# nubot-nudt/LCR-Net

Measured on AMD Instinct MI355X. Metric: scans/s (120k-pt KITTI-shape scan -> 256-D descriptor), higher is better.
Workload: dtype f32 (K-deep GEMMs, K >= 288 and N >= 64: fp32 operands as bf16 x 3 split, 6 of 9 products on the bf16 matrix cores, fp32 accumulate — error vs fp64 <= the fp32-MFMA kernel's; every other GEMM, KPConv and attention: fp32 MFMA); 1 GPU; configs[1]: batch of 8 synthetic 64-beam scans (~120k pts, 0.3 m voxel -> ~16k pts), voxelise + 3 subsamples + 10 radius searches + KPConv encoder + NetVLAD, seeded random weights; distinct_input_batches=4, streams=pre-processing stream (own host thread, 2 batches ahead) + 2 encoder stream(s), parallelism=scan-parallel x1, all-gather of descriptors

## Files before the change

include/lcr_hip.h:

```cpp
#ifndef LCR_HIP_H
#define LCR_HIP_H
#include <stddef.h>
#include <stdint.h>
#ifdef __cplusplus
extern "C" {
#endif

#define LCR_OK 0
#define LCR_EARG (-1)
#define LCR_ESPACE (-2)
#define LCR_EHIP (-3)

#define LCR_STATUS_KEY_OVERFLOW 1u
#define LCR_STATUS_LEN_MISMATCH 2u
#define LCR_GN_REPLICAS 8

const char* lcr_last_error(void);
void lcr_ktimer_enable(int on);
void lcr_ktimer_sample(int every);
void lcr_ktimer_kinds(unsigned mask);
int lcr_ktimer_read(int kind, int max_records, double* seconds, int64_t* meta);
int lcr_ktimer_read2(int kind, int max_records, double* seconds, double* seconds_kernel, int64_t* meta);
int lcr_stream_spin(int microseconds, void* stream);
int lcr_version(void);

int lcr_grid_subsample_ws_bytes(int64_t n_cap, int B, size_t* bytes);
int lcr_grid_subsample(const float* xyz, const int64_t* len, int B, int64_t n_cap, float voxel,
                       float* out_xyz, int64_t* out_len, uint32_t* status,
                       void* ws, size_t ws_bytes, void* stream);
int lcr_grid_subsample_ex(const float* xyz, const int64_t* len, int B, int64_t n_cap, float voxel, int key_bits_hint,
                          float* out_xyz, int64_t* out_len, uint32_t* status,
                          void* ws, size_t ws_bytes, void* stream);
int lcr_grid_subsample_rows(const float* xyz, int row_floats, const int64_t* len, int B, int64_t n_cap, float voxel, int key_bits_hint,
                            float* out_xyz, int64_t* out_len, uint32_t* status,
                            void* ws, size_t ws_bytes, void* stream);
int lcr_hashmap_order_host(const uint64_t* keys_host, int64_t n, int64_t* order_host);
int lcr_hashmap_bucket_host(const uint64_t* codes_host, int64_t n, int phase, int64_t* out_host);

int lcr_voxel_down_sample_ws_bytes(int64_t n_cap, int B, size_t* bytes);
int lcr_voxel_down_sample(const float* rows, int row_floats, int out_cols, const int64_t* len, int B, int64_t n_cap, double voxel,
                          int key_bits_hint, float* out_f32, double* out_f64, int64_t* out_len, uint32_t* status,
                          void* ws, size_t ws_bytes, void* stream);

int lcr_support_grid_ws_bytes(int64_t ns_cap, int B, size_t* bytes);
int lcr_support_grid_build(const float* s, const int64_t* slen, int B, int64_t ns_cap, float radius,
                           uint32_t* status, void* grid_ws, size_t grid_ws_bytes, void* stream);
int lcr_radius_query(const float* q, const int64_t* qlen, int B, int64_t nq_cap,
                     const void* grid_ws, int64_t ns_cap , float radius, int limit,
                     int64_t* out_idx64, int32_t* out_idx32, int32_t* out_cnt, void* stream);
int lcr_radius_query_ordered(const float* q, const int64_t* qlen, int B, int64_t nq_cap,
                             const void* grid_ws, int64_t ns_cap, float radius, int limit,
                             int64_t* out_idx64, int32_t* out_idx32, int32_t* out_cnt, const int32_t* q_order, void* stream);
typedef struct LcrRadiusQuery {
    const float*   q;
    const int64_t* qlen;
    int64_t        nq_cap;
    const void*    grid_ws;
    int64_t        ns_cap;
    float          radius;
    int            limit;
    int32_t*       out_idx32;
    const int32_t* q_order;
} LcrRadiusQuery;
#define LCR_RADIUS_QUERY_MULTI_MAX 12
int lcr_radius_query_multi(const LcrRadiusQuery* list, int n, int B, void* stream);
int lcr_support_grid_build_ex(const float* s, const int64_t* slen, int B, int64_t ns_cap, float radius,
                              uint32_t* status, void* grid_ws, size_t grid_ws_bytes, int32_t* order, void* stream);
int lcr_support_grid_order(const void* grid_ws, int64_t ns_cap, int B, int32_t* order, void* stream);
int lcr_radius_search_ws_bytes(int64_t nq_cap, int64_t ns_cap, int B, size_t* bytes);
int lcr_radius_search(const float* q, const float* s, const int64_t* qlen, const int64_t* slen, int B,
                      int64_t nq_cap, int64_t ns_cap, float radius, int limit,
                      int64_t* out_idx64, int32_t* out_idx32, int32_t* out_cnt, uint32_t* status,
                      void* ws, size_t ws_bytes, void* stream);

#define LCR_MAX_STAGES 8
typedef struct LcrPrecomputeLayout {
  int     num_stages, B, upsampling;
  int64_t n_raw;
  int     limits[LCR_MAX_STAGES];
  int64_t cap[LCR_MAX_STAGES];
  size_t  off_points[LCR_MAX_STAGES];
  size_t  off_lengths[LCR_MAX_STAGES];
  size_t  off_order[LCR_MAX_STAGES];
  size_t  off_neighbors[LCR_MAX_STAGES];
  size_t  off_subsampling[LCR_MAX_STAGES];
  size_t  off_upsampling[LCR_MAX_STAGES];
  size_t  out_bytes, ws_bytes;
} LcrPrecomputeLayout;
int lcr_precompute_layout(int64_t n0, int B, int num_stages, const int* limits, int upsampling, int64_t n_raw,
                          LcrPrecomputeLayout* layout);
int lcr_precompute_batch(const float* points0, const int64_t* lengths0, const LcrPrecomputeLayout* layout, float voxel_size,
                         float radius, float raw_voxel, int key_bits_hint, void* out, size_t out_bytes, void* ws, size_t ws_bytes,
                         int64_t* lengths_host, uint32_t* status_host, void* stream);
int lcr_precompute_batch_rows(const float* points0, int raw_row_floats, const int64_t* lengths0, const LcrPrecomputeLayout* layout,
                              float voxel_size, float radius, float raw_voxel, int key_bits_hint, void* out, size_t out_bytes, void* ws,
                              size_t ws_bytes, int64_t* lengths_host, uint32_t* status_host, void* stream);
int lcr_precompute_ws_bytes_ex(const LcrPrecomputeLayout* layout, int raw_method, size_t* bytes);
int lcr_precompute_batch_rows_ex(const float* points0, int raw_row_floats, const int64_t* lengths0, const LcrPrecomputeLayout* layout,
                                 float voxel_size, float radius, double raw_voxel, int raw_method, int key_bits_hint, void* out,
                                 size_t out_bytes, void* ws, size_t ws_bytes, int64_t* lengths_host, uint32_t* status_host, void* stream);

int lcr_gemm_f32(const float* A, const float* B, float* C, int64_t M, int N, int K, int transA, int transB,
                 const float* bias, const float* rowdiv, const int64_t* seg_len, int S, int groups, double* stats,
                 void* stream);
int lcr_split_bf16x3(const float* w, int64_t n, uint16_t* planes, void* stream);
int lcr_split_bf16x3_tiles(const float* w, int N, int K, uint16_t* tiles, void* stream);
int lcr_gemm_f32_bsplit(const float* A, const uint16_t* Bs_tiles, float* C, int64_t M, int N, int K, const float* bias, const float* rowdiv,
                        const int64_t* seg_len, int S, int groups, double* stats, void* stream);
int lcr_gemm_f32_masked(const float* A, const float* B, float* C, int64_t M, int N, int K, const float* bias, const float* rowdiv,
                        const int64_t* seg_len, int S, int groups, double* stats, const uint16_t* row_mask, int block_k, void* stream);
int lcr_gemm_f32_bsplit_masked(const float* A, const uint16_t* Bs_tiles, float* C, int64_t M, int N, int K, const float* bias,
                               const float* rowdiv, const int64_t* seg_len, int S, int groups, double* stats, const uint16_t* row_mask,
                               int block_k, void* stream);
int lcr_kpconv_mask_ok(int64_t M, int N, int K, int split);
int lcr_gemm_f32_anorm(const float* A, const float* B, float* C, int64_t M, int N, int K, const float* bias,
                       const double* a_stats, const float* a_gamma, const float* a_beta, int a_groups, float a_eps,
                       float a_slope, const int64_t* seg_len, int S, int groups, double* stats, void* stream);
int lcr_gemm_f32_batched_ta(const float* A, const float* B, float* C, int64_t M, int N, int count, const int* k_host,
                            const int64_t* a_off_host, const int64_t* b_off_host, const int64_t* c_off_host, void* stream);
int lcr_kpconv_aggregate(const float* s_feats, const uint8_t* s_pos, const float* q_pts, const float* s_pts,
                         const void* idx, int idx_is_64, int64_t M, int64_t Ns, int H, int C,
                         const float* kernel_points_host, float sigma, float* A, float* nn,
                         const int32_t* order , void* stream);
#define LCR_KP_VALID_FIRST 1
int lcr_kpconv_aggregate_ex(const float* s_feats, const uint8_t* s_pos, const float* q_pts, const float* s_pts,
                            const void* idx, int idx_is_64, int64_t M, int64_t Ns, int H, int C,
                            const float* kernel_points_host, float sigma, float* A, float* nn,
                            const int32_t* order, int flags, void* stream);
int lcr_kpconv_aggregate_mask(const float* s_feats, const uint8_t* s_pos, const float* q_pts, const float* s_pts,
                              const void* idx, int idx_is_64, int64_t M, int64_t Ns, int H, int C,
                              const float* kernel_points_host, float sigma, float* A, float* nn, uint16_t* mask,
                              const int32_t* order, int flags, void* stream);
int lcr_kpconv_fused(const float* s_feats, const uint8_t* s_pos, const float* q_pts, const float* s_pts, const void* idx,
                     int idx_is_64, int64_t M, int64_t Ns, int H, int C, const float* kernel_points_host, float sigma,
                     const float* W, const float* bias, float* out, const int64_t* seg_len, int S, int groups, double* stats,
                     const int32_t* order, void* stream);
int lcr_kpconv_cin1(const float* s_feats, const float* q_pts, const float* s_pts, const void* idx, int idx_is_64,
                    int64_t M, int64_t Ns, int H, const float* kernel_points_host, float sigma, const float* W,
                    const float* bias, int Cout, float* out, const int32_t* order, void* stream);
int lcr_maxpool(const float* x, const void* idx, int idx_is_64, int64_t M, int64_t Ns, int H, int C, float* out,
                const int32_t* order, void* stream);
int lcr_row_positive(const float* x, int64_t N, int C, uint8_t* pos, void* stream);
int lcr_groupnorm_stats(const float* x, int64_t N, int C, int groups, const int64_t* seg_len, int S, double* stats, void* stream);
int lcr_groupnorm_apply(const float* x, const double* stats, const float* gamma, const float* beta, const float* res,
                        const double* res_stats, const float* res_gamma, const float* res_beta, float* y, int64_t N, int C,
                        int groups, const int64_t* seg_len, int S, float eps, float slope, int act, uint8_t* pos, void* stream);

#define LCR_ENC_BLOCKS 10
typedef struct LcrUnaryW {
  const float *w, *b;
  const float *gn_w, *gn_b;
  const uint16_t* w_split;
} LcrUnaryW;
typedef struct LcrBlockW {
  int   cin, cout, strided;
  float sigma;
  const float* kernel_points_host;
  const float *kp_w, *kp_b;
  const float* kp_wt;
  const uint16_t* kp_wt_split;
  const float *normconv_w, *normconv_b;
  LcrUnaryW unary1, unary2, shortcut;
} LcrBlockW;
typedef struct LcrEncoderW {
  int   groups, c1_cout;
  float c1_sigma;
  const float* c1_kernel_points_host;
  const float *c1_w, *c1_b;
  const float *c1_gn_w, *c1_gn_b;
  LcrBlockW blocks[LCR_ENC_BLOCKS];
} LcrEncoderW;
int lcr_encoder_ws_bytes(const LcrEncoderW* W, const int64_t* n_host, int S, size_t* bytes);
int lcr_encoder_forward(const LcrEncoderW* W, const float* feats0, const float* const* points, const int32_t* const* neighbors,
                        const int32_t* const* subsampling, const int32_t* const* order, const int64_t* const* seg_len, int S,
                        const int64_t* n_host, const int64_t* seg_min_rows_host, const int* limits, float* const* out_feats, void* ws,
                        size_t ws_bytes, void* stream);
#define LCR_ENC_LISTS_VALID_FIRST 1u
int lcr_encoder_forward_ex(const LcrEncoderW* W, const float* feats0, const float* const* points, const int32_t* const* neighbors,
                           const int32_t* const* subsampling, const int32_t* const* order, const int64_t* const* seg_len, int S,
                           const int64_t* n_host, const int64_t* seg_min_rows_host, const int* limits, float* const* out_feats,
                           unsigned flags, void* ws, size_t ws_bytes, void* stream);

typedef struct LcrNetvladWeights {
  const float* cluster_weights;
  const float* cluster_weights2;
  const float* hidden1_weights;
  const float *bn1_w, *bn1_b, *bn1_mean, *bn1_var;
  const float *bn2_w, *bn2_b, *bn2_mean, *bn2_var;
  const float* gating_weights;
  const float *gbn_w, *gbn_b, *gbn_mean, *gbn_var;
} LcrNetvladWeights;
int lcr_netvlad_ws_bytes(int64_t n_rows, int S, size_t* bytes);
int lcr_netvlad_forward(const float* feats , const int64_t* seg_len_host, int S,
                        const LcrNetvladWeights* weights_host, float* out , void* ws, size_t ws_bytes, void* stream);

int lcr_rotary_embed(float* x, const float* theta, int64_t N, int heads, void* stream);
int lcr_attention_f32(const float* q, const float* k, const float* v, int64_t Nq, int64_t Nk, int heads, int head_dim,
                      float* out, void* stream);
int lcr_attention_seg_f32(const float* q, const float* k, const float* v, const int64_t* q_len_host, const int64_t* k_len_host, int P,
                          int heads, int head_dim, float* out, void* stream);
int lcr_attention_topk_f32(const float* q, const float* k, const float* v, const int64_t* q_len_host, const int64_t* k_len_host,
                           const int* kk_host, int P, int heads, int head_dim, float* out, void* stream);
int lcr_add_layernorm(const float* a, const float* b, const float* gamma, const float* beta, int64_t N, int D, float eps,
                      float* y, void* stream);
int lcr_relu_inplace(float* x, int64_t n, void* stream);

#define LCR_ROFORMER_MAX_BLOCKS 16
typedef struct LcrLinearW {
  const float *w, *b;
} LcrLinearW;
typedef struct LcrRoformerLayerW {
  LcrLinearW   q, k, v, lin;
  const float *ln1_w, *ln1_b;
  float        ln1_eps;
  LcrLinearW   expand, squeeze;
  const float *ln2_w, *ln2_b;
  float        ln2_eps;
} LcrRoformerLayerW;
typedef struct LcrRoformerW {
  int        d_in, d_model, d_out, heads, num_blocks;
  int        block_is_self[LCR_ROFORMER_MAX_BLOCKS];
  LcrLinearW emb1, emb2, in_proj, out_proj;
  LcrRoformerLayerW layers[LCR_ROFORMER_MAX_BLOCKS];
} LcrRoformerW;
int lcr_roformer_ws_bytes(const LcrRoformerW* W, int64_t n_rows, size_t* bytes);
int lcr_roformer_forward(const LcrRoformerW* W, const float* points, const float* feats, const int64_t* lens0_host, const int64_t* lens1_host,
                         int P, float* out, float* theta_out, void* ws, size_t ws_bytes, void* stream);

int lcr_retrieval_ws_bytes(int64_t Q, int64_t C, size_t* bytes);
int lcr_retrieval_topk(const float* queries , int64_t Q, int64_t q0, const float* database , int64_t C,
                       int D, int k, int exclude, int32_t* out_idx , float* out_d2 ,
                       void* ws, size_t ws_bytes, void* stream);

int lcr_gemm_f32_strided_batched(const float* A, const float* B, float* C, int64_t M, int N, int K, int transA, int transB,
                                 int64_t strideA, int64_t strideB, int64_t strideC, int count, void* stream);

int lcr_vote_shift(const float* xyz, const float* offsets, int64_t N, float max_range, float* out, void* stream);
int lcr_greedy_nms_ws_bytes(int64_t n_total, size_t* bytes);
int lcr_greedy_nms(const float* pts, const int64_t* len, int B, int64_t n_total, float radius, uint8_t* keep,
                   int64_t* out_len, void* ws, void* stream);
int lcr_neighbor_mean(const float* pts, const void* idx, int idx_is_64, int64_t M, int H, int64_t pad, float* out, void* stream);
int lcr_point_to_node_ws_bytes(int64_t N, int M, size_t* bytes);
int lcr_point_to_node_partition(const float* points, int64_t N, const float* nodes, int M, int K, int32_t* p2n, int64_t* knn,
                                uint8_t* knn_mask, uint8_t* node_mask, uint32_t* status, void* ws, size_t ws_bytes, void* stream);

int lcr_point_to_node_partition_stack(const float* points, const int64_t* point_off, const float* nodes, const int64_t* node_off, int C, int K,
                                      int32_t* p2n_out, int64_t* knn, uint8_t* knn_mask, uint8_t* node_mask, uint32_t* status, void* ws,
                                      size_t ws_bytes, void* stream);
int lcr_build_padded_scores(const float* raw, const uint8_t* row_mask, const uint8_t* col_mask, int64_t B, int M, int N,
                            float scale, const float* alpha, float inf_val, float* S, void* stream);
int lcr_log_sinkhorn(float* S, const uint8_t* row_mask, const uint8_t* col_mask, int64_t B, int M, int N, int iters,
                     float inf_val, float* uv_ws, void* stream);
int lcr_log_sinkhorn_ws_floats(int64_t B, int M, int N, size_t* floats);
int lcr_log_sinkhorn_form(int64_t B, int M, int N, int* form);
int lcr_log_sinkhorn_ex(float* S, const uint8_t* row_mask, const uint8_t* col_mask, int64_t B, int M, int N, int iters,
                        float inf_val, float* uv_ws, size_t uv_floats, void* stream);
int lcr_top1_matching_ws_bytes(int64_t B, int M, int N, size_t* bytes);
int lcr_top1_matching(const float* logS, int64_t B, int M, int N, const uint8_t* row_mask, const uint8_t* col_mask,
                      int64_t* total, int32_t* out_bij, float* out_score, void* ws, size_t ws_bytes, void* stream);
int lcr_top1_matching_ex(const float* logS, int64_t B, int M, int N, const uint8_t* row_mask, const uint8_t* col_mask, int mutual,
                         int64_t* total, int32_t* out_bij, float* out_score, void* ws, size_t ws_bytes, void* stream);
int lcr_patch_scores(const float* feats_a, int64_t Na, const float* feats_b, int64_t Nb, int C, const int64_t* idx_a, const int64_t* idx_b,
                     const uint8_t* mask_a, const uint8_t* mask_b, int64_t P, int K, float scale, const float* alpha, float inf_val, float* S,
                     void* stream);
int lcr_topk_matching_ws_bytes(int64_t B, int M, int N, size_t* bytes);
int lcr_topk_matching(const float* logS, int64_t B, int M, int N, const uint8_t* row_mask, const uint8_t* col_mask, int K, int mutual,
                      int64_t* total, int32_t* out_bij, float* out_score, void* ws, size_t ws_bytes, void* stream);
int lcr_topk_matching_ex(const float* logS, int64_t B, int M, int N, const uint8_t* row_mask, const uint8_t* col_mask, int K, int mutual,
                         int use_dustbin, float confidence_threshold, const float* global_scores, int64_t* total, int32_t* out_bij,
                         float* out_score, void* ws, size_t ws_bytes, void* stream);
int lcr_upsample_concat(const float* x, int64_t Nx, int C1, const void* idx, int idx_is_64, int H, const float* skip, int C2,
                        int64_t N, float* out, void* stream);
int lcr_gather_rows(const float* src, int64_t pad, int C, const int64_t* idx, int64_t R, float* out, void* stream);
int lcr_procrustes_batched(const float* src, const float* ref, const float* w, const int32_t* start, int P, float eps, float* T, void* stream);
int lcr_inlier_count(const float* T, int P, const float* src, const float* ref, int n, float radius, const int32_t* start,
                     int min_count, int32_t* counts, int32_t* best, void* stream);
int lcr_lgr_ws_bytes(int64_t n, int H, int S, size_t* bytes);
int lcr_local_global_registration(const float* src, const float* ref, const float* score, int64_t n, const int32_t* hyp_start, int H,
                                  const int32_t* seg_hyp_start, int S, float radius, int min_count, int steps, float* T_out,
                                  float* hyp_out, int32_t* counts_out, int32_t* best_out, void* ws, size_t ws_bytes, void* stream);
int lcr_local_global_registration_ex(const float* src, const float* ref, const float* score, int64_t n, const int32_t* hyp_start, int H,
                                     const int32_t* seg_hyp_start, int S, float radius, int min_count, int steps, int correspondence_limit,
                                     float* T_out, float* hyp_out, int32_t* counts_out, int32_t* best_out, void* ws, size_t ws_bytes,
                                     void* stream);
int lcr_inlier_weights(const float* T_all, const int32_t* sel, const float* src, const float* ref, const float* score, int n,
                       float radius, float* w_out, void* stream);

int lcr_ransac_ws_bytes(int S, int iterations, size_t* bytes);
int lcr_ransac_correspondences(const float* src, const float* ref, const int32_t* start, int S, float thr, int ransac_n, int iterations,
                               uint64_t seed, float* T, int32_t* inliers, float* rmse, int32_t* best_h, float* T_all, int32_t* counts_all,
                               float* sse_all, void* ws, size_t ws_bytes, void* stream);
int lcr_ransac_sample_host(uint64_t seed, int64_t h0, int64_t count, int ransac_n, int64_t n, int32_t* idx_host);
int lcr_ransac_ex_ws_bytes(int S, int iterations, int64_t n_corr, size_t* bytes);
int lcr_ransac_correspondences_ex(const float* src, const float* ref, const int32_t* start, int S, const int32_t* corr, const int32_t* src_start,
                                  const int32_t* ref_start, int64_t n_corr, float thr, int ransac_n, int iterations, uint64_t seed,
                                  float edge_similarity, float checker_distance, float* T, int32_t* inliers, float* rmse, int32_t* best_h,
                                  float* T_all, int32_t* counts_all, float* sse_all, uint8_t* reject_all, void* ws, size_t ws_bytes, void* stream);

int lcr_feature_nn_ws_bytes(int S, int64_t nq, int64_t nd, size_t* bytes);
int lcr_feature_nn(const float* qf, const float* df, const int32_t* q_start, const int32_t* d_start, int S, int C, int64_t nq, int64_t nd,
                   int32_t* nn, float* d2, void* ws, size_t ws_bytes, void* stream);
int lcr_feature_correspondences_ws_bytes(int S, size_t* bytes);
int lcr_feature_correspondences(const int32_t* nn_sr, const int32_t* src_start, const int32_t* nn_rs, const int32_t* ref_start, int S, int min_rows,
                                int32_t* corr, int32_t* start, int32_t* mutual_used, void* ws, size_t ws_bytes, void* stream);

int lcr_icp_ws_bytes(int S, int64_t ns, int64_t nt, size_t* bytes);
int lcr_icp_point_to_point(const float* src, const int64_t* src_len, const float* tgt, const int64_t* tgt_len, int S, const double* init,
                           float max_correspondence_distance, int max_iteration, double relative_fitness, double relative_rmse, double* T,
                           double* fitness, double* inlier_rmse, int32_t* iterations, int32_t* corr, double* T_hist, double* fitness_hist,
                           double* rmse_hist, int check_every, void* ws, size_t ws_bytes, void* stream);

int lcr_icp_plane_ws_bytes(int S, int64_t ns, int64_t nt, size_t* bytes);
int lcr_icp_point_to_plane(const float* src, const int64_t* src_len, const float* tgt, const int64_t* tgt_len, const float* tgt_normals, int S,
                           const double* init, float max_correspondence_distance, int max_iteration, double relative_fitness,
                           double relative_rmse, double* T, double* fitness, double* inlier_rmse, int32_t* iterations, int32_t* corr,
                           double* T_hist, double* fitness_hist, double* rmse_hist, int check_every, void* ws, size_t ws_bytes, void* stream);

int lcr_normals_ws_bytes(int B, int64_t n, size_t* bytes);
int lcr_estimate_normals(const float* points, const int64_t* lengths, int B, float radius, int max_nn, const float* viewpoint, float* normals,
                         float* curvature, int32_t* count, void* ws, size_t ws_bytes, void* stream);

#ifdef __cplusplus
}
#endif
#endif
```

include/lcr_hip_debug.h:

```cpp
#ifndef LCR_HIP_DEBUG_H
#define LCR_HIP_DEBUG_H

#ifdef __cplusplus
extern "C" {
#endif

void lcr_gemm_debug_force_tile(int tile);
void lcr_gemm_debug_deep(int mode);
void lcr_gemm_debug_streamk(int mode);
void lcr_groupnorm_debug_general(int on);
void lcr_kpconv_debug_off64(int on);

#ifdef __cplusplus
}
#endif
#endif
```

lcr-net_amd/_lib.py:

```python
import ctypes
import os

import torch

_PKG = os.path.dirname(os.path.abspath(__file__))
LIB_PATH = os.path.join(_PKG, "liblcr_hip.so")

_lib = None

c_f32p = ctypes.c_void_p
c_vp = ctypes.c_void_p
c_i64 = ctypes.c_int64
c_int = ctypes.c_int
c_float = ctypes.c_float
c_size_p = ctypes.POINTER(ctypes.c_size_t)
c_size_t = ctypes.c_size_t

_SIGS = {
    "lcr_last_error": (ctypes.c_char_p, []),
    "lcr_version": (c_int, []),
    "lcr_support_grid_ws_bytes": (c_int, [c_i64, c_int, c_size_p]),
    "lcr_support_grid_build": (c_int, [c_vp, c_vp, c_int, c_i64, c_float, c_vp, c_vp, ctypes.c_size_t, c_vp]),
    "lcr_precompute_layout": (c_int, [c_i64, c_int, c_int, c_vp, c_int, c_i64, c_vp]),
    "lcr_precompute_batch": (c_int, [c_vp, c_vp, c_vp, c_float, c_float, c_float, c_int, c_vp, c_size_t, c_vp, c_size_t, c_vp, c_vp, c_vp]),
    "lcr_precompute_batch_rows": (c_int, [c_vp, c_int, c_vp, c_vp, c_float, c_float, c_float, c_int, c_vp, c_size_t, c_vp, c_size_t, c_vp, c_vp, c_vp]),
    "lcr_precompute_ws_bytes_ex": (c_int, [c_vp, c_int, c_size_p]),
    "lcr_precompute_batch_rows_ex": (c_int, [c_vp, c_int, c_vp, c_vp, c_float, c_float, ctypes.c_double, c_int, c_int, c_vp, c_size_t, c_vp, c_size_t,
                                             c_vp, c_vp, c_vp]),
    "lcr_radius_query_multi": (c_int, [c_vp, c_int, c_int, c_vp]),
    "lcr_radius_query": (c_int, [c_vp, c_vp, c_int, c_i64, c_vp, c_i64, c_float, c_int, c_vp, c_vp, c_vp, c_vp]),
    "lcr_stream_spin": (c_int, [c_int, c_vp]),
    "lcr_radius_query_ordered": (c_int, [c_vp, c_vp, c_int, c_i64, c_vp, c_i64, c_float, c_int, c_vp, c_vp, c_vp, c_vp, c_vp]),
    "lcr_radius_search_ws_bytes": (c_int, [c_i64, c_i64, c_int, c_size_p]),
    "lcr_radius_search": (c_int, [c_vp, c_vp, c_vp, c_vp, c_int, c_i64, c_i64, c_float, c_int, c_vp, c_vp, c_vp, c_vp,
                                  c_vp, ctypes.c_size_t, c_vp]),
    "lcr_grid_subsample_ws_bytes": (c_int, [c_i64, c_int, c_size_p]),
    "lcr_grid_subsample": (c_int, [c_vp, c_vp, c_int, c_i64, c_float, c_vp, c_vp, c_vp, c_vp, ctypes.c_size_t, c_vp]),
    "lcr_grid_subsample_ex": (c_int, [c_vp, c_vp, c_int, c_i64, c_float, c_int, c_vp, c_vp, c_vp, c_vp, ctypes.c_size_t, c_vp]),
    "lcr_grid_subsample_rows": (c_int, [c_vp, c_int, c_vp, c_int, c_i64, c_float, c_int, c_vp, c_vp, c_vp, c_vp, ctypes.c_size_t, c_vp]),
    "lcr_hashmap_order_host": (c_int, [c_vp, c_i64, c_vp]),
    "lcr_hashmap_bucket_host": (c_int, [c_vp, c_i64, c_int, c_vp]),
    "lcr_voxel_down_sample_ws_bytes": (c_int, [c_i64, c_int, c_size_p]),
    "lcr_voxel_down_sample": (c_int, [c_vp, c_int, c_int, c_vp, c_int, c_i64, ctypes.c_double, c_int, c_vp, c_vp, c_vp, c_vp, c_vp, ctypes.c_size_t,
                                      c_vp]),
    "lcr_gemm_f32": (c_int, [c_vp, c_vp, c_vp, c_i64, c_int, c_int, c_int, c_int, c_vp, c_vp, c_vp, c_int, c_int, c_vp, c_vp]),
    "lcr_gemm_f32_anorm": (c_int, [c_vp, c_vp, c_vp, c_i64, c_int, c_int, c_vp, c_vp, c_vp, c_vp, c_int, c_float, c_float, c_vp, c_int,
                                   c_int, c_vp, c_vp]),
    "lcr_ktimer_enable": (None, [c_int]),
    "lcr_ktimer_sample": (None, [c_int]),
    "lcr_ktimer_kinds": (None, [ctypes.c_uint]),
    "lcr_ktimer_read": (c_int, [c_int, c_int, c_vp, c_vp]),
    "lcr_ktimer_read2": (c_int, [c_int, c_int, c_vp, c_vp, c_vp]),
    "lcr_encoder_ws_bytes": (c_int, [c_vp, c_vp, c_int, c_size_p]),
    "lcr_encoder_forward": (c_int, [c_vp, c_vp, c_vp, c_vp, c_vp, c_vp, c_vp, c_int, c_vp, c_vp, c_vp, c_vp, c_vp, c_size_t, c_vp]),
    "lcr_roformer_ws_bytes": (c_int, [c_vp, c_i64, c_size_p]),
    "lcr_roformer_forward": (c_int, [c_vp, c_vp, c_vp, c_vp, c_vp, c_int, c_vp, c_vp, c_vp, c_size_t, c_vp]),
    "lcr_encoder_forward_ex": (c_int, [c_vp, c_vp, c_vp, c_vp, c_vp, c_vp, c_vp, c_int, c_vp, c_vp, c_vp, c_vp, ctypes.c_uint, c_vp, c_size_t, c_vp]),
    "lcr_kpconv_aggregate": (c_int, [c_vp, c_vp, c_vp, c_vp, c_vp, c_int, c_i64, c_i64, c_int, c_int, c_vp, c_float, c_vp, c_vp, c_vp, c_vp]),
    "lcr_kpconv_aggregate_mask": (c_int, [c_vp, c_vp, c_vp, c_vp, c_vp, c_int, c_i64, c_i64, c_int, c_int, c_vp, c_float, c_vp, c_vp, c_vp, c_vp,
                                          c_int, c_vp]),
    "lcr_kpconv_fused": (c_int, [c_vp, c_vp, c_vp, c_vp, c_vp, c_int, c_i64, c_i64, c_int, c_int, c_vp, c_float, c_vp, c_vp, c_vp, c_vp, c_int,
                                 c_int, c_vp, c_vp, c_vp]),
    "lcr_kpconv_cin1": (c_int, [c_vp, c_vp, c_vp, c_vp, c_int, c_i64, c_i64, c_int, c_vp, c_float, c_vp, c_vp, c_int, c_vp, c_vp, c_vp]),
    "lcr_maxpool": (c_int, [c_vp, c_vp, c_int, c_i64, c_i64, c_int, c_int, c_vp, c_vp, c_vp]),
    "lcr_support_grid_order": (c_int, [c_vp, c_i64, c_int, c_vp, c_vp]),
    "lcr_row_positive": (c_int, [c_vp, c_i64, c_int, c_vp, c_vp]),
    "lcr_groupnorm_stats": (c_int, [c_vp, c_i64, c_int, c_int, c_vp, c_int, c_vp, c_vp]),
    "lcr_groupnorm_apply": (c_int, [c_vp, c_vp, c_vp, c_vp, c_vp, c_vp, c_vp, c_vp, c_vp, c_i64, c_int, c_int, c_vp, c_int,
                                    c_float, c_float, c_int, c_vp, c_vp]),
    "lcr_rotary_embed": (c_int, [c_vp, c_vp, c_i64, c_int, c_vp]),
    "lcr_attention_f32": (c_int, [c_vp, c_vp, c_vp, c_i64, c_i64, c_int, c_int, c_vp, c_vp]),
    "lcr_attention_seg_f32": (c_int, [c_vp, c_vp, c_vp, c_vp, c_vp, c_int, c_int, c_int, c_vp, c_vp]),
    "lcr_attention_topk_f32": (c_int, [c_vp, c_vp, c_vp, c_vp, c_vp, c_vp, c_int, c_int, c_int, c_vp, c_vp]),
    "lcr_add_layernorm": (c_int, [c_vp, c_vp, c_vp, c_vp, c_i64, c_int, c_float, c_vp, c_vp]),
    "lcr_relu_inplace": (c_int, [c_vp, c_i64, c_vp]),
    "lcr_retrieval_ws_bytes": (c_int, [c_i64, c_i64, c_size_p]),
    "lcr_retrieval_topk": (c_int, [c_vp, c_i64, c_i64, c_vp, c_i64, c_int, c_int, c_int, c_vp, c_vp, c_vp, ctypes.c_size_t, c_vp]),
    "lcr_gemm_f32_strided_batched": (c_int, [c_vp, c_vp, c_vp, c_i64, c_int, c_int, c_int, c_int, c_i64, c_i64, c_i64, c_int, c_vp]),
    "lcr_gemm_f32_batched_ta": (c_int, [c_vp, c_vp, c_vp, c_i64, c_int, c_int, c_vp, c_vp, c_vp, c_vp, c_vp]),
    "lcr_vote_shift": (c_int, [c_vp, c_vp, c_i64, c_float, c_vp, c_vp]),
    "lcr_greedy_nms_ws_bytes": (c_int, [c_i64, c_size_p]),
    "lcr_greedy_nms": (c_int, [c_vp, c_vp, c_int, c_i64, c_float, c_vp, c_vp, c_vp, c_vp]),
    "lcr_neighbor_mean": (c_int, [c_vp, c_vp, c_int, c_i64, c_int, c_i64, c_vp, c_vp]),
    "lcr_point_to_node_ws_bytes": (c_int, [c_i64, c_int, c_size_p]),
    "lcr_point_to_node_partition": (c_int, [c_vp, c_i64, c_vp, c_int, c_int, c_vp, c_vp, c_vp, c_vp, c_vp, c_vp, ctypes.c_size_t, c_vp]),
    "lcr_point_to_node_partition_stack": (c_int, [c_vp, c_vp, c_vp, c_vp, c_int, c_int, c_vp, c_vp, c_vp, c_vp, c_vp, c_vp, ctypes.c_size_t, c_vp]),
    "lcr_build_padded_scores": (c_int, [c_vp, c_vp, c_vp, c_i64, c_int, c_int, c_float, c_vp, c_float, c_vp, c_vp]),
    "lcr_log_sinkhorn": (c_int, [c_vp, c_vp, c_vp, c_i64, c_int, c_int, c_int, c_float, c_vp, c_vp]),
    "lcr_log_sinkhorn_ws_floats": (c_int, [c_i64, c_int, c_int, c_size_p]),
    "lcr_log_sinkhorn_form": (c_int, [c_i64, c_int, c_int, ctypes.POINTER(c_int)]),
    "lcr_split_bf16x3": (c_int, [c_vp, c_i64, c_vp, c_vp]),
    "lcr_split_bf16x3_tiles": (c_int, [c_vp, c_int, c_int, c_vp, c_vp]),
    "lcr_gemm_f32_bsplit": (c_int, [c_vp, c_vp, c_vp, c_i64, c_int, c_int, c_vp, c_vp, c_vp, c_int, c_int, c_vp, c_vp]),
    "lcr_gemm_f32_bsplit_masked": (c_int, [c_vp, c_vp, c_vp, c_i64, c_int, c_int, c_vp, c_vp, c_vp, c_int, c_int, c_vp, c_vp, c_int, c_vp]),
    "lcr_gemm_f32_masked": (c_int, [c_vp, c_vp, c_vp, c_i64, c_int, c_int, c_vp, c_vp, c_vp, c_int, c_int, c_vp, c_vp, c_int, c_vp]),
    "lcr_kpconv_mask_ok": (c_int, [c_i64, c_int, c_int, c_int]),
    "lcr_log_sinkhorn_ex": (c_int, [c_vp, c_vp, c_vp, c_i64, c_int, c_int, c_int, c_float, c_vp, ctypes.c_size_t, c_vp]),
    "lcr_top1_matching_ws_bytes": (c_int, [c_i64, c_int, c_int, c_size_p]),
    "lcr_top1_matching": (c_int, [c_vp, c_i64, c_int, c_int, c_vp, c_vp, c_vp, c_vp, c_vp, c_vp, ctypes.c_size_t, c_vp]),
    "lcr_top1_matching_ex": (c_int, [c_vp, c_i64, c_int, c_int, c_vp, c_vp, c_int, c_vp, c_vp, c_vp, c_vp, ctypes.c_size_t, c_vp]),
    "lcr_topk_matching_ws_bytes": (c_int, [c_i64, c_int, c_int, c_size_p]),
    "lcr_topk_matching": (c_int, [c_vp, c_i64, c_int, c_int, c_vp, c_vp, c_int, c_int, c_vp, c_vp, c_vp, c_vp, ctypes.c_size_t, c_vp]),
    "lcr_patch_scores": (c_int, [c_vp, c_i64, c_vp, c_i64, c_int, c_vp, c_vp, c_vp, c_vp, c_i64, c_int, c_float, c_vp, c_float, c_vp, c_vp]),
    "lcr_topk_matching_ex": (c_int, [c_vp, c_i64, c_int, c_int, c_vp, c_vp, c_int, c_int, c_int, c_float, c_vp, c_vp, c_vp, c_vp, c_vp, ctypes.c_size_t,
                                     c_vp]),
    "lcr_local_global_registration_ex": (c_int, [c_vp, c_vp, c_vp, c_i64, c_vp, c_int, c_vp, c_int, c_float, c_int, c_int, c_int, c_vp, c_vp, c_vp, c_vp,
                                                 c_vp, ctypes.c_size_t, c_vp]),
    "lcr_upsample_concat": (c_int, [c_vp, c_i64, c_int, c_vp, c_int, c_int, c_vp, c_int, c_i64, c_vp, c_vp]),
    "lcr_gather_rows": (c_int, [c_vp, c_i64, c_int, c_vp, c_i64, c_vp, c_vp]),
    "lcr_procrustes_batched": (c_int, [c_vp, c_vp, c_vp, c_vp, c_int, c_float, c_vp, c_vp]),
    "lcr_inlier_count": (c_int, [c_vp, c_int, c_vp, c_vp, c_int, c_float, c_vp, c_int, c_vp, c_vp, c_vp]),
    "lcr_inlier_weights": (c_int, [c_vp, c_vp, c_vp, c_vp, c_vp, c_int, c_float, c_vp, c_vp]),
    "lcr_lgr_ws_bytes": (c_int, [c_i64, c_int, c_int, c_size_p]),
    "lcr_local_global_registration": (c_int, [c_vp, c_vp, c_vp, c_i64, c_vp, c_int, c_vp, c_int, c_float, c_int, c_int, c_vp, c_vp, c_vp, c_vp, c_vp,
                                              ctypes.c_size_t, c_vp]),
    "lcr_netvlad_ws_bytes": (c_int, [c_i64, c_int, c_size_p]),
    "lcr_netvlad_forward": (c_int, [c_vp, c_vp, c_int, c_vp, c_vp, c_vp, ctypes.c_size_t, c_vp]),
    "lcr_ransac_ws_bytes": (c_int, [c_int, c_int, c_size_p]),
    "lcr_ransac_correspondences": (c_int, [c_vp, c_vp, c_vp, c_int, c_float, c_int, c_int, ctypes.c_uint64, c_vp, c_vp, c_vp, c_vp, c_vp, c_vp, c_vp,
                                           c_vp, ctypes.c_size_t, c_vp]),
    "lcr_ransac_sample_host": (c_int, [ctypes.c_uint64, c_i64, c_i64, c_int, c_i64, c_vp]),
    "lcr_ransac_ex_ws_bytes": (c_int, [c_int, c_int, c_i64, c_size_p]),
    "lcr_ransac_correspondences_ex": (c_int, [c_vp, c_vp, c_vp, c_int, c_vp, c_vp, c_vp, c_i64, c_float, c_int, c_int, ctypes.c_uint64, c_float,
                                              c_float, c_vp, c_vp, c_vp, c_vp, c_vp, c_vp, c_vp, c_vp, c_vp, ctypes.c_size_t, c_vp]),
    "lcr_feature_nn_ws_bytes": (c_int, [c_int, c_i64, c_i64, c_size_p]),
    "lcr_feature_nn": (c_int, [c_vp, c_vp, c_vp, c_vp, c_int, c_int, c_i64, c_i64, c_vp, c_vp, c_vp, ctypes.c_size_t, c_vp]),
    "lcr_feature_correspondences_ws_bytes": (c_int, [c_int, c_size_p]),
    "lcr_feature_correspondences": (c_int, [c_vp, c_vp, c_vp, c_vp, c_int, c_int, c_vp, c_vp, c_vp, c_vp, ctypes.c_size_t, c_vp]),
    "lcr_icp_ws_bytes": (c_int, [c_int, c_i64, c_i64, c_size_p]),
    "lcr_icp_point_to_point": (c_int, [c_vp, c_vp, c_vp, c_vp, c_int, c_vp, c_float, c_int, ctypes.c_double, ctypes.c_double, c_vp, c_vp, c_vp, c_vp,
                                       c_vp, c_vp, c_vp, c_vp, c_int, c_vp, ctypes.c_size_t, c_vp]),
    "lcr_icp_plane_ws_bytes": (c_int, [c_int, c_i64, c_i64, c_size_p]),
    "lcr_icp_point_to_plane": (c_int, [c_vp, c_vp, c_vp, c_vp, c_vp, c_int, c_vp, c_float, c_int, ctypes.c_double, ctypes.c_double, c_vp, c_vp,
                                       c_vp, c_vp, c_vp, c_vp, c_vp, c_vp, c_int, c_vp, ctypes.c_size_t, c_vp]),
    "lcr_normals_ws_bytes": (c_int, [c_int, c_i64, c_size_p]),
    "lcr_estimate_normals": (c_int, [c_vp, c_vp, c_int, c_float, c_int, c_vp, c_vp, c_vp, c_vp, c_vp, ctypes.c_size_t, c_vp]),
}


_RELEASES_GIL = {"lcr_roformer_forward", "lcr_precompute_batch", "lcr_precompute_batch_rows", "lcr_precompute_batch_rows_ex", "lcr_hashmap_bucket_host", "lcr_encoder_forward", "lcr_encoder_forward_ex", "lcr_ktimer_read",
                 "lcr_ktimer_read2", "lcr_hashmap_order_host", "lcr_ransac_sample_host", "lcr_icp_point_to_point", "lcr_icp_point_to_plane", "lcr_netvlad_forward", "lcr_log_sinkhorn", "lcr_log_sinkhorn_ex",
                 "lcr_local_global_registration", "lcr_local_global_registration_ex", "lcr_retrieval_topk", "lcr_stream_spin"}


def build():
    import importlib.util
    spec = importlib.util.spec_from_file_location("_lcr_build", os.path.join(_PKG, "csrc", "build.py"))
    mod = importlib.util.module_from_spec(spec)
    spec.loader.exec_module(mod)
    return mod.build()


def lib():
    global _lib
    if _lib is None:
        if not os.path.exists(LIB_PATH):
            raise RuntimeError(
                "liblcr_hip.so not found at %s — build it with `python lcr-net_amd/csrc/build.py` "
                "(there is no CPU fallback for the lcr-net_amd hot path)" % LIB_PATH)
        L = ctypes.CDLL(LIB_PATH)
        for name, (res, args) in _SIGS.items():
            if not hasattr(L, name):
                continue
            fn = getattr(L, name)
            fn.restype = res
            fn.argtypes = args
        if os.environ.get("LCR_CTYPES_KEEP_GIL", "1") != "0":
            K = ctypes.PyDLL(LIB_PATH)
            for name, (res, args) in _SIGS.items():
                if name in _RELEASES_GIL or not hasattr(K, name):
                    continue
                fn = getattr(K, name)
                fn.restype = res
                fn.argtypes = args
                setattr(L, name, fn)
        _lib = L
    return _lib


def check(rc, what):
    if rc != 0:
        msg = lib().lcr_last_error()
        raise RuntimeError("%s failed (rc=%d): %s" % (what, rc, msg.decode() if msg else ""))


def ptr(t):
    return ctypes.c_void_p(t.data_ptr()) if t is not None else ctypes.c_void_p(0)


def stream_ptr(device=None):
    idx = device.index if isinstance(device, torch.device) else None
    if idx is None:
        idx = torch.cuda.current_device() if not isinstance(device, int) else device
    return ctypes.c_void_p(torch._C._cuda_getCurrentRawStream(idx))


def require_cuda(*tensors):
    for t in tensors:
        if t is not None and not t.is_cuda:
            raise RuntimeError("lcr-net_amd ops run on the GPU only: got a %s tensor (no CPU fallback)" % t.device)


def workspace(nbytes, device):
    return torch.empty(max(int(nbytes), 256), dtype=torch.uint8, device=device)
```

lcr-net_amd/csrc/encoder.hip:

```cpp
#include <algorithm>
#include <cstdlib>
#include <cstring>

#include "common.h"

#define TURN(call) ([&]() { LaunchTurn turn_; return (call); }())

namespace lcr {

constexpr float ENC_GN_EPS = 1e-5f;
constexpr float ENC_SLOPE = 0.1f;

struct Arena {
  char*  base;
  size_t off, cap;
  template <typename T>
  T* take(size_t n) {
    const size_t o = off;
    off = align_up(off + n * sizeof(T));
    return (base && off <= cap) ? reinterpret_cast<T*>(base + o) : nullptr;
  }
};

struct StageIO {
  const float*   pts;
  const int64_t* seg;
  const int32_t* order;
  int64_t        n;
  int64_t        min_rows;
};

struct StatsPool {
  double* base;
  size_t  off, cap;
  int     S, groups;
  double* take() {
    const size_t n = static_cast<size_t>(GN_REPLICAS) * S * groups * 2;
    if (off + n > cap) return nullptr;
    double* p = base + off;
    off += n;
    return p;
  }
};

static size_t stats_doubles(int S, int groups) { return static_cast<size_t>(GN_REPLICAS) * S * groups * 2 * 44; }

static int unary_raw(const LcrUnaryW& u, const float* x, int64_t n, int cin, int cout, const StageIO& st, StatsPool& sp, Arena& ws,
                     float** y_out, double** stats_out, hipStream_t s) {
  float* y = ws.take<float>(static_cast<size_t>(n) * cout);
  double* stats = sp.take();
  if (!y || !stats) return LCR_ESPACE;
  const bool split = u.w_split && cin >= 288 && cin % 32 == 0 && cout >= 64;
  int rc = split ? TURN(lcr_gemm_f32_bsplit(x, u.w_split, y, n, cout, cin, u.b, nullptr, st.seg, sp.S, sp.groups, stats, s))
                 : TURN(lcr_gemm_f32(x, u.w, y, n, cout, cin, 0, 1, u.b, nullptr, st.seg, sp.S, sp.groups, stats, s));
  *y_out = y;
  *stats_out = stats;
  return rc;
}

static int residual_block(const LcrBlockW& b, const float* s_feats, const StageIO& q, const StageIO& sup, const void* idx, int H,
                          StatsPool& sp, Arena& ws, float* out, unsigned enc_flags, hipStream_t s) {
  const int mid = b.cout / 4, g = sp.groups;
  const int64_t M = q.n, Ns = sup.n;
  int rc;
  const float* x = s_feats;
  uint8_t* pos = ws.take<uint8_t>(static_cast<size_t>(Ns));
  if (!pos) return LCR_ESPACE;
  if (b.unary1.w) {
    float* y1;
    double* st1;
    if ((rc = unary_raw(b.unary1, s_feats, Ns, b.cin, mid, sup, sp, ws, &y1, &st1, s))) return rc;
    float* x1 = ws.take<float>(static_cast<size_t>(Ns) * mid);
    if (!x1) return LCR_ESPACE;
    if ((rc = TURN(lcr_groupnorm_apply(y1, st1, b.unary1.gn_w, b.unary1.gn_b, nullptr, nullptr, nullptr, nullptr, x1, Ns, mid, g, sup.seg, sp.S,
                                  ENC_GN_EPS, ENC_SLOPE, 1, pos, s))))
      return rc;
    x = x1;
  } else if ((rc = TURN(lcr_row_positive(s_feats, Ns, b.cin, pos, s)))) {
    return rc;
  }
  float* A = ws.take<float>(static_cast<size_t>(M) * 15 * mid);
  float* nn = ws.take<float>(static_cast<size_t>(M));
  float* kpo = ws.take<float>(static_cast<size_t>(M) * mid);
  uint16_t* kmask = ws.take<uint16_t>(static_cast<size_t>(M));
  double* stc = sp.take();
  if (!A || !nn || !kpo || !kmask || !stc) return LCR_ESPACE;
  static const bool vf_env_off = getenv("LCR_KP_VALID_FIRST") && atoi(getenv("LCR_KP_VALID_FIRST")) == 0;
  const int vf_flag = ((enc_flags & LCR_ENC_LISTS_VALID_FIRST) && !vf_env_off) ? LCR_KP_VALID_FIRST : 0;
  static const bool fused32 = getenv("LCR_KPCONV_FUSED") != nullptr;
  if (fused32 && mid == 32 && sp.S <= 64) {
    if ((rc = TURN(lcr_kpconv_fused(x, pos, q.pts, sup.pts, idx, 0, M, Ns, H, mid, b.kernel_points_host, b.sigma, b.kp_w, b.kp_b, kpo, q.seg, sp.S, g,
                                    stc, q.order, s))))
      return rc;
  } else {
    const bool split = b.kp_wt_split && mid >= 64;
    if (!((split || b.kp_wt) && lcr_kpconv_mask_ok(M, mid, 15 * mid, split))) kmask = nullptr;
    if ((rc = TURN(lcr_kpconv_aggregate_mask(x, pos, q.pts, sup.pts, idx, 0, M, Ns, H, mid, b.kernel_points_host, b.sigma, A, nn, kmask, q.order, vf_flag,
                                             s))))
      return rc;
    if (split) {
      if ((rc = TURN(kmask ? lcr_gemm_f32_bsplit_masked(A, b.kp_wt_split, kpo, M, mid, 15 * mid, b.kp_b, nn, q.seg, sp.S, g, stc, kmask, mid, s)
                           : lcr_gemm_f32_bsplit(A, b.kp_wt_split, kpo, M, mid, 15 * mid, b.kp_b, nn, q.seg, sp.S, g, stc, s))))
        return rc;
    } else if (kmask) {
      if ((rc = TURN(lcr_gemm_f32_masked(A, b.kp_wt, kpo, M, mid, 15 * mid, b.kp_b, nn, q.seg, sp.S, g, stc, kmask, mid, s)))) return rc;
    } else if ((rc = TURN(b.kp_wt ? lcr_gemm_f32(A, b.kp_wt, kpo, M, mid, 15 * mid, 0, 1, b.kp_b, nn, q.seg, sp.S, g, stc, s)
                                  : lcr_gemm_f32(A, b.kp_w, kpo, M, mid, 15 * mid, 0, 0, b.kp_b, nn, q.seg, sp.S, g, stc, s)))) return rc;
  }
  float* y;
  double* sty;
  static const bool no_anorm = getenv("LCR_NO_NORM_ON_LOAD") != nullptr;
  if (!no_anorm && mid <= 256 && mid % 4 == 0 && b.cout > 32 && q.min_rows >= 64) {
    y = ws.take<float>(static_cast<size_t>(M) * b.cout);
    sty = sp.take();
    if (!y || !sty) return LCR_ESPACE;
    if ((rc = TURN(lcr_gemm_f32_anorm(kpo, b.unary2.w, y, M, b.cout, mid, b.unary2.b, stc, b.normconv_w, b.normconv_b, g, ENC_GN_EPS, ENC_SLOPE,
                                      q.seg, sp.S, g, sty, s))))
      return rc;
  } else {
    float* x2 = ws.take<float>(static_cast<size_t>(M) * mid);
    if (!x2) return LCR_ESPACE;
    if ((rc = TURN(lcr_groupnorm_apply(kpo, stc, b.normconv_w, b.normconv_b, nullptr, nullptr, nullptr, nullptr, x2, M, mid, g, q.seg, sp.S, ENC_GN_EPS,
                                  ENC_SLOPE, 1, nullptr, s))))
      return rc;
    if ((rc = unary_raw(b.unary2, x2, M, mid, b.cout, q, sp, ws, &y, &sty, s))) return rc;
  }
  const float* res = s_feats;
  if (b.strided) {
    float* pooled = ws.take<float>(static_cast<size_t>(M) * b.cin);
    if (!pooled) return LCR_ESPACE;
    if ((rc = TURN(lcr_maxpool(s_feats, idx, 0, M, Ns, H, b.cin, pooled, q.order, s)))) return rc;
    res = pooled;
  }
  const double* str = nullptr;
  if (b.shortcut.w) {
    float* r;
    double* st;
    if ((rc = unary_raw(b.shortcut, res, M, b.cin, b.cout, q, sp, ws, &r, &st, s))) return rc;
    res = r;
    str = st;
  }
  return TURN(lcr_groupnorm_apply(y, sty, b.unary2.gn_w, b.unary2.gn_b, res, str, str ? b.shortcut.gn_w : nullptr, str ? b.shortcut.gn_b : nullptr, out,
                             M, b.cout, g, q.seg, sp.S, ENC_GN_EPS, ENC_SLOPE, 1, nullptr, s));
}

static size_t block_ws_bytes(const LcrBlockW& b, int64_t M, int64_t Ns) {
  Arena a{nullptr, 0, ~size_t(0)};
  const int mid = b.cout / 4;
  a.take<uint8_t>(Ns);
  a.take<float>(static_cast<size_t>(Ns) * mid);
  a.take<float>(static_cast<size_t>(Ns) * mid);
  a.take<float>(static_cast<size_t>(M) * 15 * mid);
  a.take<float>(M);
  a.take<float>(static_cast<size_t>(M) * mid);
  a.take<uint16_t>(static_cast<size_t>(M));
  a.take<float>(static_cast<size_t>(M) * mid);
  a.take<float>(static_cast<size_t>(M) * b.cout);
  a.take<float>(static_cast<size_t>(M) * b.cin);
  a.take<float>(static_cast<size_t>(M) * b.cout);
  return a.off;
}

static const int BLOCK_Q[LCR_ENC_BLOCKS] = {0, 1, 1, 1, 2, 2, 2, 3, 3, 3};
static const int BLOCK_S[LCR_ENC_BLOCKS] = {0, 0, 1, 1, 1, 2, 2, 2, 3, 3};

}

using namespace lcr;

extern "C" int lcr_encoder_ws_bytes(const LcrEncoderW* W, const int64_t* n_host, int S, size_t* bytes) {
  if (!W || !n_host || !bytes || S < 1) return LCR_EARG;
  size_t blk = 0, pp = 0;
  for (int i = 0; i < LCR_ENC_BLOCKS; ++i) {
    blk = std::max(blk, block_ws_bytes(W->blocks[i], n_host[BLOCK_Q[i]], n_host[BLOCK_S[i]]));
    pp = std::max(pp, align_up(sizeof(float) * static_cast<size_t>(n_host[BLOCK_Q[i]]) * W->blocks[i].cout));
  }
  pp = std::max(pp, align_up(sizeof(float) * static_cast<size_t>(n_host[0]) * W->c1_cout * 2));
  *bytes = blk + 2 * pp + align_up(sizeof(double) * stats_doubles(S, W->groups)) + 4096;
  return LCR_OK;
}

extern "C" int lcr_encoder_forward(const LcrEncoderW* W, const float* feats0, const float* const* points, const int32_t* const* neighbors,
                                   const int32_t* const* subsampling, const int32_t* const* order, const int64_t* const* seg_len, int S,
                                   const int64_t* n_host, const int64_t* seg_min_rows_host, const int* limits, float* const* out_feats,
                                   void* ws, size_t ws_bytes, void* stream) {
  return lcr_encoder_forward_ex(W, feats0, points, neighbors, subsampling, order, seg_len, S, n_host, seg_min_rows_host, limits, out_feats, 0u, ws,
                                ws_bytes, stream);
}

extern "C" int lcr_encoder_forward_ex(const LcrEncoderW* W, const float* feats0, const float* const* points, const int32_t* const* neighbors,
                                      const int32_t* const* subsampling, const int32_t* const* order, const int64_t* const* seg_len, int S,
                                      const int64_t* n_host, const int64_t* seg_min_rows_host, const int* limits, float* const* out_feats,
                                      unsigned flags, void* ws, size_t ws_bytes, void* stream) {
  if (!W || !feats0 || !points || !neighbors || !subsampling || !seg_len || !n_host || !limits || !out_feats || !ws || S < 1) {
    set_error("lcr_encoder_forward: bad argument");
    return LCR_EARG;
  }
  size_t need = 0;
  lcr_encoder_ws_bytes(W, n_host, S, &need);
  if (ws_bytes < need) {
    set_error("lcr_encoder_forward: workspace too small (%zu < %zu)", ws_bytes, need);
    return LCR_ESPACE;
  }
  hipStream_t s = static_cast<hipStream_t>(stream);
  StageIO st[4];
  for (int i = 0; i < 4; ++i) st[i] = StageIO{points[i], seg_len[i], order ? order[i] : nullptr, n_host[i], seg_min_rows_host ? seg_min_rows_host[i] : 0};
  Arena top{static_cast<char*>(ws), 0, ws_bytes};
  StatsPool sp{top.take<double>(stats_doubles(S, W->groups)), 0, stats_doubles(S, W->groups), S, W->groups};
  size_t pp = 0;
  for (int i = 0; i < LCR_ENC_BLOCKS; ++i) pp = std::max(pp, sizeof(float) * static_cast<size_t>(n_host[BLOCK_Q[i]]) * W->blocks[i].cout);
  pp = std::max(pp, sizeof(float) * static_cast<size_t>(n_host[0]) * W->c1_cout * 2);
  float* ping = reinterpret_cast<float*>(top.take<char>(pp));
  float* pong = reinterpret_cast<float*>(top.take<char>(pp));
  const size_t scratch0 = top.off;
  if (!sp.base || !ping || !pong) return LCR_ESPACE;
  hipMemsetAsync(sp.base, 0, sizeof(double) * sp.cap, s);

  int rc;
  float* cur;
  {
    const int64_t n0 = n_host[0];
    float* raw = ping;
    float* f = ping + static_cast<size_t>(n0) * W->c1_cout;
    double* stt = sp.take();
    if ((rc = TURN(lcr_kpconv_cin1(feats0, st[0].pts, st[0].pts, neighbors[0], 0, n0, n0, limits[0], W->c1_kernel_points_host, W->c1_sigma, W->c1_w,
                              W->c1_b, W->c1_cout, raw, st[0].order, s))))
      return rc;
    if ((rc = TURN(lcr_groupnorm_stats(raw, n0, W->c1_cout, W->groups, st[0].seg, S, stt, s)))) return rc;
    if ((rc = TURN(lcr_groupnorm_apply(raw, stt, W->c1_gn_w, W->c1_gn_b, nullptr, nullptr, nullptr, nullptr, f, n0, W->c1_cout, W->groups, st[0].seg, S,
                                  ENC_GN_EPS, ENC_SLOPE, 1, nullptr, s))))
      return rc;
    cur = f;
  }
  static const int STAGE_LAST[4] = {0, 3, 6, 9};
  for (int i = 0; i < LCR_ENC_BLOCKS; ++i) {
    const int qs = BLOCK_Q[i], ss = BLOCK_S[i];
    const bool strided = qs != ss;
    const void* idx = strided ? static_cast<const void*>(subsampling[ss]) : static_cast<const void*>(neighbors[qs]);
    const int H = limits[ss];
    float* out = nullptr;
    for (int k = 0; k < 4; ++k)
      if (STAGE_LAST[k] == i) out = out_feats[k];
    if (!out) out = (cur >= ping && cur < ping + pp / sizeof(float)) ? pong : ping;
    Arena scratch{static_cast<char*>(ws), scratch0, ws_bytes};
    if ((rc = residual_block(W->blocks[i], cur, st[qs], st[ss], idx, H, sp, scratch, out, flags, s))) {
      if (rc == LCR_ESPACE) set_error("lcr_encoder_forward: block %d ran out of workspace", i);
      return rc;
    }
    cur = out;
  }
  return check_launch("lcr_encoder_forward");
}
```

lcr-net_amd/csrc/gemm_f32.hip:

```cpp
#include <cstdio>
#include <cstdlib>
#include <map>
#include <mutex>
#include <type_traits>

#include "common.h"

namespace lcr {

typedef float floatx16 __attribute__((ext_vector_type(16)));

constexpr int GM_BK = 32;
constexpr int GM_T = 256;

constexpr int GM_MAX_BATCH = 64;
struct GemmBatch {
  int     count;
  int     strided;
  int     k[GM_MAX_BATCH];
  int64_t a_off[GM_MAX_BATCH], b_off[GM_MAX_BATCH], c_off[GM_MAX_BATCH];
};

struct GemmEpilogue {
  const float*   bias;
  const float*   rowdiv;
  const int64_t* seg_len;
  int            S;
  int            groups;
  double*        stats;
};

struct ANorm {
  const double* stats;
  const float*  gamma;
  const float*  beta;
  int           groups;
  float         eps, slope;
};
constexpr int AN_KMAX = 256;

__device__ __forceinline__ float4 ld4(const float* p) { return *reinterpret_cast<const float4*>(p); }

template <int R, int LD, bool VEC, bool RM = false>
struct LoaderT {
  static constexpr int PIECES = R * 8 / GM_T;
  float4 reg[PIECES];
  unsigned okmask;
  int kb;
  __device__ __forceinline__ void load(const float* __restrict__ src, int64_t rows_total, int K, int64_t r0, int k0) {
    kb = k0;
#pragma unroll
    for (int j = 0; j < PIECES; ++j) {
      const int f = threadIdx.x + GM_T * j;
      const int row = f >> 3, c4 = f & 7;
      int64_t gr = r0 + row;
      gr = gr < rows_total ? gr : rows_total - 1;
      const int gk = k0 + c4 * 4;
      if (VEC) {
        const bool ok = gk < K;
        reg[j] = ld4(src + gr * K + (ok ? gk : 0));
        okmask = j == 0 ? (ok ? 1u : 0u) : (okmask | (ok ? (1u << j) : 0u));
      } else {
        const float* p = src + gr * K;
        float4 v;
        v.x = gk + 0 < K ? p[gk + 0] : 0.f;
        v.y = gk + 1 < K ? p[gk + 1] : 0.f;
        v.z = gk + 2 < K ? p[gk + 2] : 0.f;
        v.w = gk + 3 < K ? p[gk + 3] : 0.f;
        reg[j] = v;
        okmask = ~0u;
      }
    }
  }
  __device__ __forceinline__ void store_piece(float* __restrict__ S, int j) const {
    const int f = threadIdx.x + GM_T * j;
    const int row = f >> 3, c4 = f & 7;
    const bool ok = (okmask >> j) & 1u;
    if (RM) {
      *reinterpret_cast<float4*>(&S[row * LD + c4 * 4]) = ok ? reg[j] : make_float4(0.f, 0.f, 0.f, 0.f);
      return;
    }
    S[(c4 * 4 + 0) * LD + row] = ok ? reg[j].x : 0.f;
    S[(c4 * 4 + 1) * LD + row] = ok ? reg[j].y : 0.f;
    S[(c4 * 4 + 2) * LD + row] = ok ? reg[j].z : 0.f;
    S[(c4 * 4 + 3) * LD + row] = ok ? reg[j].w : 0.f;
  }
  __device__ __forceinline__ void store(float* __restrict__ S) const {
#pragma unroll
    for (int j = 0; j < PIECES; ++j) store_piece(S, j);
  }
  __device__ __forceinline__ void store_norm(float* __restrict__ S, const float* __restrict__ tab, int split, float slope) const {
    static_assert(RM, "normalise-on-load is built for the row-major A tile");
#pragma unroll
    for (int j = 0; j < PIECES; ++j) {
      const int f = threadIdx.x + GM_T * j;
      const int row = f >> 3, c4 = f & 7;
      const bool ok = (okmask >> j) & 1u;
      const float* t = tab + (row >= split ? 2 * AN_KMAX : 0) + (ok ? kb + c4 * 4 : 0);
      const float4 sc = *reinterpret_cast<const float4*>(t), sh = *reinterpret_cast<const float4*>(t + AN_KMAX);
      float4 v;
      v.x = fmaf(reg[j].x, sc.x, sh.x), v.y = fmaf(reg[j].y, sc.y, sh.y), v.z = fmaf(reg[j].z, sc.z, sh.z), v.w = fmaf(reg[j].w, sc.w, sh.w);
      v.x = v.x > 0.f ? v.x : v.x * slope, v.y = v.y > 0.f ? v.y : v.y * slope;
      v.z = v.z > 0.f ? v.z : v.z * slope, v.w = v.w > 0.f ? v.w : v.w * slope;
      *reinterpret_cast<float4*>(&S[row * LD + c4 * 4]) = ok ? v : make_float4(0.f, 0.f, 0.f, 0.f);
    }
  }
};

template <int W, int LD, bool VEC>
struct LoaderN {
  static constexpr int PIECES = 8 * W / GM_T;
  float4 reg[PIECES];
  unsigned okmask;
  __device__ __forceinline__ void load(const float* __restrict__ src, int64_t cols_total, int K, int64_t c0, int k0) {
#pragma unroll
    for (int j = 0; j < PIECES; ++j) {
      const int f = threadIdx.x + GM_T * j;
      const int kr = f / (W / 4), c4 = f % (W / 4);
      const int gk = k0 + kr;
      const int64_t gc = c0 + c4 * 4;
      const bool kok = gk < K;
      const float* p = src + static_cast<int64_t>(kok ? gk : 0) * cols_total;
      if (VEC) {
        const bool ok = kok && gc < cols_total;
        reg[j] = ld4(p + (gc < cols_total ? gc : 0));
        okmask = j == 0 ? (ok ? 1u : 0u) : (okmask | (ok ? (1u << j) : 0u));
      } else {
        float4 v;
        v.x = (kok && gc + 0 < cols_total) ? p[gc + 0] : 0.f;
        v.y = (kok && gc + 1 < cols_total) ? p[gc + 1] : 0.f;
        v.z = (kok && gc + 2 < cols_total) ? p[gc + 2] : 0.f;
        v.w = (kok && gc + 3 < cols_total) ? p[gc + 3] : 0.f;
        reg[j] = v;
        okmask = ~0u;
      }
    }
  }
  __device__ __forceinline__ void store_piece(float* __restrict__ S, int j) const {
    const int f = threadIdx.x + GM_T * j;
    const int kr = f / (W / 4), c4 = f % (W / 4);
    const bool ok = (okmask >> j) & 1u;
    *reinterpret_cast<float4*>(&S[kr * LD + c4 * 4]) = ok ? reg[j] : make_float4(0.f, 0.f, 0.f, 0.f);
  }
  __device__ __forceinline__ void store(float* __restrict__ S) const {
#pragma unroll
    for (int j = 0; j < PIECES; ++j) store_piece(S, j);
  }
};

__device__ __forceinline__ int seg_of_row(const int64_t* __restrict__ seg_len, int S, int64_t row) {
  int s = 0;
  int64_t end = seg_len[0];
  while (s + 1 < S && row >= end) {
    ++s;
    end += seg_len[s];
  }
  return s;
}

template <int BM, int BN, int WM, int WN, int NT>
__device__ __forceinline__ void gemm_epilogue(floatx16 (&acc)[NT], float* __restrict__ C, int64_t M, int N, int64_t m0, int n0, int64_t m_tile,
                                              const GemmEpilogue& ep, const float (&bias_v)[NT], int blk_first, int64_t blk_seg_start,
                                              int64_t blk_seg_end, int wm, int wn, int lane) {
  const bool want_stats = ep.stats != nullptr;
  const int gs = want_stats ? N / ep.groups : 1;
  const int64_t wrow0 = m0 + wm * 32;

  const bool interior = m0 + BM <= M && n0 + BN <= N && M * static_cast<int64_t>(N) < (int64_t(1) << 30);
  if (interior) {
    const unsigned row_l = static_cast<unsigned>(wrow0) + 4u * static_cast<unsigned>(lane >> 5);
#pragma unroll
    for (int j = 0; j < NT; ++j) {
      const unsigned col = static_cast<unsigned>(n0 + wn * (32 * NT) + j * 32 + (lane & 31));
      const float bv = bias_v[j];
      const unsigned off0 = row_l * static_cast<unsigned>(N) + col;
      if (ep.rowdiv) {
#pragma unroll
        for (int r = 0; r < 16; ++r) {
          const unsigned dr = static_cast<unsigned>((r & 3) + 8 * (r >> 2));
          const float v = acc[j][r] / ep.rowdiv[row_l + dr] + bv;
          C[off0 + dr * static_cast<unsigned>(N)] = v;
          acc[j][r] = v;
        }
      } else {
#pragma unroll
        for (int r = 0; r < 16; ++r) {
          const unsigned dr = static_cast<unsigned>((r & 3) + 8 * (r >> 2));
          const float v = acc[j][r] + bv;
          C[off0 + dr * static_cast<unsigned>(N)] = v;
          acc[j][r] = v;
        }
      }
    }
  } else
#pragma unroll
  for (int j = 0; j < NT; ++j) {
    const int col = n0 + wn * (32 * NT) + j * 32 + (lane & 31);
    const float bv = bias_v[j];
#pragma unroll
    for (int r = 0; r < 16; ++r) {
      const int64_t row = wrow0 + (r & 3) + 8 * (r >> 2) + 4 * (lane >> 5);
      float v = acc[j][r];
      if (row < M) {
        if (ep.rowdiv) v = v / ep.rowdiv[row];
        v += bv;
        if (col < N) C[row * N + col] = v;
      } else {
        v = 0.f;
      }
      acc[j][r] = v;
    }
  }

  if (want_stats) {
    __shared__ float s_part[2][2 * WM][BN];
    double* rep = ep.stats + static_cast<int64_t>(m_tile % GN_REPLICAS) * ep.S * ep.groups * 2;
    int64_t seg_start = blk_seg_start, seg_end = blk_seg_end;
    const int64_t blk_last_row = min(m0 + BM - 1, M - 1);
    const bool uniform = blk_last_row < seg_end;
    if (uniform) {
#pragma unroll
      for (int j = 0; j < NT; ++j) {
        float s = 0.f, ss = 0.f;
#pragma unroll
        for (int r = 0; r < 16; ++r) {
          s += acc[j][r];
          ss = fmaf(acc[j][r], acc[j][r], ss);
        }
        const int cl = wn * (32 * NT) + j * 32 + (lane & 31);
        s_part[0][2 * wm + (lane >> 5)][cl] = s;
        s_part[1][2 * wm + (lane >> 5)][cl] = ss;
      }
      __syncthreads();
      if (threadIdx.x < BN) {
        const int cl = threadIdx.x;
        double ds = 0.0, dss = 0.0;
#pragma unroll
        for (int r = 0; r < 2 * WM; ++r) {
          ds += static_cast<double>(s_part[0][r][cl]);
          dss += static_cast<double>(s_part[1][r][cl]);
        }
        const int span = gs < 64 ? gs : 64;
        for (int d = 1; d < span; d <<= 1) {
          ds += __shfl_xor(ds, d);
          dss += __shfl_xor(dss, d);
        }
        const int col = n0 + cl;
        if ((cl & (span - 1)) == 0 && col < N) {
          double* d = rep + (static_cast<int64_t>(blk_first) * ep.groups + col / gs) * 2;
          atomicAdd(d, ds);
          atomicAdd(d + 1, dss);
        }
      }
    } else if (wrow0 < M) {
      const int64_t wlast = min(wrow0 + 31, M - 1);
      int sg = blk_first;
      while (sg + 1 < ep.S && wrow0 >= seg_end) {
        ++sg;
        seg_start = seg_end;
        seg_end += ep.seg_len[sg];
      }
      while (true) {
        const bool whole = seg_start <= wrow0 && wlast < seg_end;
#pragma unroll
        for (int j = 0; j < NT; ++j) {
          const int col = n0 + wn * (32 * NT) + j * 32 + (lane & 31);
          float s = 0.f, ss = 0.f;
#pragma unroll
          for (int r = 0; r < 16; ++r) {
            const int64_t row = wrow0 + (r & 3) + 8 * (r >> 2) + 4 * (lane >> 5);
            const float v = (whole || (row >= seg_start && row < seg_end)) ? acc[j][r] : 0.f;
            s += v;
            ss = fmaf(v, v, ss);
          }
          double ds = s, dss = ss;
          ds += __shfl_xor(ds, 32);
          dss += __shfl_xor(dss, 32);
          const int span = gs < 32 ? gs : 32;
          for (int d = 1; d < span; d <<= 1) {
            ds += __shfl_xor(ds, d);
            dss += __shfl_xor(dss, d);
          }
          if (lane < 32 && (lane & (span - 1)) == 0 && col < N) {
            double* d = rep + (static_cast<int64_t>(sg) * ep.groups + col / gs) * 2;
            atomicAdd(d, ds);
            atomicAdd(d + 1, dss);
          }
        }
        if (wlast < seg_end || sg + 1 >= ep.S) break;
        ++sg;
        seg_start = seg_end;
        seg_end += ep.seg_len[sg];
      }
    }
  }
}

template <int BM, int BN, int WM, int WN, bool TA, bool TB, bool VEC, bool SHORT = false, bool ANORM = false>
__global__ __launch_bounds__(GM_T, SHORT ? 6 : 2) void k_gemm_f32(const float* __restrict__ A, const float* __restrict__ B, float* __restrict__ C,
                                                       int64_t M, int N, int K, GemmEpilogue ep, GemmBatch batch, ANorm an) {
  static_assert(!ANORM || (SHORT && !TA && VEC && BN / (32 * WN) == 1), "normalise-on-load: light form, row-major A");
  static_assert(WM * WN == 4 && BM == 32 * WM, "one 32-row MFMA tile per wavefront along M");
  constexpr int k_begin = 0;
  if (batch.count) {
    const int z = blockIdx.z;
    if (batch.strided) {
      A += static_cast<int64_t>(z) * batch.a_off[0];
      B += static_cast<int64_t>(z) * batch.b_off[0];
      C += static_cast<int64_t>(z) * batch.c_off[0];
      K = batch.k[0];
    } else {
      A += batch.a_off[z];
      B += batch.b_off[z];
      C += batch.c_off[z];
      K = batch.k[z];
    }
  }
  constexpr int NT = BN / (32 * WN);
  constexpr int NBUF = SHORT ? 1 : 2;
  constexpr bool NEWP = NT == 1;
  constexpr bool ARM = NEWP && !TA, BRM = NEWP && TB;
  constexpr int LDR = GM_BK + 4;
  constexpr int LDA = ARM ? LDR : (TA ? BM + 4 : BM + 1);
  constexpr int LDB = BRM ? LDR : (TB ? BN + 1 : BN + 4);
  __shared__ __attribute__((aligned(16))) float As[NBUF][ARM ? BM * LDR : GM_BK * LDA];
  __shared__ __attribute__((aligned(16))) float Bs[NBUF][BRM ? BN * LDR : GM_BK * LDB];

  const int lane = threadIdx.x & 63, w = __builtin_amdgcn_readfirstlane(threadIdx.x >> 6);
  const int wm = w / WN, wn = w % WN;
  const int ntn = (N + BN - 1) / BN;
  const int xcd = blockIdx.x & 7, slot = blockIdx.x >> 3;
  const int64_t m_tile = static_cast<int64_t>(slot / ntn) * 8 + xcd;
  const int64_t m0 = m_tile * BM;
  const int n0 = (slot % ntn) * BN;
  if (m0 >= M) return;

  LoaderT<BM, LDA, VEC, ARM> la_t[NBUF];
  LoaderN<BM, LDA, VEC> la_n[NBUF];
  LoaderT<BN, LDB, VEC, BRM> lb_t[NBUF];
  LoaderN<BN, LDB, VEC> lb_n[NBUF];

  auto gload = [&](int k0, int r) {
    if (TA) la_n[r].load(A, M, K, m0, k0);
    else la_t[r].load(A, M, K, m0, k0);
    if (TB) lb_t[r].load(B, N, K, n0, k0);
    else lb_n[r].load(B, N, K, n0, k0);
  };
  auto sstore = [&](int buf, int r) {
    if (TA) la_n[r].store(As[buf]);
    else la_t[r].store(As[buf]);
    if (TB) lb_t[r].store(Bs[buf]);
    else lb_n[r].store(Bs[buf]);
  };

  constexpr int NACC = (NT == 1 && BM == 128) ? 2 : 1;
  floatx16 acc[NT], acc2[NT];
#pragma unroll
  for (int j = 0; j < NT; ++j)
#pragma unroll
    for (int r = 0; r < 16; ++r) {
      acc[j][r] = 0.f;
      acc2[j][r] = 0.f;
    }

  const int nk = (K + GM_BK - 1) / GM_BK;
  gload(k_begin, 0);
  if (!SHORT) gload(k_begin + GM_BK, NBUF - 1);
  const bool want_stats = ep.stats != nullptr;
  float bias_v[NT];
#pragma unroll
  for (int j = 0; j < NT; ++j) {
    const int col = n0 + (w % WN) * (32 * NT) + j * 32 + (lane & 31);
    bias_v[j] = (ep.bias && col < N) ? ep.bias[col] : 0.f;
  }
  float an_g[2] = {0.f, 0.f}, an_b[2] = {0.f, 0.f};
  if constexpr (ANORM) {
#pragma unroll
    for (int u = 0; u < 2; ++u) {
      const int e = threadIdx.x + u * GM_T;
      if (e < 2 * K) {
        const int k = e >= K ? e - K : e;
        an_g[u] = an.gamma[k];
        an_b[u] = an.beta[k];
      }
    }
  }
  int blk_first = 0;
  int64_t blk_seg_start = 0, blk_seg_end = 0;
  if (want_stats || ANORM) {
    blk_seg_end = ep.seg_len[0];
    while (blk_first + 1 < ep.S && m0 >= blk_seg_end) {
      ++blk_first;
      blk_seg_start = blk_seg_end;
      blk_seg_end += ep.seg_len[blk_first];
    }
  }
  __shared__ __attribute__((aligned(16))) float s_an[ANORM ? 4 * AN_KMAX : 4];
  int an_split = BM;
  if constexpr (ANORM) {
    an_split = static_cast<int>(min(static_cast<int64_t>(BM), blk_seg_end - m0));
    const int gs = K / an.groups;
    __shared__ float2 s_mr[2 * 64];
    for (int e = threadIdx.x; e < 2 * an.groups; e += GM_T) {
      const int slot = e >= an.groups ? 1 : 0, g = e - slot * an.groups;
      const int sg = min(blk_first + slot, ep.S - 1);
      const double cnt = static_cast<double>(ep.seg_len[sg]) * gs;
      double sx = 0.0, sxx = 0.0;
      for (int rep = 0; rep < GN_REPLICAS; ++rep) {
        const int64_t o = ((static_cast<int64_t>(rep) * ep.S + sg) * an.groups + g) * 2;
        sx += an.stats[o];
        sxx += an.stats[o + 1];
      }
      const double mean = sx / cnt;
      const double var = fmax(sxx / cnt - mean * mean, 0.0);
      s_mr[e] = make_float2(static_cast<float>(mean), static_cast<float>(1.0 / sqrt(var + static_cast<double>(an.eps))));
    }
    __syncthreads();
#pragma unroll
    for (int u = 0; u < 2; ++u) {
      const int e = threadIdx.x + u * GM_T;
      if (e < 2 * K) {
        const int slot = e >= K ? 1 : 0, k = e - slot * K;
        const float2 mr = s_mr[slot * an.groups + k / gs];
        const float sc = mr.y * an_g[u];
        s_an[slot * 2 * AN_KMAX + k] = sc;
        s_an[slot * 2 * AN_KMAX + AN_KMAX + k] = fmaf(-mr.x, sc, an_b[u]);
      }
    }
    __syncthreads();
  }
  auto sstore_a0 = [&]() {
    if constexpr (ANORM) la_t[0].store_norm(As[0], s_an, an_split, an.slope);
  };
  if constexpr (ANORM) {
    sstore_a0();
    lb_t[0].store(Bs[0]);
  } else {
    sstore(0, 0);
  }
  __syncthreads();
  const int half = lane >> 5;
  const int a_off = ARM ? (wm * 32 + (lane & 31)) * LDR + half * 16 : half * (NEWP ? 16 : 1) * LDA + wm * 32 + (lane & 31);
  const int b_off = BRM ? (wn * (32 * NT) + (lane & 31)) * LDR + half * 16 : half * (NEWP ? 16 : 1) * LDB + wn * (32 * NT) + (lane & 31);
  auto fetch4_a = [&](const float* as, int q, float (&o)[4]) {
    if (ARM) {
      const float4 v = *reinterpret_cast<const float4*>(as + 4 * q);
      o[0] = v.x, o[1] = v.y, o[2] = v.z, o[3] = v.w;
    } else {
#pragma unroll
      for (int i = 0; i < 4; ++i) o[i] = as[(4 * q + i) * LDA];
    }
  };
  auto fetch4_b = [&](const float* bs, int q, float (&o)[4]) {
    if (BRM) {
      const float4 v = *reinterpret_cast<const float4*>(bs + 4 * q);
      o[0] = v.x, o[1] = v.y, o[2] = v.z, o[3] = v.w;
    } else {
#pragma unroll
      for (int i = 0; i < 4; ++i) o[i] = bs[(4 * q + i) * LDB];
    }
  };
  if constexpr (SHORT) {
    constexpr int KKS = GM_BK / 2, PFS = 4;
    for (int t = 0; t < nk; ++t) {
      if (t > 0) {
        gload(k_begin + t * GM_BK, 0);
        __syncthreads();
        if constexpr (ANORM) {
          sstore_a0();
          lb_t[0].store(Bs[0]);
        } else {
          sstore(0, 0);
        }
        __syncthreads();
      }
      const float* as = As[0] + a_off;
      const float* bs = Bs[0] + b_off;
      static_assert(NEWP, "the light form is only instantiated for single-accumulator tiles");
      float af[2][4], bf[2][4];
      fetch4_a(as, 0, af[0]);
      fetch4_b(bs, 0, bf[0]);
      fetch4_a(as, 1, af[1]);
      fetch4_b(bs, 1, bf[1]);
#pragma unroll
      for (int q = 0; q < KKS / 4; ++q) {
#pragma unroll
        for (int i = 0; i < 4; ++i) acc[0] = __builtin_amdgcn_mfma_f32_32x32x2f32(af[q & 1][i], bf[q & 1][i], acc[0], 0, 0, 0);
        if (q + 2 < KKS / 4) {
          fetch4_a(as, q + 2, af[q & 1]);
          fetch4_b(bs, q + 2, bf[q & 1]);
        }
      }
    }
  } else {
  constexpr int KK = GM_BK / 2;
  constexpr int PF = NT == 1 ? KK : (NT == 2 ? 8 : 4);
  constexpr int PA = BM * 8 / GM_T, PB = BN * 8 / GM_T;
  constexpr int ST0 = KK - (PA + PB) - 1 > 2 ? (KK - (PA + PB)) / 2 : 1;
  auto step = [&](auto buf_c, auto full_c, int t) {
    constexpr int BUF = decltype(buf_c)::value;
    constexpr bool FULL = decltype(full_c)::value;
    if (FULL || t + 2 < nk) gload(k_begin + (t + 2) * GM_BK, BUF);
    const bool do_store = FULL || t + 1 < nk;
    const float* as = As[BUF] + a_off;
    const float* bs = Bs[BUF] + b_off;
    float af[PF], bf[PF][NT];
    if constexpr (NEWP) {
#pragma unroll
      for (int q = 0; q < KK / 4; ++q) {
        float a4[4], b4[4];
        fetch4_a(as, q, a4);
        fetch4_b(bs, q, b4);
#pragma unroll
        for (int i = 0; i < 4; ++i) {
          af[4 * q + i] = a4[i];
          bf[4 * q + i][0] = b4[i];
        }
      }
    } else {
#pragma unroll
      for (int d = 0; d < PF; ++d) {
        af[d] = as[d * 2 * LDA];
#pragma unroll
        for (int j = 0; j < NT; ++j) bf[d][j] = bs[d * 2 * LDB + j * 32];
      }
    }
    __builtin_amdgcn_sched_barrier(0);
#pragma unroll
    for (int kk = 0; kk < KK; ++kk) {
      const int sl = kk % PF;
#pragma unroll
      for (int j = 0; j < NT; ++j) {
        if (NACC == 2 && (kk & 1)) acc2[j] = __builtin_amdgcn_mfma_f32_32x32x2f32(af[sl], bf[sl][j], acc2[j], 0, 0, 0);
        else acc[j] = __builtin_amdgcn_mfma_f32_32x32x2f32(af[sl], bf[sl][j], acc[j], 0, 0, 0);
      }
      if (kk + PF < KK) {
        af[sl] = as[(kk + PF) * 2 * LDA];
#pragma unroll
        for (int j = 0; j < NT; ++j) bf[sl][j] = bs[(kk + PF) * 2 * LDB + j * 32];
      }
      const int piece = kk - ST0;
      if (do_store && piece >= 0 && piece < PA + PB) {
        if (piece < PA) {
          if (TA) la_n[1 - BUF].store_piece(As[1 - BUF], piece);
          else la_t[1 - BUF].store_piece(As[1 - BUF], piece);
        } else {
          if (TB) lb_t[1 - BUF].store_piece(Bs[1 - BUF], piece - PA);
          else lb_n[1 - BUF].store_piece(Bs[1 - BUF], piece - PA);
        }
      }
    }
    __syncthreads();
  };
  int t = 0;
  for (; t + 3 < nk; t += 2) {
    step(std::integral_constant<int, 0>{}, std::true_type{}, t);
    step(std::integral_constant<int, 1>{}, std::true_type{}, t + 1);
  }
  for (; t < nk; t += 2) {
    step(std::integral_constant<int, 0>{}, std::false_type{}, t);
    if (t + 1 >= nk) break;
    step(std::integral_constant<int, 1>{}, std::false_type{}, t + 1);
  }

  }

  if (NACC == 2) {
#pragma unroll
    for (int j = 0; j < NT; ++j)
#pragma unroll
      for (int r = 0; r < 16; ++r) acc[j][r] += acc2[j][r];
  }

  gemm_epilogue<BM, BN, WM, WN, NT>(acc, C, M, N, m0, n0, m_tile, ep, bias_v, blk_first, blk_seg_start, blk_seg_end, wm, wn, lane);
}

template <int N_OUTSTANDING>
__device__ __forceinline__ void wait_vmcnt() {
  asm volatile("s_waitcnt vmcnt(%0)" ::"n"(N_OUTSTANDING) : "memory");
}
__device__ __forceinline__ void glds16(const float* base, unsigned off, unsigned lds_dst) {
  unsigned keep;
  asm volatile("s_mov_b32 %0, m0\n\ts_mov_b32 m0, %3\n\ts_nop 0\n\tglobal_load_lds_dwordx4 %1, %2\n\ts_mov_b32 m0, %0"
               : "=&s"(keep)
               : "v"(off), "s"(base), "s"(lds_dst)
               : "memory");
}

__device__ __forceinline__ void glds16_v(const float* addr, unsigned lds_dst) {
  unsigned keep;
  asm volatile("s_mov_b32 %0, m0\n\ts_mov_b32 m0, %2\n\ts_nop 0\n\tglobal_load_lds_dwordx4 %1, off\n\ts_mov_b32 m0, %0"
               : "=&s"(keep)
               : "v"(addr), "s"(lds_dst)
               : "memory");
}
__device__ __attribute__((aligned(16))) float g_zero16[4];

template <int BM, int BN, int WM, int WN, bool MASK = false>
__global__ __launch_bounds__(GM_T, (BM == 64 ? 3 : 2)) void k_gemm_f32_deep(const float* __restrict__ A, const float* __restrict__ B, float* __restrict__ C,
                                                            int64_t M, int N, int K, GemmEpilogue ep, const uint16_t* __restrict__ amask,
                                                            int kshift) {
  static_assert(WM * WN == 4 && BM == 32 * WM && BN == 32 * WN, "one 32x32 accumulator per wavefront");
  constexpr int LA = BM / 32, LB = BN / 32, LPW = LA + LB;
  constexpr int STAGE_A = BM * 128, STAGE = (BM + BN) * 128;
  constexpr int NS = 3;
  __shared__ __attribute__((aligned(1024))) char lds[NS * STAGE];
  const int lane = threadIdx.x & 63, w = __builtin_amdgcn_readfirstlane(threadIdx.x >> 6);
  const int wm = w / WN, wn = w % WN;
  const int ntn = (N + BN - 1) / BN;
  const int xcd = blockIdx.x & 7, slot = blockIdx.x >> 3;
  const int64_t m_tile = static_cast<int64_t>(slot / ntn) * 8 + xcd;
  const int64_t m0 = m_tile * BM;
  const int n0 = (slot % ntn) * BN;
  if (m0 >= M) return;
  const unsigned lds_base = static_cast<unsigned>(reinterpret_cast<uintptr_t>(lds));

  unsigned oa[LA], ob[LB];
  uint32_t rmask[MASK ? LA : 1];
#pragma unroll
  for (int j = 0; j < LA; ++j) {
    const int row = (w * LA + j) * 8 + (lane >> 3);
    const int c = (lane & 7) ^ ((row >> 1) & 7);
    int64_t gr = m0 + row;
    gr = gr < M ? gr : M - 1;
    oa[j] = static_cast<unsigned>((gr * K + c * 4) * 4);
    if constexpr (MASK) rmask[j] = amask[gr];
  }
#pragma unroll
  for (int j = 0; j < LB; ++j) {
    const int row = (w * LB + j) * 8 + (lane >> 3);
    const int c = (lane & 7) ^ ((row >> 1) & 7);
    int gr = n0 + row;
    gr = gr < N ? gr : N - 1;
    ob[j] = static_cast<unsigned>((static_cast<int64_t>(gr) * K + c * 4) * 4);
  }
  const unsigned dst_a = lds_base + w * LA * 1024, dst_b = lds_base + STAGE_A + w * LB * 1024;
  const float* Ak = A;
  const float* Bk = B;
  int kt = 0;
  auto issue_one = [&](int stage, int j) {
    if (j < LA) {
      if constexpr (MASK) {
        const float* src = ((rmask[j] >> (kt >> kshift)) & 1u)
                               ? reinterpret_cast<const float*>(reinterpret_cast<const char*>(A) + (oa[j] + static_cast<unsigned>(kt * GM_BK * 4)))
                               : g_zero16;
        glds16_v(src, dst_a + stage * STAGE + j * 1024);
      } else {
        glds16(Ak, oa[j], dst_a + stage * STAGE + j * 1024);
      }
    } else {
      glds16(Bk, ob[j - LA], dst_b + stage * STAGE + (j - LA) * 1024);
    }
  };
  auto advance = [&] {
    Ak += GM_BK;
    Bk += GM_BK;
    if constexpr (MASK) ++kt;
  };
  auto issue = [&](int stage) {
#pragma unroll
    for (int j = 0; j < LPW; ++j) issue_one(stage, j);
    advance();
  };

  const int half = lane >> 5;
  const int ra = wm * 32 + (lane & 31), rb = wn * 32 + (lane & 31);
  int offa[4], offb[4];
#pragma unroll
  for (int q = 0; q < 4; ++q) {
    offa[q] = ra * 128 + (((4 * half + q) ^ ((ra >> 1) & 7)) << 4);
    offb[q] = STAGE_A + rb * 128 + (((4 * half + q) ^ ((rb >> 1) & 7)) << 4);
  }
  float4 fa[4], fb[4];
  floatx16 acc;
#pragma unroll
  for (int r = 0; r < 16; ++r) acc[r] = 0.f;
  const int nk = K / GM_BK;

  issue(0);
  if (nk > 1) issue(1);
  if (nk > 2) issue(2);
  float bias_v[1];
  {
    const int col = n0 + wn * 32 + (lane & 31);
    bias_v[0] = (ep.bias && col < N) ? ep.bias[col] : 0.f;
  }
  int blk_first = 0;
  int64_t blk_seg_start = 0, blk_seg_end = 0;
  if (ep.stats != nullptr) {
    blk_seg_end = ep.seg_len[0];
    while (blk_first + 1 < ep.S && m0 >= blk_seg_end) {
      ++blk_first;
      blk_seg_start = blk_seg_end;
      blk_seg_end += ep.seg_len[blk_first];
    }
  }
  if (nk > 2) wait_vmcnt<2 * LPW>();
  else if (nk > 1) wait_vmcnt<LPW>();
  else wait_vmcnt<0>();
  __syncthreads();
#pragma unroll
  for (int q = 0; q < 4; ++q) {
    fa[q] = *reinterpret_cast<const float4*>(lds + offa[q]);
    fb[q] = *reinterpret_cast<const float4*>(lds + offb[q]);
  }

  auto mfma = [&](float a, float b) { acc = __builtin_amdgcn_mfma_f32_32x32x2f32(a, b, acc, 0, 0, 0); };
  auto mfma4 = [&](const float4& a, const float4& b) {
    mfma(a.x, b.x);
    mfma(a.y, b.y);
    mfma(a.z, b.z);
    mfma(a.w, b.w);
  };
  auto pin = [] { __builtin_amdgcn_sched_barrier(0); };
  auto step = [&](auto st_c, auto full_c, int t) {
    constexpr int ST = decltype(st_c)::value;
    constexpr bool FULL = decltype(full_c)::value;
    constexpr int NXT = (ST + 1) % NS;
    float4 na[4], nb[4];
    mfma4(fa[0], fb[0]);
    const bool more = FULL || t + 1 < nk;
    const bool load = FULL || t + 3 < nk;
    pin();
    if (more) {
      if (FULL || t + 2 < nk) wait_vmcnt<LPW>();
      else wait_vmcnt<0>();
      __syncthreads();
    }
    const float a1[4] = {fa[1].x, fa[1].y, fa[1].z, fa[1].w}, b1[4] = {fb[1].x, fb[1].y, fb[1].z, fb[1].w};
    const float a2[4] = {fa[2].x, fa[2].y, fa[2].z, fa[2].w}, b2[4] = {fb[2].x, fb[2].y, fb[2].z, fb[2].w};
#pragma unroll
    for (int q = 0; q < 4; ++q) {
      if (more) {
        na[q] = *reinterpret_cast<const float4*>(lds + NXT * STAGE + offa[q]);
        nb[q] = *reinterpret_cast<const float4*>(lds + NXT * STAGE + offb[q]);
      }
      pin();
      mfma(a1[q], b1[q]);
      pin();
    }
#pragma unroll
    for (int q = 0; q < 4; ++q) {
      if (more && load) {
#pragma unroll
        for (int j = q; j < LPW; j += 4) issue_one(ST, j);
      }
      pin();
      mfma(a2[q], b2[q]);
      pin();
    }
    if (more && load) advance();
    mfma4(fa[3], fb[3]);
    if (more) {
#pragma unroll
      for (int q = 0; q < 4; ++q) fa[q] = na[q], fb[q] = nb[q];
    }
  };
  using I0 = std::integral_constant<int, 0>;
  using I1 = std::integral_constant<int, 1>;
  using I2 = std::integral_constant<int, 2>;
  int t = 0;
  for (; t + 6 <= nk; t += 3) {
    step(I0{}, std::true_type{}, t);
    step(I1{}, std::true_type{}, t + 1);
    step(I2{}, std::true_type{}, t + 2);
  }
  for (; t < nk; t += 3) {
    step(I0{}, std::false_type{}, t);
    if (t + 1 < nk) step(I1{}, std::false_type{}, t + 1);
    if (t + 2 < nk) step(I2{}, std::false_type{}, t + 2);
  }

  floatx16 accs[1] = {acc};
  gemm_epilogue<BM, BN, WM, WN, 1>(accs, C, M, N, m0, n0, m_tile, ep, bias_v, blk_first, blk_seg_start, blk_seg_end, wm, wn, lane);
}

template <int BM, int BN, int WM, int WN>
static int launch_gemm_deep(const float* A, const float* B, float* C, int64_t M, int N, int K, const GemmEpilogue& ep, hipStream_t st,
                            const uint16_t* amask = nullptr, int kshift = 0) {
  const int mt8 = (div_up(M, BM) + 7) / 8 * 8;
  if (amask)
    LCR_LAUNCH_TIMED((k_gemm_f32_deep<BM, BN, WM, WN, true>), dim3(mt8 * div_up(N, BN)), dim3(GM_T), 0, st, A, B, C, M, N, K, ep, amask, kshift);
  else
    LCR_LAUNCH_TIMED((k_gemm_f32_deep<BM, BN, WM, WN>), dim3(mt8 * div_up(N, BN)), dim3(GM_T), 0, st, A, B, C, M, N, K, ep, amask, kshift);
  return check_launch("lcr_gemm_f32");
}

typedef __bf16 bf16x8_t __attribute__((ext_vector_type(8)));
typedef __bf16 bf16x2_t __attribute__((ext_vector_type(2)));
typedef float f32x2_t __attribute__((ext_vector_type(2)));
typedef float f32x4_t __attribute__((ext_vector_type(4)));
typedef uint32_t u32x4_t __attribute__((ext_vector_type(4)));

__device__ __forceinline__ uint32_t pk_bf16(float a, float b) {
  f32x2_t v = {a, b};
  return __builtin_bit_cast(uint32_t, __builtin_convertvector(v, bf16x2_t));
}
__device__ __forceinline__ void split2(float x0, float x1, uint32_t& h1, uint32_t& h2, uint32_t& h3) {
  h1 = pk_bf16(x0, x1);
  const float r0 = fsub(x0, __uint_as_float(h1 << 16)), r1 = fsub(x1, __uint_as_float(h1 & 0xffff0000u));
  h2 = pk_bf16(r0, r1);
  const float s0 = fsub(r0, __uint_as_float(h2 << 16)), s1 = fsub(r1, __uint_as_float(h2 & 0xffff0000u));
  h3 = pk_bf16(s0, s1);
}

__global__ __launch_bounds__(256) void k_split_bf16x3(const float* __restrict__ w, int64_t n, uint16_t* __restrict__ planes) {
  for (int64_t i = (blockIdx.x * static_cast<int64_t>(blockDim.x) + threadIdx.x) * 2; i < n; i += static_cast<int64_t>(gridDim.x) * blockDim.x * 2) {
    const float x0 = w[i], x1 = i + 1 < n ? w[i + 1] : 0.f;
    uint32_t h1, h2, h3;
    split2(x0, x1, h1, h2, h3);
    planes[i] = static_cast<uint16_t>(h1), planes[n + i] = static_cast<uint16_t>(h2), planes[2 * n + i] = static_cast<uint16_t>(h3);
    if (i + 1 < n) planes[i + 1] = static_cast<uint16_t>(h1 >> 16), planes[n + i + 1] = static_cast<uint16_t>(h2 >> 16), planes[2 * n + i + 1] = static_cast<uint16_t>(h3 >> 16);
  }
}

__global__ __launch_bounds__(256) void k_split_bf16x3_tiles(const float* __restrict__ w, int N, int K, uint16_t* __restrict__ tiles) {
  const int KS = K / GM_BK;
  const int64_t blk = blockIdx.x;
  const int ct = static_cast<int>(blk / KS), ks = static_cast<int>(blk % KS);
  const int row = threadIdx.x >> 2, kc = threadIdx.x & 3;
  const int n = ct * 64 + row;
  u32x4_t p1 = {0u, 0u, 0u, 0u}, p2 = p1, p3 = p1;
  if (n < N) {
    const float* src = w + static_cast<int64_t>(n) * K + ks * GM_BK + kc * 8;
    const float4 x0 = ld4(src), x1 = ld4(src + 4);
    uint32_t h1, h2, h3;
    split2(x0.x, x0.y, h1, h2, h3), p1.x = h1, p2.x = h2, p3.x = h3;
    split2(x0.z, x0.w, h1, h2, h3), p1.y = h1, p2.y = h2, p3.y = h3;
    split2(x1.x, x1.y, h1, h2, h3), p1.z = h1, p2.z = h2, p3.z = h3;
    split2(x1.z, x1.w, h1, h2, h3), p1.w = h1, p2.w = h2, p3.w = h3;
  }
  char* dst = reinterpret_cast<char*>(tiles) + blk * 12288 + row * 64 + ((kc ^ ((row >> 2) & 3)) << 4);
  *reinterpret_cast<u32x4_t*>(dst) = p1;
  *reinterpret_cast<u32x4_t*>(dst + 4096) = p2;
  *reinterpret_cast<u32x4_t*>(dst + 8192) = p3;
}

template <int ABL, int NWM, int D = 2, bool MASK = false>
__global__ __launch_bounds__(128 * NWM, 2) void k_gemm_f32_bsplit_p(const float* __restrict__ A, const uint16_t* __restrict__ Bs, float* __restrict__ C,
                                                             int64_t M, int N, int K, GemmEpilogue ep, const uint16_t* __restrict__ amask,
                                                             int kshift) {
  constexpr int BM = 32 * NWM, BN = 64, RS = 64, T = 128 * NWM, PLA = BM * RS, STGA = 3 * PLA, PL = 64 * RS;
  constexpr int NPB = (768 + T - 1) / T;
  constexpr int STG = 3 * PL + (NPB * T - 768) * 16;
  __shared__ __attribute__((aligned(16))) char sA[2 * STGA];
  __shared__ __attribute__((aligned(16))) char sB[2 * STG];
  const int lane = threadIdx.x & 63, w = __builtin_amdgcn_readfirstlane(threadIdx.x >> 6);
  const int wm = w >> 1, wn = w & 1;
  const int ntn = (N + BN - 1) / BN;
  const int xcd = blockIdx.x & 7, slot = blockIdx.x >> 3;
  const int64_t m_tile = static_cast<int64_t>(slot / ntn) * 8 + xcd;
  const int64_t m0 = m_tile * BM;
  const int n0 = (slot % ntn) * BN;
  if (m0 >= M) return;
  const int srow = threadIdx.x >> 3, spc = threadIdx.x & 7;
  const float* ap[2];
  int soff[2];
  uint32_t aoff[2], rmask[2];
#pragma unroll
  for (int j = 0; j < 2; ++j) {
    const int r = srow + j * (T / 8);
    int64_t ga = m0 + r;
    ga = ga < M ? ga : M - 1;
    ap[j] = A + ga * K + spc * 4;
    if constexpr (MASK) {
      aoff[j] = static_cast<uint32_t>((ga * K + spc * 4) * 4);
      rmask[j] = amask[ga];
    } else {
      aoff[j] = rmask[j] = 0;
    }
    soff[j] = r * RS + (((spc >> 1) ^ ((r >> 2) & 3)) << 4) + (spc & 1) * 8;
  }
  const char* bp = reinterpret_cast<const char*>(Bs) + static_cast<int64_t>(n0 / 64) * (K / GM_BK) * 12288;
  int bsrc[NPB], bdst[NPB];
#pragma unroll
  for (int j = 0; j < NPB; ++j) {
    const int q = threadIdx.x + T * j;
// ... 137 lines not shown
      step(I0{}, I0{}, t);
      step(I1{}, I1{}, t + 1);
    }
    if (t < nk) step(I0{}, I0{}, t);
  } else {
    for (; t + 4 <= nk; t += 4) {
      step(I0{}, I0{}, t);
      step(I1{}, I1{}, t + 1);
      step(I0{}, I2{}, t + 2);
      step(I1{}, I3{}, t + 3);
    }
    if (t < nk) step(I0{}, I0{}, t);
    if (t + 1 < nk) step(I1{}, I1{}, t + 1);
    if (t + 2 < nk) step(I0{}, I2{}, t + 2);
  }
#pragma unroll
  for (int r = 0; r < 16; ++r) acc[r] += acc2[r];
  floatx16 accs[1] = {acc};
  gemm_epilogue<BM, BN, NWM, 2, 1>(accs, C, M, N, m0, n0, m_tile, ep, bias_v, blk_first, blk_seg_start, blk_seg_end, wm, wn, lane);
}

struct GemmStreamK {
  float*    partial;
  uint32_t* arrived;
  int       U;
};

template <int BM, int BN, int WM, int WN>
__global__ __launch_bounds__(GM_T, 3) void k_gemm_f32_sk(const float* __restrict__ A, const float* __restrict__ B, float* __restrict__ C,
                                                         int64_t M, int N, int K, GemmEpilogue ep, GemmStreamK sk) {
  static_assert(WM * WN == 4 && BM == 32 * WM, "one 32-row MFMA tile per wavefront along M");
  constexpr int LDA = BM + 1, LDB = BN + 4;
  constexpr int NT = BN / (32 * WN);
  __shared__ __attribute__((aligned(16))) float As[2][GM_BK * LDA];
  __shared__ __attribute__((aligned(16))) float Bs[2][GM_BK * LDB];
  const int lane = threadIdx.x & 63, w = __builtin_amdgcn_readfirstlane(threadIdx.x >> 6);
  const int wm = w / WN, wn = w % WN;
  const int ntn = (N + BN - 1) / BN;
  const int64_t mt = (M + BM - 1) / BM;
  const int xcd = blockIdx.x & 7, u = blockIdx.x >> 3;
  const int64_t mt_x = mt > xcd ? (mt - xcd + 7) / 8 : 0;
  const int nk = (K + GM_BK - 1) / GM_BK;
  const int64_t I = mt_x * ntn * nk;
  auto first_it = [&](int uu) { return static_cast<int64_t>(uu) * I / sk.U; };
  const int64_t it_begin = first_it(u), it_end = first_it(u + 1);
  LoaderT<BM, LDA, true> la[2];
  LoaderN<BN, LDB, true> lb[2];
  const int a_off = (lane >> 5) * LDA + wm * 32 + (lane & 31);
  const int b_off = (lane >> 5) * LDB + wn * (32 * NT) + (lane & 31);
  constexpr int PIECE = NT * 16 * GM_T;
  __shared__ unsigned s_arrived;

  int64_t it = it_begin;
  while (it < it_end) {
    const int64_t lt = it / nk;
    const int ks = static_cast<int>(it - lt * nk);
    const int ns = static_cast<int>(min(static_cast<int64_t>(nk - ks), it_end - it));
    const int64_t m_tile = (lt / ntn) * 8 + xcd;
    const int64_t m0 = m_tile * BM;
    const int n0 = static_cast<int>(lt % ntn) * BN;
    const int k_begin = ks * GM_BK;
    auto gload = [&](int k0, int r) {
      la[r].load(A, M, K, m0, k0);
      lb[r].load(B, N, K, n0, k0);
    };
    floatx16 acc[NT];
#pragma unroll
    for (int j = 0; j < NT; ++j)
#pragma unroll
      for (int r = 0; r < 16; ++r) acc[j][r] = 0.f;
    gload(k_begin, 0);
    gload(k_begin + GM_BK, 1);
    const bool covers_end = ks + ns == nk, covers_start = ks == 0;
    float bias_v[NT];
#pragma unroll
    for (int j = 0; j < NT; ++j) {
      const int col = n0 + wn * (32 * NT) + j * 32 + (lane & 31);
      bias_v[j] = (ep.bias && col < N) ? ep.bias[col] : 0.f;
    }
    int blk_first = 0;
    int64_t blk_seg_start = 0, blk_seg_end = 0;
    la[0].store(As[0]);
    lb[0].store(Bs[0]);
    __syncthreads();

    constexpr int KK = GM_BK / 2;
    constexpr int PF = NT == 1 ? KK : (NT == 2 ? 8 : 4);
    constexpr int PA = BM * 8 / GM_T, PB = BN * 8 / GM_T;
    constexpr int ST0 = KK - (PA + PB) - 1 > 2 ? (KK - (PA + PB)) / 2 : 1;
    auto step = [&](auto buf_c, auto full_c, int t) {
      constexpr int BUF = decltype(buf_c)::value;
      constexpr bool FULL = decltype(full_c)::value;
      if (FULL || t + 2 < ns) gload(k_begin + (t + 2) * GM_BK, BUF);
      const bool do_store = FULL || t + 1 < ns;
      const float* as = As[BUF] + a_off;
      const float* bs = Bs[BUF] + b_off;
      float af[PF], bf[PF][NT];
#pragma unroll
      for (int d = 0; d < PF; ++d) {
        af[d] = as[d * 2 * LDA];
#pragma unroll
        for (int j = 0; j < NT; ++j) bf[d][j] = bs[d * 2 * LDB + j * 32];
      }
      __builtin_amdgcn_sched_barrier(0);
#pragma unroll
      for (int kk = 0; kk < KK; ++kk) {
        const int sl = kk % PF;
#pragma unroll
        for (int j = 0; j < NT; ++j) acc[j] = __builtin_amdgcn_mfma_f32_32x32x2f32(af[sl], bf[sl][j], acc[j], 0, 0, 0);
        if (kk + PF < KK) {
          af[sl] = as[(kk + PF) * 2 * LDA];
#pragma unroll
          for (int j = 0; j < NT; ++j) bf[sl][j] = bs[(kk + PF) * 2 * LDB + j * 32];
        }
        const int piece = kk - ST0;
        if (do_store && piece >= 0 && piece < PA + PB) {
          if (piece < PA) la[1 - BUF].store_piece(As[1 - BUF], piece);
          else lb[1 - BUF].store_piece(Bs[1 - BUF], piece - PA);
        }
      }
      __syncthreads();
    };
    int t = 0;
    for (; t + 3 < ns; t += 2) {
      step(std::integral_constant<int, 0>{}, std::true_type{}, t);
      step(std::integral_constant<int, 1>{}, std::true_type{}, t + 1);
    }
    for (; t < ns; t += 2) {
      step(std::integral_constant<int, 0>{}, std::false_type{}, t);
      if (t + 1 >= ns) break;
      step(std::integral_constant<int, 1>{}, std::false_type{}, t + 1);
    }

    bool finish = true;
    if (!(covers_start && covers_end)) {
      float* mine = sk.partial + (static_cast<int64_t>(blockIdx.x) * 2 + (it == it_begin ? 0 : 1)) * PIECE;
#pragma unroll
      for (int j = 0; j < NT; ++j)
#pragma unroll
        for (int r = 0; r < 16; ++r)
          __hip_atomic_store(&mine[(j * 16 + r) * GM_T + threadIdx.x], acc[j][r], __ATOMIC_RELAXED, __HIP_MEMORY_SCOPE_AGENT);
      const int64_t tile_it0 = lt * nk, tile_it1 = tile_it0 + nk;
      int uf = static_cast<int>(tile_it0 * sk.U / I);
      while (uf > 0 && first_it(uf) > tile_it0) --uf;
      while (first_it(uf + 1) <= tile_it0) ++uf;
      int ul = uf, pieces = 0;
      for (int uu = uf; uu < sk.U && first_it(uu) < tile_it1; ++uu)
        if (first_it(uu + 1) > first_it(uu)) {
          ul = uu;
          ++pieces;
        }
      __builtin_amdgcn_s_waitcnt(0);
      __builtin_amdgcn_fence(__ATOMIC_RELEASE, "workgroup");
      __syncthreads();
      uint32_t* cnt = sk.arrived + (m_tile * ntn + lt % ntn);
      if (threadIdx.x == 0) s_arrived = __hip_atomic_fetch_add(cnt, 1u, __ATOMIC_RELAXED, __HIP_MEMORY_SCOPE_AGENT);
      __syncthreads();
      finish = s_arrived == static_cast<unsigned>(pieces - 1);
      if (finish) {
        __builtin_amdgcn_fence(__ATOMIC_ACQUIRE, "workgroup");
#pragma unroll
        for (int j = 0; j < NT; ++j)
#pragma unroll
          for (int r = 0; r < 16; ++r) acc[j][r] = 0.f;
        for (int uu = uf; uu <= ul; ++uu) {
          if (first_it(uu + 1) <= first_it(uu)) continue;
          const float* pp = sk.partial + (static_cast<int64_t>(uu * 8 + xcd) * 2 + (first_it(uu) >= tile_it0 ? 0 : 1)) * PIECE;
#pragma unroll
          for (int j = 0; j < NT; ++j)
#pragma unroll
            for (int r = 0; r < 16; ++r)
              acc[j][r] += __hip_atomic_load(&pp[(j * 16 + r) * GM_T + threadIdx.x], __ATOMIC_RELAXED, __HIP_MEMORY_SCOPE_AGENT);
        }
        if (threadIdx.x == 0) __hip_atomic_store(cnt, 0u, __ATOMIC_RELAXED, __HIP_MEMORY_SCOPE_AGENT);
      }
    }
    if (finish) {
      if (ep.stats != nullptr) {
        blk_first = 0;
        blk_seg_start = 0;
        blk_seg_end = ep.seg_len[0];
        while (blk_first + 1 < ep.S && m0 >= blk_seg_end) {
          ++blk_first;
          blk_seg_start = blk_seg_end;
          blk_seg_end += ep.seg_len[blk_first];
        }
      }
      gemm_epilogue<BM, BN, WM, WN, NT>(acc, C, M, N, m0, n0, m_tile, ep, bias_v, blk_first, blk_seg_start, blk_seg_end, wm, wn, lane);
    }
    it += ns;
    __syncthreads();
  }
}

template <int BM, int BN, int WM, int WN, bool VEC, bool SHORT = false>
static int launch_gemm(const float* A, const float* B, float* C, int64_t M, int N, int K, int transA, int transB, const GemmEpilogue& ep,
                       hipStream_t st, const GemmBatch* batch = nullptr) {
  static const GemmBatch no_batch = {};
  const GemmBatch& bt = batch ? *batch : no_batch;
  const int mt8 = (div_up(M, BM) + 7) / 8 * 8;
  dim3 grid(mt8 * div_up(N, BN), 1, bt.count ? bt.count : 1);
  dim3 block(GM_T);
  if (!transA && !transB) LCR_LAUNCH_TIMED((k_gemm_f32<BM, BN, WM, WN, false, false, VEC, SHORT>), grid, block, 0, st, A, B, C, M, N, K, ep, bt, ANorm{});
  else if (!transA && transB) LCR_LAUNCH_TIMED((k_gemm_f32<BM, BN, WM, WN, false, true, VEC, SHORT>), grid, block, 0, st, A, B, C, M, N, K, ep, bt, ANorm{});
  else if (transA && !transB) LCR_LAUNCH_TIMED((k_gemm_f32<BM, BN, WM, WN, true, false, VEC, SHORT>), grid, block, 0, st, A, B, C, M, N, K, ep, bt, ANorm{});
  else LCR_LAUNCH_TIMED((k_gemm_f32<BM, BN, WM, WN, true, true, VEC, SHORT>), grid, block, 0, st, A, B, C, M, N, K, ep, bt, ANorm{});
  return check_launch("lcr_gemm_f32");
}

struct SkScratch {
  float*    partial = nullptr;
  uint32_t* arrived = nullptr;
};
static std::mutex g_sk_mu;
static std::map<std::pair<int, hipStream_t>, SkScratch> g_sk_scratch;
constexpr int SK_MAX_GRID = 1024;
constexpr int SK_MAX_TILES = 8192;

static int sk_cu_count() {
  static const int n = [] {
    int dev = 0, cus = 0;
    hipGetDevice(&dev);
    if (hipDeviceGetAttribute(&cus, hipDeviceAttributeMultiprocessorCount, dev) != hipSuccess || cus <= 0) cus = 256;
    return cus;
  }();
  return n;
}

static bool sk_worth(int64_t M, int N, int K) {
  const int cus = sk_cu_count();
  const int64_t tiles = static_cast<int64_t>(div_up(M, 64)) * div_up(N, 64);
  if (K < 480 || tiles < cus / 2 || tiles > 6 * static_cast<int64_t>(cus) || tiles > SK_MAX_TILES) return false;
  const double avg = static_cast<double>(tiles) / cus;
  const double worst = static_cast<double>((tiles + cus - 1) / cus);
  return worst / avg >= 1.10;
}

static int launch_gemm_sk(const float* A, const float* B, float* C, int64_t M, int N, int K, const GemmEpilogue& ep, hipStream_t st) {
  const int cus = sk_cu_count();
  const int64_t iters = static_cast<int64_t>(div_up(M, 64)) * div_up(N, 64) * div_up(K, GM_BK);
  int per_cu = 3;
  while (per_cu > 1 && iters / (static_cast<int64_t>(cus) * per_cu) < 24) --per_cu;
  if (getenv("LCR_SK_PER_CU")) per_cu = atoi(getenv("LCR_SK_PER_CU"));
  int U = cus * per_cu / 8;
  if (U < 1) U = 1;
  if (8 * U > SK_MAX_GRID) U = SK_MAX_GRID / 8;
  int dev = 0;
  hipGetDevice(&dev);
  GemmStreamK sk;
  {
    std::lock_guard<std::mutex> lk(g_sk_mu);
    SkScratch& sc = g_sk_scratch[{dev, st}];
    if (!sc.partial) {
      if (hipMalloc(reinterpret_cast<void**>(&sc.partial), sizeof(float) * 2 * 16 * GM_T * SK_MAX_GRID) != hipSuccess ||
          hipMalloc(reinterpret_cast<void**>(&sc.arrived), sizeof(uint32_t) * SK_MAX_TILES) != hipSuccess) {
        set_error("lcr_gemm_f32: cannot allocate the stream-K scratch");
        return LCR_EHIP;
      }
      hipMemsetAsync(sc.arrived, 0, sizeof(uint32_t) * SK_MAX_TILES, st);
    }
    sk.partial = sc.partial;
    sk.arrived = sc.arrived;
    sk.U = U;
  }
  LCR_LAUNCH_TIMED((k_gemm_f32_sk<64, 64, 2, 2>), dim3(8 * U), dim3(GM_T), 0, st, A, B, C, M, N, K, ep, sk);
  return check_launch("lcr_gemm_f32");
}

}

using namespace lcr;

static int g_force_tile = 0;
extern "C" void lcr_gemm_debug_force_tile(int t) { g_force_tile = t; }
static int g_force_streamk = -1;
static int g_force_deep = -1;
extern "C" void lcr_gemm_debug_deep(int mode) { g_force_deep = mode; }
extern "C" void lcr_gemm_debug_streamk(int mode) { g_force_streamk = mode; }

static int gemm_impl(const float* A, const float* B, float* C, int64_t M, int N, int K, int transA, int transB, const float* bias,
                     const float* rowdiv, const int64_t* seg_len, int S, int groups, double* stats, void* stream);

static int env_int(const char* name, int unset) { return getenv(name) ? atoi(getenv(name)) : unset; }
enum GemmForm { GF_SCALAR, GF_FORCED_TILE, GF_SHORT, GF_DEEP, GF_STREAMK, GF_TILE };
static GemmForm gemm_form(int64_t M, int N, int K, int transA, int transB, bool vec) {
  static const bool no_short = getenv("LCR_GEMM_NO_SHORT") != nullptr;
  static const int short_k = env_int("LCR_GEMM_SHORT_K", 256);
  static const int deep_env = env_int("LCR_GEMM_DEEP", 1);
  static const int sk_env = env_int("LCR_GEMM_STREAMK", 0);
  if (!vec) return GF_SCALAR;
  if (g_force_tile >= 1 && g_force_tile <= 5) return GF_FORCED_TILE;
  const int deep_mode = g_force_deep >= 0 ? g_force_deep : deep_env;
  const bool deep_ok = !transA && transB && K % GM_BK == 0 && !g_force_tile && M * K < (int64_t(1) << 30) && static_cast<int64_t>(N) * K < (int64_t(1) << 30);
  if (deep_mode == 2 && deep_ok) return GF_DEEP;
  if (!no_short && K <= short_k && !transA) return GF_SHORT;
  if (deep_mode && deep_ok) return GF_DEEP;
  if (N <= 32) return GF_TILE;
  const int sk_mode = g_force_streamk >= 0 ? g_force_streamk : sk_env;
  const bool sk_legal = !transA && !transB && K >= 64 && static_cast<int64_t>(div_up(M, 64)) * div_up(N, 64) <= SK_MAX_TILES;
  if (sk_mode && sk_legal && (sk_mode == 2 || sk_worth(M, N, K))) return GF_STREAMK;
  return GF_TILE;
}

extern "C" int lcr_gemm_f32_anorm(const float* A, const float* B, float* C, int64_t M, int N, int K, const float* bias,
                                  const double* a_stats, const float* a_gamma, const float* a_beta, int a_groups, float a_eps,
                                  float a_slope, const int64_t* seg_len, int S, int groups, double* stats, void* stream) {
  if (!A || !B || !C || M < 0 || N <= 32 || K <= 0 || K > AN_KMAX || K % 4 != 0 || !a_stats || !a_gamma || !a_beta || a_groups < 1 ||
      K % a_groups != 0 || a_groups > 64 || !seg_len || S < 1 || reinterpret_cast<uintptr_t>(A) % 16 != 0 || reinterpret_cast<uintptr_t>(B) % 16 != 0) {
    set_error("lcr_gemm_f32_anorm: needs 32 < N, K <= 256, K % 4 == 0, a_groups dividing K, a segment table and 16-byte aligned operands");
    return LCR_EARG;
  }
  if (stats) {
    const int gs = groups >= 1 && N % groups == 0 ? N / groups : 3;
    if ((gs & (gs - 1)) != 0) {
      set_error("lcr_gemm_f32_anorm: statistics need groups dividing N into power-of-two sized groups");
      return LCR_EARG;
    }
  }
  hipStream_t st = static_cast<hipStream_t>(stream);
  KernelTimerScope timed(KT_GEMM, st, M, N, K);
  if (M == 0) return LCR_OK;
  GemmEpilogue ep{bias, nullptr, seg_len, S, groups, stats};
  ANorm an{a_stats, a_gamma, a_beta, a_groups, a_eps, a_slope};
  const int mt8 = (div_up(M, 64) + 7) / 8 * 8;
  LCR_LAUNCH_TIMED((k_gemm_f32<64, 64, 2, 2, false, true, true, true, true>), dim3(mt8 * div_up(N, 64)), dim3(GM_T), 0, st, A, B, C, M,
                     N, K, ep, GemmBatch{}, an);
  return check_launch("lcr_gemm_f32_anorm");
}

extern "C" int lcr_gemm_f32(const float* A, const float* B, float* C, int64_t M, int N, int K, int transA, int transB, const float* bias,
                            const float* rowdiv, const int64_t* seg_len, int S, int groups, double* stats, void* stream) {
  return gemm_impl(A, B, C, M, N, K, transA, transB, bias, rowdiv, seg_len, S, groups, stats, stream);
}

static int gemm_impl(const float* A, const float* B, float* C, int64_t M, int N, int K, int transA, int transB, const float* bias,
                     const float* rowdiv, const int64_t* seg_len, int S, int groups, double* stats, void* stream) {
  if (!A || !B || !C || M < 0 || N <= 0 || K <= 0) {
    set_error("lcr_gemm_f32: bad argument");
    return LCR_EARG;
  }
  if (stats && (!seg_len || S < 1 || groups < 1 || N % groups != 0)) {
    set_error("lcr_gemm_f32: statistics need seg_len, S >= 1 and groups dividing N");
    return LCR_EARG;
  }
  if (stats) {
    const int gs = N / groups;
    if ((gs & (gs - 1)) != 0) {
      set_error("lcr_gemm_f32: channels per group must be a power of two");
      return LCR_EARG;
    }
  }
  hipStream_t st = static_cast<hipStream_t>(stream);
  KernelTimerScope timed(KT_GEMM, st, M, N, K);
  if (M == 0) return LCR_OK;
  GemmEpilogue ep{bias, rowdiv, seg_len, S, groups, stats};
  const int64_t lda = transA ? M : K, ldb = transB ? K : N;
  const bool vec = (lda % 4 == 0) && (ldb % 4 == 0) && (reinterpret_cast<uintptr_t>(A) % 16 == 0) && (reinterpret_cast<uintptr_t>(B) % 16 == 0);
  switch (gemm_form(M, N, K, transA, transB, vec)) {
    case GF_SCALAR: return launch_gemm<128, 64, 4, 1, false>(A, B, C, M, N, K, transA, transB, ep, st);
    case GF_FORCED_TILE:
      switch (g_force_tile) {
        case 1: return launch_gemm<128, 128, 4, 1, true>(A, B, C, M, N, K, transA, transB, ep, st);
        case 2: return launch_gemm<128, 64, 4, 1, true>(A, B, C, M, N, K, transA, transB, ep, st);
        case 3: return launch_gemm<128, 32, 4, 1, true>(A, B, C, M, N, K, transA, transB, ep, st);
        case 4: return launch_gemm<64, 64, 2, 2, true>(A, B, C, M, N, K, transA, transB, ep, st);
        default: return launch_gemm<64, 128, 2, 2, true>(A, B, C, M, N, K, transA, transB, ep, st);
      }
    case GF_SHORT:
      if (N <= 32) return launch_gemm<128, 32, 4, 1, true, true>(A, B, C, M, N, K, transA, transB, ep, st);
      return launch_gemm<64, 64, 2, 2, true, true>(A, B, C, M, N, K, transA, transB, ep, st);
    case GF_DEEP:
      if (N <= 32) return launch_gemm_deep<128, 32, 4, 1>(A, B, C, M, N, K, ep, st);
      return launch_gemm_deep<64, 64, 2, 2>(A, B, C, M, N, K, ep, st);
    case GF_STREAMK: return launch_gemm_sk(A, B, C, M, N, K, ep, st);
    case GF_TILE: break;
  }
  if (N <= 32) return launch_gemm<128, 32, 4, 1, true>(A, B, C, M, N, K, transA, transB, ep, st);
  const int64_t b128 = (M + 127) / 128, nb128 = (N + 127) / 128;
  if (K >= 512 && b128 * nb128 >= 512) return launch_gemm<128, 128, 4, 1, true>(A, B, C, M, N, K, transA, transB, ep, st);
  return launch_gemm<64, 64, 2, 2, true>(A, B, C, M, N, K, transA, transB, ep, st);
}

extern "C" int lcr_split_bf16x3(const float* w, int64_t n, uint16_t* planes, void* stream) {
  if (!w || !planes || n < 0) {
    set_error("lcr_split_bf16x3: bad argument");
    return LCR_EARG;
  }
  if (n == 0) return LCR_OK;
  hipLaunchKernelGGL(k_split_bf16x3, dim3(min(div_up(n, 512), 2048)), dim3(256), 0, static_cast<hipStream_t>(stream), w, n, planes);
  return check_launch("lcr_split_bf16x3");
}

extern "C" int lcr_split_bf16x3_tiles(const float* w, int N, int K, uint16_t* tiles, void* stream) {
  if (!w || !tiles || N < 1 || K < GM_BK || K % GM_BK != 0 || reinterpret_cast<uintptr_t>(w) % 16 != 0 || reinterpret_cast<uintptr_t>(tiles) % 16 != 0) {
    set_error("lcr_split_bf16x3_tiles: needs K %% 32 == 0 and 16-byte aligned buffers");
    return LCR_EARG;
  }
  hipLaunchKernelGGL(k_split_bf16x3_tiles, dim3(div_up(N, 64) * (K / GM_BK)), dim3(256), 0, static_cast<hipStream_t>(stream), w, N, K, tiles);
  return check_launch("lcr_split_bf16x3_tiles");
}

static int bsplit_impl(const float* A, const uint16_t* Bs, float* C, int64_t M, int N, int K, const float* bias, const float* rowdiv,
                       const int64_t* seg_len, int S, int groups, double* stats, const uint16_t* amask, int kshift, void* stream) {
  if (!A || !Bs || !C || M < 0 || N <= 0 || K <= 0 || K % GM_BK != 0 || reinterpret_cast<uintptr_t>(A) % 16 != 0 || reinterpret_cast<uintptr_t>(Bs) % 16 != 0 ||
      K < GM_BK) {
    set_error("lcr_gemm_f32_bsplit: needs K %% 32 == 0 and 16-byte aligned operands");
    return LCR_EARG;
  }
  if (stats && (!seg_len || S < 1 || groups < 1 || N % groups != 0 || ((N / groups) & (N / groups - 1)) != 0)) {
    set_error("lcr_gemm_f32_bsplit: statistics need seg_len, S >= 1 and groups dividing N into power-of-two sized groups");
    return LCR_EARG;
  }
  hipStream_t st = static_cast<hipStream_t>(stream);
  KernelTimerScope timed(KT_GEMM, st, M, N, K);
  if (M == 0) return LCR_OK;
  GemmEpilogue ep{bias, rowdiv, seg_len, S, groups, stats};
  const int mt8 = (div_up(M, 64) + 7) / 8 * 8;
  static const int abl = getenv("LCR_SPLIT_ABL") ? atoi(getenv("LCR_SPLIT_ABL")) : 0;
  const dim3 grid(mt8 * div_up(N, 64)), block(256);
  if (amask) {
    LCR_LAUNCH_TIMED((k_gemm_f32_bsplit_p<0, 2, 2, true>), grid, block, 0, st, A, Bs, C, M, N, K, ep, amask, kshift);
    return check_launch("lcr_gemm_f32_bsplit_masked");
  }
  switch (abl) {
    case 1: LCR_LAUNCH_TIMED((k_gemm_f32_bsplit_p<1, 2>), grid, block, 0, st, A, Bs, C, M, N, K, ep, amask, kshift); break;
    case 2: LCR_LAUNCH_TIMED((k_gemm_f32_bsplit_p<2, 2>), grid, block, 0, st, A, Bs, C, M, N, K, ep, amask, kshift); break;
    case 4: LCR_LAUNCH_TIMED((k_gemm_f32_bsplit_p<4, 2>), grid, block, 0, st, A, Bs, C, M, N, K, ep, amask, kshift); break;
    case 8: LCR_LAUNCH_TIMED((k_gemm_f32_bsplit_p<8, 2>), grid, block, 0, st, A, Bs, C, M, N, K, ep, amask, kshift); break;
    case 16: LCR_LAUNCH_TIMED((k_gemm_f32_bsplit_p<16, 2>), grid, block, 0, st, A, Bs, C, M, N, K, ep, amask, kshift); break;
    case 23: LCR_LAUNCH_TIMED((k_gemm_f32_bsplit_p<23, 2>), grid, block, 0, st, A, Bs, C, M, N, K, ep, amask, kshift); break;
    case 30: LCR_LAUNCH_TIMED((k_gemm_f32_bsplit_p<30, 2>), grid, block, 0, st, A, Bs, C, M, N, K, ep, amask, kshift); break;
    default: LCR_LAUNCH_TIMED((k_gemm_f32_bsplit_p<0, 2>), grid, block, 0, st, A, Bs, C, M, N, K, ep, amask, kshift); break;
  }
  return check_launch("lcr_gemm_f32_bsplit");
}

extern "C" int lcr_gemm_f32_bsplit(const float* A, const uint16_t* Bs, float* C, int64_t M, int N, int K, const float* bias, const float* rowdiv,
                                   const int64_t* seg_len, int S, int groups, double* stats, void* stream) {
  return bsplit_impl(A, Bs, C, M, N, K, bias, rowdiv, seg_len, S, groups, stats, nullptr, 0, stream);
}

static int mask_kshift(int K, int block_k) {
  for (int s = 0; s <= 3; ++s)
    if (block_k == (GM_BK << s)) return K <= 16 * block_k ? s : -1;
  return -1;
}

extern "C" int lcr_gemm_f32_bsplit_masked(const float* A, const uint16_t* Bs, float* C, int64_t M, int N, int K, const float* bias,
                                          const float* rowdiv, const int64_t* seg_len, int S, int groups, double* stats, const uint16_t* row_mask,
                                          int block_k, void* stream) {
  const int ks = mask_kshift(K, block_k);
  if (!row_mask || ks < 0 || M * static_cast<int64_t>(K) >= (int64_t(1) << 29)) {
    set_error("lcr_gemm_f32_bsplit_masked: needs a row mask, block_k = 32 << s (s <= 3) with K <= 16 block_k, and M*K < 2^29");
    return LCR_EARG;
  }
  return bsplit_impl(A, Bs, C, M, N, K, bias, rowdiv, seg_len, S, groups, stats, row_mask, ks, stream);
}

extern "C" int lcr_kpconv_mask_ok(int64_t M, int N, int K, int split) {
  static const bool off = getenv("LCR_KP_MASK") && atoi(getenv("LCR_KP_MASK")) == 0;
  if (off || M <= 0 || N <= 0 || K % 15 != 0 || mask_kshift(K, K / 15) < 0) return 0;
  if (split) return M * static_cast<int64_t>(K) < (int64_t(1) << 29);
  return gemm_form(M, N, K, 0, 1, true) == GF_DEEP;
}

extern "C" int lcr_gemm_f32_masked(const float* A, const float* B, float* C, int64_t M, int N, int K, const float* bias, const float* rowdiv,
                                   const int64_t* seg_len, int S, int groups, double* stats, const uint16_t* row_mask, int block_k, void* stream) {
  const int ks = mask_kshift(K, block_k);
  if (!A || !B || !C || !row_mask || M < 0 || N <= 0 || K <= 0 || K % GM_BK != 0 || ks < 0 || M * static_cast<int64_t>(K) >= (int64_t(1) << 30) ||
      static_cast<int64_t>(N) * K >= (int64_t(1) << 30) || reinterpret_cast<uintptr_t>(A) % 16 != 0 || reinterpret_cast<uintptr_t>(B) % 16 != 0) {
    set_error("lcr_gemm_f32_masked: needs a row mask, block_k = 32 << s (s <= 3) with K <= 16 block_k, K %% 32 == 0, M*K and N*K < 2^30, "
              "16-byte aligned operands");
    return LCR_EARG;
  }
  if (stats && (!seg_len || S < 1 || groups < 1 || N % groups != 0 || ((N / groups) & (N / groups - 1)) != 0)) {
    set_error("lcr_gemm_f32_masked: statistics need seg_len, S >= 1 and groups dividing N into power-of-two sized groups");
    return LCR_EARG;
  }
  hipStream_t st = static_cast<hipStream_t>(stream);
  KernelTimerScope timed(KT_GEMM, st, M, N, K);
  if (M == 0) return LCR_OK;
  GemmEpilogue ep{bias, rowdiv, seg_len, S, groups, stats};
  if (N <= 32) return launch_gemm_deep<128, 32, 4, 1>(A, B, C, M, N, K, ep, st, row_mask, ks);
  return launch_gemm_deep<64, 64, 2, 2>(A, B, C, M, N, K, ep, st, row_mask, ks);
}

extern "C" int lcr_gemm_f32_batched_ta(const float* A, const float* B, float* C, int64_t M, int N, int count, const int* k_host,
                                       const int64_t* a_off_host, const int64_t* b_off_host, const int64_t* c_off_host, void* stream) {
  if (!A || !B || !C || M <= 0 || N <= 0 || count < 1 || count > GM_MAX_BATCH || !k_host || !a_off_host || !b_off_host || !c_off_host) {
    set_error("lcr_gemm_f32_batched_ta: bad argument (count <= %d)", GM_MAX_BATCH);
    return LCR_EARG;
  }
  GemmBatch bt = {};
  bt.count = count;
  for (int i = 0; i < count; ++i) {
    bt.k[i] = k_host[i];
    bt.a_off[i] = a_off_host[i];
    bt.b_off[i] = b_off_host[i];
    bt.c_off[i] = c_off_host[i];
    if (a_off_host[i] % 4 || b_off_host[i] % 4 || k_host[i] < 1) {
      set_error("lcr_gemm_f32_batched_ta: offsets must be multiples of 4 floats and K >= 1");
      return LCR_EARG;
    }
  }
  if ((M % 4) || (N % 4)) {
    set_error("lcr_gemm_f32_batched_ta: M and N must be multiples of 4");
    return LCR_EARG;
  }
  GemmEpilogue ep{nullptr, nullptr, nullptr, 0, 0, nullptr};
  return launch_gemm<64, 64, 2, 2, true>(A, B, C, M, N,  1, 1, 0, ep, static_cast<hipStream_t>(stream), &bt);
}

extern "C" int lcr_gemm_f32_strided_batched(const float* A, const float* B, float* C, int64_t M, int N, int K, int transA, int transB,
                                            int64_t strideA, int64_t strideB, int64_t strideC, int count, void* stream) {
  if (!A || !B || !C || M <= 0 || N <= 0 || K <= 0 || count < 1 || count > 65535 || (strideA % 4) || (strideB % 4)) {
    set_error("lcr_gemm_f32_strided_batched: bad argument");
    return LCR_EARG;
  }
  const int64_t lda = transA ? M : K, ldb = transB ? K : N;
  if ((lda % 4) || (ldb % 4)) {
    set_error("lcr_gemm_f32_strided_batched: leading dimensions must be multiples of 4");
    return LCR_EARG;
  }
  GemmBatch bt = {};
  bt.count = count;
  bt.strided = 1;
  bt.k[0] = K;
  bt.a_off[0] = strideA;
  bt.b_off[0] = strideB;
  bt.c_off[0] = strideC;
  GemmEpilogue ep{nullptr, nullptr, nullptr, 0, 0, nullptr};
  static const int batch_tile = env_int("LCR_GEMM_BATCH_TILE", 64);
  if (batch_tile == 128 && M >= 128 && N >= 128) return launch_gemm<128, 128, 4, 1, true>(A, B, C, M, N, K, transA, transB, ep, static_cast<hipStream_t>(stream), &bt);
  static const bool batch_short = env_int("LCR_GEMM_BATCH_SHORT", 1) != 0;
  if (batch_short && K <= 256 && !transA) return launch_gemm<64, 64, 2, 2, true, true>(A, B, C, M, N, K, transA, transB, ep, static_cast<hipStream_t>(stream), &bt);
  return launch_gemm<64, 64, 2, 2, true>(A, B, C, M, N, K, transA, transB, ep, static_cast<hipStream_t>(stream), &bt);
}
```

lcr-net_amd/functional.py:

```python
import ctypes
import os
import threading

import numpy as np
import torch

from . import _lib

GN_EPS = 1e-5
GN_REPLICAS = 8


class KernelTimer:
    KINDS = {"gemm": 0, "kpconv_aggregate": 1, "radius_query": 2, "attention": 3, "kpconv_fused": 4, "sinkhorn": 5}

    def __init__(self, names):
        self.names = set(names)
        self._cache = None

    def summary(self):
        return {k: [(b, m) for b, _, m in v] for k, v in self.records().items()}

    def records(self):
        if self._cache is None:
            out = {}
            L = _lib.lib()
            for name in self.names:
                kind = self.KINDS[name]
                n = L.lcr_ktimer_read2(kind, 0, None, None, None)
                sec = (ctypes.c_double * max(n, 1))()
                ksec = (ctypes.c_double * max(n, 1))()
                meta = (ctypes.c_int64 * (5 * max(n, 1)))()
                L.lcr_ktimer_read2(kind, n, ctypes.cast(sec, ctypes.c_void_p), ctypes.cast(ksec, ctypes.c_void_p), ctypes.cast(meta, ctypes.c_void_p))
                width = 3 if name == "gemm" else 5
                out[name] = [(sec[i], ksec[i] if ksec[i] >= 0 else None, tuple(int(meta[5 * i + k]) for k in range(width))) for i in range(n)]
            self._cache = out
        return self._cache


def set_timer(timer, sample_every=1):
    _lib.lib().lcr_ktimer_sample(int(sample_every))
    mask = 0
    for name in (timer.names if timer is not None else ()):
        mask |= 1 << KernelTimer.KINDS[name]
    _lib.lib().lcr_ktimer_kinds(mask if timer is not None else 0xffffffff)
    _lib.lib().lcr_ktimer_enable(1 if timer is not None else 0)


def _timed(name, fn, meta=None):
    return fn()


def _seg(seg_len, n, device):
    if seg_len is None:
        return torch.full((1,), int(n), dtype=torch.int64, device=device)
    return seg_len


def host_values(values, dtype, device):
    return torch.tensor(values, dtype=dtype).pin_memory().to(device, non_blocking=True)


def host_tensor(t, device):
    if not torch.is_tensor(t):
        t = torch.from_numpy(t)
    return t.pin_memory().to(device, non_blocking=True)


def _idx_args(idx):
    if idx.dtype == torch.int64:
        return 1
    if idx.dtype == torch.int32:
        return 0
    raise RuntimeError("neighbor indices must be int32 or int64")


class _StatsArena(threading.local):
    buf = None
    off = 0


_ARENA = _StatsArena()


class stats_arena:

    def __init__(self, device, entries=1 << 18):
        self.device, self.entries = device, entries

    def __enter__(self):
        self.prev = (_ARENA.buf, _ARENA.off)
        _ARENA.buf = torch.zeros(self.entries, dtype=torch.float64, device=self.device)
        _ARENA.off = 0
        return self

    def __exit__(self, *exc):
        _ARENA.buf, _ARENA.off = self.prev
        return False


def _zero_stats(S, groups, device):
    n = GN_REPLICAS * S * groups * 2
    buf = _ARENA.buf
    if buf is not None and buf.device == device and _ARENA.off + n <= buf.numel():
        v = buf[_ARENA.off:_ARENA.off + n].view(GN_REPLICAS, S, groups, 2)
        _ARENA.off += n
        return v
    return torch.zeros((GN_REPLICAS, S, groups, 2), dtype=torch.float64, device=device)


def gemm(a, b, trans_b=False, trans_a=False, bias=None, rowdiv=None, seg_len=None, groups=0, row_mask=None):
    if row_mask is not None:
        return _gemm_masked(a, b, trans_b, trans_a, bias, rowdiv, seg_len, groups, row_mask)
    _lib.require_cuda(a, b)
    assert a.dtype == torch.float32 and b.dtype == torch.float32 and a.is_contiguous() and b.is_contiguous()
    M, K = (a.shape[1], a.shape[0]) if trans_a else (a.shape[0], a.shape[1])
    N = b.shape[0] if trans_b else b.shape[1]
    assert (b.shape[1] if trans_b else b.shape[0]) == K, "inner dimensions differ"
    c = torch.empty((M, N), dtype=torch.float32, device=a.device)
    stats = None
    S = 0
    if groups:
        seg_len = _seg(seg_len, M, a.device)
        S = seg_len.numel()
        stats = _zero_stats(S, groups, a.device)
    _timed("gemm", lambda: _lib.check(_lib.lib().lcr_gemm_f32(
        _lib.ptr(a), _lib.ptr(b), _lib.ptr(c), M, N, K, int(trans_a), int(trans_b), _lib.ptr(bias), _lib.ptr(rowdiv),
        _lib.ptr(seg_len) if groups else None, S, int(groups), _lib.ptr(stats), _lib.stream_ptr(a.device)), "lcr_gemm_f32"),
        meta=(M, N, K))
    return c, stats


def kpconv_mask_ok(M, N, K, split):
    return bool(_lib.lib().lcr_kpconv_mask_ok(int(M), int(N), int(K), int(bool(split))))


def _mask_args(a, row_mask):
    M, K = a.shape
    assert row_mask.dtype == torch.int16 and row_mask.is_contiguous() and row_mask.numel() == M and row_mask.device == a.device
    assert K % 15 == 0
    return K // 15


def _gemm_masked(a, b, trans_b, trans_a, bias, rowdiv, seg_len, groups, row_mask):
    _lib.require_cuda(a, b)
    assert trans_b and not trans_a, "the masked form takes A [M,K] and B [N,K]"
    assert a.dtype == torch.float32 and b.dtype == torch.float32 and a.is_contiguous() and b.is_contiguous()
    block_k = _mask_args(a, row_mask)
    M, K = a.shape
    N = b.shape[0]
    assert b.shape[1] == K, "inner dimensions differ"
    c = torch.empty((M, N), dtype=torch.float32, device=a.device)
    stats, S = None, 0
    if groups:
        seg_len = _seg(seg_len, M, a.device)
        S = seg_len.numel()
        stats = _zero_stats(S, groups, a.device)
    _timed("gemm", lambda: _lib.check(_lib.lib().lcr_gemm_f32_masked(
        _lib.ptr(a), _lib.ptr(b), _lib.ptr(c), M, N, K, _lib.ptr(bias), _lib.ptr(rowdiv), _lib.ptr(seg_len) if groups else None, S,
        int(groups), _lib.ptr(stats), _lib.ptr(row_mask), block_k, _lib.stream_ptr(a.device)), "lcr_gemm_f32_masked"), meta=(M, N, K))
    return c, stats


_GEMM_SPLIT = [os.environ.get("LCR_GEMM_SPLIT", "1") not in ("", "0")]


def gemm_split_enabled():
    return _GEMM_SPLIT[0]


def set_gemm_split(on):
    _GEMM_SPLIT[0] = bool(on)


def gemm_split_ok(N, K):
    return K >= 288 and K % 32 == 0 and N >= 64


derived_lock = threading.RLock()


class WeightStamp:
    __slots__ = ("ref", "ptr", "ver", "dev")

    def __init__(self, t):
        import weakref
        self.ref, self.ptr, self.ver, self.dev = weakref.ref(t), t.data_ptr(), t._version, t.device

    def same(self, t):
        return self.ref is not None and self.ref() is t and self.ptr == t.data_ptr() and self.ver == t._version and self.dev == t.device

    def __reduce__(self):
        return (_dead_stamp, ())


def _dead_stamp():
    s = WeightStamp.__new__(WeightStamp)
    s.ref, s.ptr, s.ver, s.dev = None, 0, -1, None
    return s


def drop_derived(module, *names):
    for n in names:
        if n in module.__dict__:
            module.__dict__[n] = None



def publish_derived(t):
    torch.cuda.current_stream(t.device).synchronize()
    return t


def split_bf16x3(w):
    w = w.detach().contiguous()
    N, K = w.shape
    assert K % 32 == 0
    tiles = torch.empty(((N + 63) // 64, K // 32, 3, 64, 32), dtype=torch.int16, device=w.device)
    _lib.check(_lib.lib().lcr_split_bf16x3_tiles(_lib.ptr(w), int(N), int(K), _lib.ptr(tiles), _lib.stream_ptr(w.device)), "lcr_split_bf16x3_tiles")
    tiles.lcr_n = int(N)
    return tiles


def unsplit_bf16x3(tiles):
    CT, KS = tiles.shape[0], tiles.shape[1]
    t = tiles.view(CT, KS, 3, 64, 4, 8)
    row = torch.arange(64, device=tiles.device)
    phys = torch.arange(4, device=tiles.device)[None, :] ^ ((row >> 2) & 3)[:, None]
    t = torch.gather(t, 4, phys.view(1, 1, 1, 64, 4, 1).expand(CT, KS, 3, 64, 4, 8))
    t = t.reshape(CT, KS, 3, 64, 32).permute(2, 0, 3, 1, 4).reshape(3, CT * 64, KS * 32)
    return t[:, :tiles.lcr_n].contiguous().view(torch.bfloat16).float()


def gemm_bsplit(a, planes, bias=None, rowdiv=None, seg_len=None, groups=0, row_mask=None):
    _lib.require_cuda(a, planes)
    assert a.dtype == torch.float32 and a.is_contiguous() and planes.dtype == torch.int16 and planes.is_contiguous() and planes.dim() == 5
    M, K = a.shape
    N = planes.lcr_n
    assert planes.shape[1] * 32 == K and planes.shape[0] == (N + 63) // 64, "inner dimensions differ"
    c = torch.empty((M, N), dtype=torch.float32, device=a.device)
    stats, S = None, 0
    if groups:
        seg_len = _seg(seg_len, M, a.device)
        S = seg_len.numel()
        stats = _zero_stats(S, groups, a.device)
    if row_mask is not None:
        block_k = _mask_args(a, row_mask)
        _lib.check(_lib.lib().lcr_gemm_f32_bsplit_masked(_lib.ptr(a), _lib.ptr(planes), _lib.ptr(c), M, N, K, _lib.ptr(bias), _lib.ptr(rowdiv),
                                                         _lib.ptr(seg_len) if groups else None, S, int(groups), _lib.ptr(stats),
                                                         _lib.ptr(row_mask), block_k, _lib.stream_ptr(a.device)), "lcr_gemm_f32_bsplit_masked")
        return c, stats
    _lib.check(_lib.lib().lcr_gemm_f32_bsplit(_lib.ptr(a), _lib.ptr(planes), _lib.ptr(c), M, N, K, _lib.ptr(bias), _lib.ptr(rowdiv),
                                              _lib.ptr(seg_len) if groups else None, S, int(groups), _lib.ptr(stats), _lib.stream_ptr(a.device)),
               "lcr_gemm_f32_bsplit")
    return c, stats


ANORM_MAX_K, ANORM_MIN_SEG_ROWS = 256, 64


def gemm_anorm_ok(K, N):
    return K <= ANORM_MAX_K and K % 4 == 0 and N > 32


def gemm_anorm(a, a_stats, a_gamma, a_beta, a_groups, weight, bias=None, seg_len=None, groups=0, slope=0.1):
    _lib.require_cuda(a, weight)
    assert a.dtype == torch.float32 and weight.dtype == torch.float32 and a.is_contiguous() and weight.is_contiguous()
    M, K = a.shape
    N = weight.shape[0]
    assert weight.shape[1] == K and gemm_anorm_ok(K, N)
    c = torch.empty((M, N), dtype=torch.float32, device=a.device)
    seg_len = _seg(seg_len, M, a.device)
    S = seg_len.numel()
    stats = _zero_stats(S, groups, a.device) if groups else None
    _timed("gemm", lambda: _lib.check(_lib.lib().lcr_gemm_f32_anorm(
        _lib.ptr(a), _lib.ptr(weight), _lib.ptr(c), M, N, K, _lib.ptr(bias), _lib.ptr(a_stats), _lib.ptr(a_gamma), _lib.ptr(a_beta),
        int(a_groups), GN_EPS, float(slope), _lib.ptr(seg_len), S, int(groups), _lib.ptr(stats), _lib.stream_ptr(a.device)),
        "lcr_gemm_f32_anorm"), meta=(M, N, K))
    return c, stats


def groupnorm_stats(x, groups, seg_len=None):
    seg_len = _seg(seg_len, x.shape[0], x.device)
    stats = _zero_stats(seg_len.numel(), groups, x.device)
    _lib.check(_lib.lib().lcr_groupnorm_stats(_lib.ptr(x), x.shape[0], x.shape[1], groups, _lib.ptr(seg_len), seg_len.numel(),
                                              _lib.ptr(stats), _lib.stream_ptr(x.device)), "lcr_groupnorm_stats")
    return stats


def groupnorm_apply(x, stats, gamma, beta, groups, seg_len=None, res=None, res_norm=None, slope=0.1, act=True, want_pos=False):
    seg_len = _seg(seg_len, x.shape[0], x.device)
    y = torch.empty_like(x)
    pos = torch.empty((x.shape[0],), dtype=torch.uint8, device=x.device) if want_pos else None
    rs, rg, rb = res_norm if res_norm is not None else (None, None, None)
    _lib.check(_lib.lib().lcr_groupnorm_apply(_lib.ptr(x), _lib.ptr(stats), _lib.ptr(gamma), _lib.ptr(beta), _lib.ptr(res), _lib.ptr(rs),
                                              _lib.ptr(rg), _lib.ptr(rb), _lib.ptr(y), x.shape[0], x.shape[1], groups, _lib.ptr(seg_len),
                                              seg_len.numel(), GN_EPS, float(slope), int(act), _lib.ptr(pos),
                                              _lib.stream_ptr(x.device)), "lcr_groupnorm_apply")
    return (y, pos) if want_pos else y


def row_positive(x):
    pos = torch.empty((x.shape[0],), dtype=torch.uint8, device=x.device)
    _lib.check(_lib.lib().lcr_row_positive(_lib.ptr(x), x.shape[0], x.shape[1], _lib.ptr(pos), _lib.stream_ptr(x.device)), "lcr_row_positive")
    return pos


def _kp_host(kernel_points):
    kp = np.ascontiguousarray(kernel_points, dtype=np.float32)
    assert kp.shape == (15, 3)
    return kp


def kpconv_aggregate(s_feats, s_pos, q_points, s_points, idx, kernel_points_host, sigma, order=None, emit_mask=False):
    _lib.require_cuda(s_feats, q_points, s_points, idx)
    M, H = idx.shape
    Ns, C = s_feats.shape
    assert idx.is_contiguous() and s_feats.is_contiguous() and q_points.is_contiguous() and s_points.is_contiguous()
    A = torch.empty((M, 15 * C), dtype=torch.float32, device=s_feats.device)
    nn = torch.empty((M,), dtype=torch.float32, device=s_feats.device)
    kp = _kp_host(kernel_points_host)
    if emit_mask:
        mask = torch.empty((M,), dtype=torch.int16, device=s_feats.device)
        _timed("kpconv_aggregate", lambda: _lib.check(_lib.lib().lcr_kpconv_aggregate_mask(
            _lib.ptr(s_feats), _lib.ptr(s_pos), _lib.ptr(q_points), _lib.ptr(s_points), _lib.ptr(idx), _idx_args(idx), M, Ns, H, C,
            ctypes.c_void_p(kp.ctypes.data), float(sigma), _lib.ptr(A), _lib.ptr(nn), _lib.ptr(mask), _lib.ptr(order), 0,
            _lib.stream_ptr(s_feats.device)), "lcr_kpconv_aggregate_mask"), meta=(M, Ns, H, C, idx.element_size()))
        return A, nn, mask
    _timed("kpconv_aggregate", lambda: _lib.check(_lib.lib().lcr_kpconv_aggregate(
        _lib.ptr(s_feats), _lib.ptr(s_pos), _lib.ptr(q_points), _lib.ptr(s_points), _lib.ptr(idx), _idx_args(idx), M, Ns, H, C,
        ctypes.c_void_p(kp.ctypes.data), float(sigma), _lib.ptr(A), _lib.ptr(nn), _lib.ptr(order), _lib.stream_ptr(s_feats.device)),
        "lcr_kpconv_aggregate"), meta=(M, Ns, H, C, idx.element_size()))
    return A, nn


KPCONV_FUSED_C = 32


def kpconv_fused(s_feats, s_pos, q_points, s_points, idx, kernel_points_host, sigma, weights, bias, seg_len=None, groups=0, order=None):
    _lib.require_cuda(s_feats, q_points, s_points, idx)
    M, H = idx.shape
    Ns, C = s_feats.shape
    assert C == KPCONV_FUSED_C and tuple(weights.shape) == (15, C, C) and weights.is_contiguous()
    assert idx.is_contiguous() and s_feats.is_contiguous() and q_points.is_contiguous() and s_points.is_contiguous()
    out = torch.empty((M, C), dtype=torch.float32, device=s_feats.device)
    stats, S = None, 0
    if groups:
        seg_len = _seg(seg_len, M, s_feats.device)
        S = seg_len.numel()
        stats = _zero_stats(S, groups, s_feats.device)
    kp = _kp_host(kernel_points_host)
    _timed("kpconv_fused", lambda: _lib.check(_lib.lib().lcr_kpconv_fused(
        _lib.ptr(s_feats), _lib.ptr(s_pos), _lib.ptr(q_points), _lib.ptr(s_points), _lib.ptr(idx), _idx_args(idx), M, Ns, H, C,
        ctypes.c_void_p(kp.ctypes.data), float(sigma), _lib.ptr(weights), _lib.ptr(bias), _lib.ptr(out),
        _lib.ptr(seg_len) if groups else None, S, int(groups), _lib.ptr(stats), _lib.ptr(order), _lib.stream_ptr(s_feats.device)),
        "lcr_kpconv_fused"), meta=(M, Ns, H, C, idx.element_size()))
    return out, stats


def kpconv_cin1(s_feats, q_points, s_points, idx, kernel_points_host, sigma, weights, bias, order=None):
    M, H = idx.shape
    Ns = s_feats.shape[0]
    Cout = weights.shape[-1]
    out = torch.empty((M, Cout), dtype=torch.float32, device=s_feats.device)
    kp = _kp_host(kernel_points_host)
    _lib.check(_lib.lib().lcr_kpconv_cin1(_lib.ptr(s_feats), _lib.ptr(q_points), _lib.ptr(s_points), _lib.ptr(idx), _idx_args(idx), M, Ns, H,
                                          ctypes.c_void_p(kp.ctypes.data), float(sigma), _lib.ptr(weights), _lib.ptr(bias), Cout,
                                          _lib.ptr(out), _lib.ptr(order), _lib.stream_ptr(s_feats.device)), "lcr_kpconv_cin1")
    return out


def maxpool(x, idx, order=None):
    M, H = idx.shape
    out = torch.empty((M, x.shape[1]), dtype=torch.float32, device=x.device)
    _lib.check(_lib.lib().lcr_maxpool(_lib.ptr(x), _lib.ptr(idx), _idx_args(idx), M, x.shape[0], H, x.shape[1], _lib.ptr(out),
                                      _lib.ptr(order), _lib.stream_ptr(x.device)), "lcr_maxpool")
    return out


class NetvladWeights(ctypes.Structure):
    _fields_ = [(n, ctypes.c_void_p) for n in (
        "cluster_weights", "cluster_weights2", "hidden1_weights", "bn1_w", "bn1_b", "bn1_mean", "bn1_var",
        "bn2_w", "bn2_b", "bn2_mean", "bn2_var", "gating_weights", "gbn_w", "gbn_b", "gbn_mean", "gbn_var")]


def netvlad_forward(feats, seg_len_host, weights_struct):
    _lib.require_cuda(feats)
    seg = np.ascontiguousarray(seg_len_host, dtype=np.int64)
    S = int(seg.shape[0])
    assert int(seg.sum()) == feats.shape[0] and feats.shape[1] == 1024 and feats.is_contiguous()
    nbytes = ctypes.c_size_t(0)
    _lib.check(_lib.lib().lcr_netvlad_ws_bytes(feats.shape[0], S, ctypes.byref(nbytes)), "lcr_netvlad_ws_bytes")
    ws = _lib.workspace(nbytes.value, feats.device)
    out = torch.empty((S, 256), dtype=torch.float32, device=feats.device)
    _lib.check(_lib.lib().lcr_netvlad_forward(_lib.ptr(feats), ctypes.c_void_p(seg.ctypes.data), S, ctypes.byref(weights_struct),
                                              _lib.ptr(out), _lib.ptr(ws), ws.numel(), _lib.stream_ptr(feats.device)),
               "lcr_netvlad_forward")
    return out


def gemm_batched_ta(a, b, c, M, N, k, a_off, b_off, c_off):
    _lib.require_cuda(a, b, c)
    assert all(t.dtype == torch.float32 and t.is_contiguous() for t in (a, b, c))
    kk = np.ascontiguousarray(k, dtype=np.int32)
    ao, bo, co = (np.ascontiguousarray(v, dtype=np.int64) for v in (a_off, b_off, c_off))
    count = int(kk.shape[0])
    assert ao.shape == bo.shape == co.shape == (count,)
    for i in range(count):
        assert 0 <= ao[i] and ao[i] + max(int(kk[i]), 0) * M <= a.numel(), "A entry out of range"
        assert 0 <= bo[i] and bo[i] + max(int(kk[i]), 0) * N <= b.numel(), "B entry out of range"
        assert 0 <= co[i] and co[i] + M * N <= c.numel(), "C entry out of range"
    _lib.check(_lib.lib().lcr_gemm_f32_batched_ta(_lib.ptr(a), _lib.ptr(b), _lib.ptr(c), int(M), int(N), count, ctypes.c_void_p(kk.ctypes.data),
                                                  ctypes.c_void_p(ao.ctypes.data), ctypes.c_void_p(bo.ctypes.data),
                                                  ctypes.c_void_p(co.ctypes.data), _lib.stream_ptr(a.device)), "lcr_gemm_f32_batched_ta")
    return c


def linear(x, weight, bias=None, relu=False):
    y = gemm(x.contiguous(), weight, trans_b=True, bias=bias)[0]
    if relu:
        _lib.check(_lib.lib().lcr_relu_inplace(_lib.ptr(y), y.numel(), _lib.stream_ptr(y.device)), "lcr_relu_inplace")
    return y


def relu_(x):
    _lib.check(_lib.lib().lcr_relu_inplace(_lib.ptr(x), x.numel(), _lib.stream_ptr(x.device)), "lcr_relu_inplace")
    return x


def rotary_embed_(x, theta, heads):
    assert x.is_contiguous() and theta.is_contiguous() and x.shape[1] == heads * 32 and theta.shape[1] == heads * 16
    _lib.check(_lib.lib().lcr_rotary_embed(_lib.ptr(x), _lib.ptr(theta), x.shape[0], heads, _lib.stream_ptr(x.device)), "lcr_rotary_embed")
    return x


def attention(q, k, v, heads, q_lens=None, k_lens=None):
    assert q.is_contiguous() and k.is_contiguous() and v.is_contiguous()
    out = torch.empty_like(q)
    if q_lens is not None:
        P = len(q_lens)
        assert len(k_lens) == P and sum(q_lens) == q.shape[0] and sum(k_lens) == k.shape[0]
        ql, kl = (ctypes.c_int64 * P)(*[int(x) for x in q_lens]), (ctypes.c_int64 * P)(*[int(x) for x in k_lens])
        _lib.check(_lib.lib().lcr_attention_seg_f32(_lib.ptr(q), _lib.ptr(k), _lib.ptr(v), ctypes.cast(ql, ctypes.c_void_p),
                                                    ctypes.cast(kl, ctypes.c_void_p), P, heads, q.shape[1] // heads, _lib.ptr(out),
                                                    _lib.stream_ptr(q.device)), "lcr_attention_seg_f32")
        return out
    _lib.check(_lib.lib().lcr_attention_f32(_lib.ptr(q), _lib.ptr(k), _lib.ptr(v), q.shape[0], k.shape[0], heads, q.shape[1] // heads,
                                            _lib.ptr(out), _lib.stream_ptr(q.device)), "lcr_attention_f32")
    return out


ATTENTION_TOPK_MAX_KEYS = 4096


def attention_topk(q, k, v, heads, q_lens, k_lens, kks):
    assert q.is_contiguous() and k.is_contiguous() and v.is_contiguous()
    P = len(q_lens)
    assert len(k_lens) == P and len(kks) == P and sum(q_lens) == q.shape[0] and sum(k_lens) == k.shape[0]
    out = torch.empty_like(q)
    ql, kl = (ctypes.c_int64 * P)(*[int(x) for x in q_lens]), (ctypes.c_int64 * P)(*[int(x) for x in k_lens])
    kk = (ctypes.c_int * P)(*[int(x) for x in kks])
    _lib.check(_lib.lib().lcr_attention_topk_f32(_lib.ptr(q), _lib.ptr(k), _lib.ptr(v), ctypes.cast(ql, ctypes.c_void_p), ctypes.cast(kl, ctypes.c_void_p),
                                                 ctypes.cast(kk, ctypes.c_void_p), P, heads, q.shape[1] // heads, _lib.ptr(out), _lib.stream_ptr(q.device)),
               "lcr_attention_topk_f32")
    return out


def add_layernorm(a, b, gamma, beta, eps=1e-5):
    y = torch.empty_like(a)
    _lib.check(_lib.lib().lcr_add_layernorm(_lib.ptr(a), _lib.ptr(b), _lib.ptr(gamma), _lib.ptr(beta), a.shape[0], a.shape[1], float(eps),
                                            _lib.ptr(y), _lib.stream_ptr(a.device)), "lcr_add_layernorm")
    return y


def _L():
    return _lib.lib()


def _sp(t):
    return _lib.stream_ptr(t.device)


def vote_shift(xyz, offsets, max_range):
    out = torch.empty_like(xyz)
    _lib.check(_L().lcr_vote_shift(_lib.ptr(xyz.contiguous()), _lib.ptr(offsets.contiguous()), xyz.shape[0], float(max_range), _lib.ptr(out),
                                   _sp(xyz)), "lcr_vote_shift")
    return out


def greedy_nms(points, lengths, radius):
    n, B = points.shape[0], lengths.numel()
    keep = torch.empty((n,), dtype=torch.uint8, device=points.device)
    out_len = torch.empty((B,), dtype=torch.int64, device=points.device)
    nbytes = ctypes.c_size_t(0)
    _lib.check(_L().lcr_greedy_nms_ws_bytes(n, ctypes.byref(nbytes)), "lcr_greedy_nms_ws_bytes")
    ws = _lib.workspace(nbytes.value, points.device)
    _lib.check(_L().lcr_greedy_nms(_lib.ptr(points.contiguous()), _lib.ptr(lengths), B, n, float(radius), _lib.ptr(keep), _lib.ptr(out_len),
                                   _lib.ptr(ws), _sp(points)), "lcr_greedy_nms")
    return keep, out_len


def neighbor_mean(points, idx, pad):
    out = torch.empty((idx.shape[0], 3), dtype=torch.float32, device=points.device)
    _lib.check(_L().lcr_neighbor_mean(_lib.ptr(points.contiguous()), _lib.ptr(idx.contiguous()), _idx_args(idx), idx.shape[0], idx.shape[1], int(pad),
                                      _lib.ptr(out), _sp(points)), "lcr_neighbor_mean")
    return out


def point_to_node_partition(points, nodes, point_limit):
    N, M, dev = points.shape[0], nodes.shape[0], points.device
    nbytes = ctypes.c_size_t(0)
    _lib.check(_L().lcr_point_to_node_ws_bytes(N, M, ctypes.byref(nbytes)), "lcr_point_to_node_ws_bytes")
    ws = _lib.workspace(nbytes.value, dev)
    p2n = torch.empty((N,), dtype=torch.int32, device=dev)
    knn = torch.empty((M, point_limit), dtype=torch.int64, device=dev)
    km = torch.empty((M, point_limit), dtype=torch.uint8, device=dev)
    nm = torch.empty((M,), dtype=torch.uint8, device=dev)
    status = torch.zeros(1, dtype=torch.int32, device=dev)
    _lib.check(_L().lcr_point_to_node_partition(_lib.ptr(points.contiguous()), N, _lib.ptr(nodes.contiguous()), M, int(point_limit), _lib.ptr(p2n),
                                                _lib.ptr(knn), _lib.ptr(km), _lib.ptr(nm), _lib.ptr(status), _lib.ptr(ws), ws.numel(), _sp(points)),
               "lcr_point_to_node_partition")
    return p2n, nm.bool(), knn, km.bool()


def point_to_node_partition_stack(points, point_off, nodes, node_off, point_limit):
    import numpy as np
    C = len(point_off) - 1
    assert len(node_off) == C + 1 and C >= 1
    dev = points.device
    N, M = int(point_off[-1] - point_off[0]), int(node_off[-1] - node_off[0])
    po = np.ascontiguousarray(point_off, dtype=np.int64)
    mo = np.ascontiguousarray(node_off, dtype=np.int64)
    nbytes = ctypes.c_size_t(0)
    _lib.check(_L().lcr_point_to_node_ws_bytes(N, M, ctypes.byref(nbytes)), "lcr_point_to_node_ws_bytes")
    ws = _lib.workspace(nbytes.value, dev)
    p2n = torch.empty((N,), dtype=torch.int32, device=dev)
    knn = torch.empty((M, point_limit), dtype=torch.int64, device=dev)
    km = torch.empty((M, point_limit), dtype=torch.uint8, device=dev)
    nm = torch.empty((M,), dtype=torch.uint8, device=dev)
    status = torch.zeros(1, dtype=torch.int32, device=dev)
    _lib.check(_L().lcr_point_to_node_partition_stack(_lib.ptr(points.contiguous()), po.ctypes.data, _lib.ptr(nodes.contiguous()), mo.ctypes.data, C,
                                                      int(point_limit), _lib.ptr(p2n), _lib.ptr(knn), _lib.ptr(km), _lib.ptr(nm), _lib.ptr(status),
                                                      _lib.ptr(ws), ws.numel(), _sp(points)), "lcr_point_to_node_partition_stack")
    return p2n, nm.bool(), knn, km.bool()


class _PendingStatus(threading.local):
    def __init__(self):
        self.items = []


_pending_ot_status = _PendingStatus()
_PENDING_OT_MAX = 32


def check_transport_status():
    items, _pending_ot_status.items = _pending_ot_status.items, []
    if items and any(int(t.reshape(()).item()) != 0 for t in items):
        raise RuntimeError("lcr_log_sinkhorn: a workgroup hand-off of the persistent form timed out (set LCR_SINKHORN_COOP=0)")


def log_optimal_transport(raw_scores, row_masks, col_masks, alpha, scale=1.0, iters=100, inf=1e12):
    B, M, N = raw_scores.shape
    dev = raw_scores.device
    rm, cm = row_masks.to(torch.uint8).contiguous(), col_masks.to(torch.uint8).contiguous()
    S = torch.empty((B, M + 1, N + 1), dtype=torch.float32, device=dev)
    _lib.check(_L().lcr_build_padded_scores(_lib.ptr(raw_scores.contiguous()), _lib.ptr(rm), _lib.ptr(cm), B, M, N, float(scale),
                                            _lib.ptr(alpha.reshape(1).float()), float(inf), _lib.ptr(S), _sp(S)), "lcr_build_padded_scores")
    return _transport_padded(S, rm, cm, iters, inf)


PATCH_SCORES_FUSED = [os.environ.get("LCR_PATCH_SCORES_FUSED", "1") != "0"]


def patch_log_optimal_transport(feats_a, idx_a, feats_b, idx_b, mask_a, mask_b, alpha, scale=1.0, iters=100, inf=1e12):
    P, K = idx_a.shape
    if not PATCH_SCORES_FUSED[0] or K != 128 or feats_a.shape[1] % 32 != 0 or P == 0:
        fa, fb = gather_rows(feats_a, idx_a.contiguous()), gather_rows(feats_b, idx_b.contiguous())
        return log_optimal_transport(bmm_nt(fa, fb), mask_a, mask_b, alpha, scale=scale, iters=iters, inf=inf)
    dev = feats_a.device
    fa, fb = feats_a.contiguous(), feats_b.contiguous()
    ia, ib = idx_a.contiguous(), idx_b.contiguous()
# ... 338 lines not shown
```

lcr-net_amd/modules/kpconv/modules.py:

```python
import os

import torch
import torch.nn as nn

from ... import functional as F
from .kpconv import KPConv


class StageContext:

    def __init__(self, seg_len=None, order=None, min_rows=None):
        self.seg_len = seg_len
        self.order = order
        self.min_rows = min_rows

    def norm_on_load(self, K, N, M):
        if _NO_NORM_ON_LOAD or not F.gemm_anorm_ok(K, N):
            return False
        rows = M if self.seg_len is None else self.min_rows
        return rows is not None and rows >= F.ANORM_MIN_SEG_ROWS


_NO_NORM_ON_LOAD = bool(os.environ.get("LCR_NO_NORM_ON_LOAD"))
_WHOLE = StageContext(None)


class GroupNorm(nn.Module):
    def __init__(self, num_groups, num_channels):
        super().__init__()
        self.num_groups, self.num_channels = num_groups, num_channels
        self.norm = nn.GroupNorm(num_groups, num_channels)

    def forward(self, x, ctx=_WHOLE, act=False, slope=0.1):
        stats = F.groupnorm_stats(x.contiguous(), self.num_groups, ctx.seg_len)
        return F.groupnorm_apply(x.contiguous(), stats, self.norm.weight, self.norm.bias, self.num_groups, ctx.seg_len, act=act, slope=slope)


class UnaryBlock(nn.Module):
    def __init__(self, in_channels, out_channels, group_norm, has_relu=True, bias=True, layer_norm=False):
        super().__init__()
        assert not layer_norm, "layer_norm=True is not used by the reference configs"
        self.in_channels, self.out_channels, self.group_norm = in_channels, out_channels, group_norm
        self.mlp = nn.Linear(in_channels, out_channels, bias=bias)
        self.norm = GroupNorm(group_norm, out_channels)
        self.leaky_relu = nn.LeakyReLU(0.1) if has_relu else None

    def weight_split(self):
        w = self.mlp.weight
        c = getattr(self, "_ws_cache", None)
        if c is None or not c[0].same(w):
            with F.derived_lock:
                c = getattr(self, "_ws_cache", None)
                if c is None or not c[0].same(w):
                    c = self._ws_cache = (F.WeightStamp(w), F.publish_derived(F.split_bf16x3(w)))
        return c[1]

    def _apply(self, fn, *args, **kwargs):
        F.drop_derived(self, "_ws_cache")
        return super()._apply(fn, *args, **kwargs)

    def raw(self, x, ctx):
        if F.gemm_split_enabled() and F.gemm_split_ok(self.out_channels, self.in_channels):
            return F.gemm_bsplit(x.contiguous(), self.weight_split(), bias=self.mlp.bias, seg_len=ctx.seg_len, groups=self.group_norm)
        return F.gemm(x.contiguous(), self.mlp.weight, trans_b=True, bias=self.mlp.bias, seg_len=ctx.seg_len, groups=self.group_norm)

    def forward(self, x, ctx=_WHOLE, want_pos=False):
        y, stats = self.raw(x, ctx)
        return F.groupnorm_apply(y, stats, self.norm.norm.weight, self.norm.norm.bias, self.group_norm, ctx.seg_len,
                                 act=self.leaky_relu is not None, want_pos=want_pos)


class LastUnaryBlock(nn.Module):
    def __init__(self, in_channels, out_channels, bias=True):
        super().__init__()
        self.mlp = nn.Linear(in_channels, out_channels, bias=bias)

    def forward(self, x):
        w = self.mlp.weight
        if F.gemm_split_enabled() and F.gemm_split_ok(w.shape[0], w.shape[1]):
            c = getattr(self, "_ws_cache", None)
            if c is None or not c[0].same(w):
                with F.derived_lock:
                    c = getattr(self, "_ws_cache", None)
                    if c is None or not c[0].same(w):
                        c = self._ws_cache = (F.WeightStamp(w), F.publish_derived(F.split_bf16x3(w)))
            return F.gemm_bsplit(x.contiguous(), c[1], bias=self.mlp.bias)[0]
        return F.gemm(x.contiguous(), w, trans_b=True, bias=self.mlp.bias)[0]

    def _apply(self, fn, *args, **kwargs):
        F.drop_derived(self, "_ws_cache")
        return super()._apply(fn, *args, **kwargs)


class ConvBlock(nn.Module):
    def __init__(self, in_channels, out_channels, kernel_size, radius, sigma, group_norm, negative_slope=0.1, bias=True, layer_norm=False):
        super().__init__()
        assert not layer_norm
        self.in_channels, self.out_channels, self.group_norm = in_channels, out_channels, group_norm
        self.KPConv = KPConv(in_channels, out_channels, kernel_size, radius, sigma, bias=bias)
        self.norm = GroupNorm(group_norm, out_channels)
        self.leaky_relu = nn.LeakyReLU(negative_slope=negative_slope)
        self.negative_slope = negative_slope

    def forward(self, s_feats, q_points, s_points, neighbor_indices, q_ctx=_WHOLE, s_ctx=_WHOLE):
        x, stats = self.KPConv.forward_raw(s_feats, q_points, s_points, neighbor_indices, seg_len=q_ctx.seg_len, groups=self.group_norm,
                                           order=q_ctx.order)
        return F.groupnorm_apply(x, stats, self.norm.norm.weight, self.norm.norm.bias, self.group_norm, q_ctx.seg_len,
                                 act=True, slope=self.negative_slope)


class ResidualBlock(nn.Module):
    def __init__(self, in_channels, out_channels, kernel_size, radius, sigma, group_norm, strided=False, bias=True, layer_norm=False):
        super().__init__()
        assert not layer_norm
        self.in_channels, self.out_channels, self.strided, self.group_norm = in_channels, out_channels, strided, group_norm
        mid = out_channels // 4
        self.unary1 = UnaryBlock(in_channels, mid, group_norm, bias=bias) if in_channels != mid else nn.Identity()
        self.KPConv = KPConv(mid, mid, kernel_size, radius, sigma, bias=bias)
        self.norm_conv = GroupNorm(group_norm, mid)
        self.unary2 = UnaryBlock(mid, out_channels, group_norm, has_relu=False, bias=bias)
        self.unary_shortcut = (UnaryBlock(in_channels, out_channels, group_norm, has_relu=False, bias=bias)
                               if in_channels != out_channels else nn.Identity())
        self.leaky_relu = nn.LeakyReLU(0.1)

    def forward(self, s_feats, q_points, s_points, neighbor_indices, q_ctx=_WHOLE, s_ctx=_WHOLE):
        g = self.group_norm
        s_feats = s_feats.contiguous()
        if isinstance(self.unary1, nn.Identity):
            x, pos = s_feats, None
        else:
            x, pos = self.unary1(s_feats, s_ctx, want_pos=True)
        x, stats = self.KPConv.forward_raw(x, q_points, s_points, neighbor_indices, s_pos=pos, seg_len=q_ctx.seg_len, groups=g,
                                           order=q_ctx.order)
        if q_ctx.norm_on_load(x.shape[1], self.out_channels, x.shape[0]):
            y, ystats = F.gemm_anorm(x, stats, self.norm_conv.norm.weight, self.norm_conv.norm.bias, g, self.unary2.mlp.weight,
                                     bias=self.unary2.mlp.bias, seg_len=q_ctx.seg_len, groups=g)
        else:
            x = F.groupnorm_apply(x, stats, self.norm_conv.norm.weight, self.norm_conv.norm.bias, g, q_ctx.seg_len, act=True)
            y, ystats = self.unary2.raw(x, q_ctx)
        shortcut = F.maxpool(s_feats, neighbor_indices, order=q_ctx.order) if self.strided else s_feats
        if isinstance(self.unary_shortcut, nn.Identity):
            res, res_norm = shortcut, None
        else:
            res, rstats = self.unary_shortcut.raw(shortcut, q_ctx)
            res_norm = (rstats, self.unary_shortcut.norm.norm.weight, self.unary_shortcut.norm.norm.bias)
        return F.groupnorm_apply(y, ystats, self.unary2.norm.norm.weight, self.unary2.norm.norm.bias, g, q_ctx.seg_len,
                                 res=res, res_norm=res_norm, act=True, slope=0.1)
```

lcr-net_amd/native_encoder.py:

```python
import ctypes

import numpy as np
import torch

from . import _lib

ENC_BLOCKS = 10
_BLOCK_NAMES = ["encoder1_2", "encoder2_1", "encoder2_2", "encoder2_3", "encoder3_1", "encoder3_2", "encoder3_3", "encoder4_1", "encoder4_2",
                "encoder4_3"]
_fp = ctypes.c_void_p


class UnaryW(ctypes.Structure):
    _fields_ = [("w", _fp), ("b", _fp), ("gn_w", _fp), ("gn_b", _fp), ("w_split", _fp)]


class BlockW(ctypes.Structure):
    _fields_ = [("cin", ctypes.c_int), ("cout", ctypes.c_int), ("strided", ctypes.c_int), ("sigma", ctypes.c_float),
                ("kernel_points_host", _fp), ("kp_w", _fp), ("kp_b", _fp), ("kp_wt", _fp), ("kp_wt_split", _fp), ("normconv_w", _fp),
                ("normconv_b", _fp),
                ("unary1", UnaryW), ("unary2", UnaryW), ("shortcut", UnaryW)]


class EncoderW(ctypes.Structure):
    _fields_ = [("groups", ctypes.c_int), ("c1_cout", ctypes.c_int), ("c1_sigma", ctypes.c_float), ("c1_kernel_points_host", _fp),
                ("c1_w", _fp), ("c1_b", _fp), ("c1_gn_w", _fp), ("c1_gn_b", _fp), ("blocks", BlockW * ENC_BLOCKS)]


def _p(t):
    return None if t is None else ctypes.c_void_p(t.data_ptr())


def _unary(u, keep):
    import torch.nn as nn
    if isinstance(u, nn.Identity):
        return UnaryW(None, None, None, None, None)
    from . import functional as F
    sp = None
    if F.gemm_split_enabled() and F.gemm_split_ok(u.mlp.weight.shape[0], u.mlp.weight.shape[1]):
        sp = F.split_bf16x3(u.mlp.weight)
        keep.append(sp)
    return UnaryW(_p(u.mlp.weight), _p(u.mlp.bias), _p(u.norm.norm.weight), _p(u.norm.norm.bias), _p(sp))


class EncoderTable:

    def __init__(self, enc):
        self.keep = []
        w = EncoderW()
        c1 = enc.encoder1_1
        w.groups, w.c1_cout, w.c1_sigma = int(c1.group_norm), int(c1.out_channels), float(c1.KPConv.sigma)
        w.c1_kernel_points_host = self._kp(c1.KPConv)
        w.c1_w, w.c1_b = _p(c1.KPConv.weights), _p(c1.KPConv.bias)
        w.c1_gn_w, w.c1_gn_b = _p(c1.norm.norm.weight), _p(c1.norm.norm.bias)
        for i, name in enumerate(_BLOCK_NAMES):
            b = getattr(enc, name)
            assert int(b.group_norm) == w.groups
            blk = w.blocks[i]
            blk.cin, blk.cout, blk.strided, blk.sigma = int(b.in_channels), int(b.out_channels), int(bool(b.strided)), float(b.KPConv.sigma)
            blk.kernel_points_host = self._kp(b.KPConv)
            blk.kp_w, blk.kp_b = _p(b.KPConv.weights), _p(b.KPConv.bias)
            wt = b.KPConv.weights_t()
            self.keep.append(wt)
            blk.kp_wt = _p(wt)
            from . import functional as F
            if F.gemm_split_enabled() and F.gemm_split_ok(wt.shape[0], wt.shape[1]):
                wts = b.KPConv.weights_t_split()
                self.keep.append(wts)
                blk.kp_wt_split = _p(wts)
            blk.normconv_w, blk.normconv_b = _p(b.norm_conv.norm.weight), _p(b.norm_conv.norm.bias)
            blk.unary1, blk.unary2, blk.shortcut = _unary(b.unary1, self.keep), _unary(b.unary2, self.keep), _unary(b.unary_shortcut, self.keep)
        self.w = w
        self.out_channels = [int(getattr(enc, n).out_channels) for n in ("encoder1_2", "encoder2_3", "encoder3_3", "encoder4_3")]

    def _kp(self, kpconv):
        a = np.ascontiguousarray(kpconv.kernel_points_host(), dtype=np.float32)
        assert a.shape == (15, 3)
        self.keep.append(a)
        return ctypes.c_void_p(a.ctypes.data)


class _Key:

    def __init__(self, enc):
        from . import functional as F
        self.split = F.gemm_split_enabled()
        self.tensors, self.children, self.sizes = [], [], []
        for m in enc.modules():
            for d in (m._parameters, m._buffers):
                self.sizes.append((d, len(d)))
                for name, t in d.items():
                    if t is not None:
                        self.tensors.append((d, name, F.WeightStamp(t)))
            self.sizes.append((m._modules, len(m._modules)))
            for name, c in m._modules.items():
                self.children.append((m._modules, name, c))

    def valid(self, enc):
        from . import functional as F
        if self.split != F.gemm_split_enabled():
            return False
        for d, n in self.sizes:
            if len(d) != n:
                return False
        for d, name, c in self.children:
            if d.get(name) is not c:
                return False
        for d, name, st in self.tensors:
            t = d.get(name)
            if t is None or not st.same(t):
                return False
        return True


LISTS_VALID_FIRST = 1


def table_for(enc):
    cached = getattr(enc, "_native_table", None)
    if cached is None or not cached[0].valid(enc):
        from . import functional as F
        with F.derived_lock:
            cached = getattr(enc, "_native_table", None)
            if cached is None or not cached[0].valid(enc):
                key = _Key(enc)
                tab = EncoderTable(enc)
                dev = next(enc.parameters()).device
                if dev.type == "cuda":
                    torch.cuda.current_stream(dev).synchronize()
                cached = (key, tab)
                enc._native_table = cached
    return cached[1]


def eligible(feats, data_dict):
    P, N, S = data_dict["points"], data_dict["neighbors"], data_dict["subsampling"]
    return (feats.is_cuda and feats.dtype == torch.float32 and feats.dim() == 2 and feats.shape[1] == 1 and len(P) == 4 and len(N) == 4
            and len(S) == 3 and all(t.dtype == torch.int32 and t.is_contiguous() for t in list(N) + list(S))
            and all(t.dtype == torch.float32 and t.is_contiguous() for t in P)
            and all(int(S[i].shape[1]) == int(N[i].shape[1]) and int(S[i].shape[0]) == int(P[i + 1].shape[0]) for i in range(3)))


def forward(enc, feats, data_dict):
    tab = table_for(enc)
    P, N, Sub = data_dict["points"], data_dict["neighbors"], data_dict["subsampling"]
    dev = feats.device
    n = [int(p.shape[0]) for p in P]
    seg = data_dict.get("segment_lengths")
    from .backbone4 import segment_min_rows
    rows = [r or 0 for r in segment_min_rows(data_dict)]
    if seg is None:
        seg = [torch.full((1,), int(k), dtype=torch.int64, device=dev) for k in n]
        rows = list(n)
    seg = [s.contiguous() for s in seg]
    nseg = int(seg[0].numel())
    order = data_dict.get("order")
    limits = [int(N[i].shape[1]) for i in range(4)]
    for i in range(3):
        assert int(Sub[i].shape[1]) == limits[i] and int(Sub[i].shape[0]) == n[i + 1]
    L = _lib.lib()
    n_host = (ctypes.c_int64 * 4)(*n)
    min_rows = (ctypes.c_int64 * 4)(*rows)
    lim = (ctypes.c_int * 4)(*limits)
    nbytes = ctypes.c_size_t(0)
    _lib.check(L.lcr_encoder_ws_bytes(ctypes.byref(tab.w), n_host, nseg, ctypes.byref(nbytes)), "lcr_encoder_ws_bytes")
    ws = torch.empty(nbytes.value, dtype=torch.uint8, device=dev)
    outs = [torch.empty((n[i], tab.out_channels[i]), dtype=torch.float32, device=dev) for i in range(4)]
    vp4 = ctypes.c_void_p * 4
    pts = vp4(*[p.data_ptr() for p in P])
    nb = vp4(*[t.data_ptr() for t in N])
    sb = vp4(*([t.data_ptr() for t in Sub] + [None]))
    od = vp4(*[t.data_ptr() for t in order]) if order is not None else None
    sg = vp4(*[t.data_ptr() for t in seg])
    of = vp4(*[t.data_ptr() for t in outs])
    f0 = feats.contiguous()
    flags = LISTS_VALID_FIRST if data_dict.get("lists_valid_first") else 0
    _lib.check(L.lcr_encoder_forward_ex(ctypes.byref(tab.w), _lib.ptr(f0), pts, nb, sb, od, sg, nseg, n_host, min_rows, lim, of, flags, _lib.ptr(ws),
                                        ws.numel(), _lib.stream_ptr(dev)), "lcr_encoder_forward_ex")
    return outs
```

Measured before the change: 3002 scans/s.

## Fuse residual block tail into one GEMM kernel with recomputed outputs

Adds a fused block-tail kernel that recomputes the unary2 GEMM (with GroupNorm applied on load to the KPConv output) and the shortcut GEMM, then applies both output GroupNorms, the residual add and LeakyReLU in one epilogue. Stats-only GEMM variants run first so the intermediate y and shortcut tensors never reach global memory. This trades extra GEMM arithmetic (each GEMM runs twice) for removing several full-tensor writes, reads and separate normalisation/add kernels. The forward entry point can also take a caller-provided workspace.

```diff
diff --git a/include/lcr_hip.h b/include/lcr_hip.h
--- a/include/lcr_hip.h
+++ b/include/lcr_hip.h
@@ -116,6 +116,18 @@
 int lcr_gemm_f32_anorm(const float* A, const float* B, float* C, int64_t M, int N, int K, const float* bias,
                        const double* a_stats, const float* a_gamma, const float* a_beta, int a_groups, float a_eps,
                        float a_slope, const int64_t* seg_len, int S, int groups, double* stats, void* stream);
+int lcr_gemm_f32_stats_only(const float* A, const float* B, float* C, int64_t M, int N, int K, int transA, int transB,
+                            const float* bias, const float* rowdiv, const int64_t* seg_len, int S, int groups, double* stats,
+                            void* stream);
+int lcr_gemm_f32_anorm_stats_only(const float* A, const float* B, float* C, int64_t M, int N, int K, const float* bias,
+                                  const double* a_stats, const float* a_gamma, const float* a_beta, int a_groups, float a_eps,
+                                  float a_slope, const int64_t* seg_len, int S, int groups, double* stats, void* stream);
+int lcr_block_tail_ok(int64_t M, int mid, int cin, int cout, int has_shortcut, int64_t min_rows);
+int lcr_block_tail(const float* kpo, const double* kp_stats, const float* kp_gamma, const float* kp_beta, int kp_groups,
+                   const float* w2, const float* b2, const double* y_stats, const float* y_gamma, const float* y_beta,
+                   const float* res, const float* ws, const float* bs, const double* r_stats, const float* r_gamma,
+                   const float* r_beta, float* out, int64_t M, int cout, int mid, int cin, int groups, const int64_t* seg_len,
+                   int S, float eps, float slope, void* stream);
 int lcr_gemm_f32_batched_ta(const float* A, const float* B, float* C, int64_t M, int N, int count, const int* k_host,
                             const int64_t* a_off_host, const int64_t* b_off_host, const int64_t* c_off_host, void* stream);
 int lcr_kpconv_aggregate(const float* s_feats, const uint8_t* s_pos, const float* q_pts, const float* s_pts,
diff --git a/include/lcr_hip_debug.h b/include/lcr_hip_debug.h
--- a/include/lcr_hip_debug.h
+++ b/include/lcr_hip_debug.h
@@ -8,6 +8,7 @@
 void lcr_gemm_debug_force_tile(int tile);
 void lcr_gemm_debug_deep(int mode);
 void lcr_gemm_debug_streamk(int mode);
+void lcr_block_tail_debug(int mode);
 void lcr_groupnorm_debug_general(int on);
 void lcr_kpconv_debug_off64(int on);
 
diff --git a/lcr-net_amd/_lib.py b/lcr-net_amd/_lib.py
--- a/lcr-net_amd/_lib.py
+++ b/lcr-net_amd/_lib.py
@@ -46,6 +46,12 @@
     "lcr_gemm_f32": (c_int, [c_vp, c_vp, c_vp, c_i64, c_int, c_int, c_int, c_int, c_vp, c_vp, c_vp, c_int, c_int, c_vp, c_vp]),
     "lcr_gemm_f32_anorm": (c_int, [c_vp, c_vp, c_vp, c_i64, c_int, c_int, c_vp, c_vp, c_vp, c_vp, c_int, c_float, c_float, c_vp, c_int,
                                    c_int, c_vp, c_vp]),
+    "lcr_gemm_f32_stats_only": (c_int, [c_vp, c_vp, c_vp, c_i64, c_int, c_int, c_int, c_int, c_vp, c_vp, c_vp, c_int, c_int, c_vp, c_vp]),
+    "lcr_gemm_f32_anorm_stats_only": (c_int, [c_vp, c_vp, c_vp, c_i64, c_int, c_int, c_vp, c_vp, c_vp, c_vp, c_int, c_float, c_float, c_vp, c_int,
+                                              c_int, c_vp, c_vp]),
+    "lcr_block_tail_ok": (c_int, [c_i64, c_int, c_int, c_int, c_int, c_i64]),
+    "lcr_block_tail": (c_int, [c_vp, c_vp, c_vp, c_vp, c_int, c_vp, c_vp, c_vp, c_vp, c_vp, c_vp, c_vp, c_vp, c_vp, c_vp, c_vp, c_vp, c_i64,
+                               c_int, c_int, c_int, c_int, c_vp, c_int, c_float, c_float, c_vp]),
     "lcr_ktimer_enable": (None, [c_int]),
     "lcr_ktimer_sample": (None, [c_int]),
     "lcr_ktimer_kinds": (None, [ctypes.c_uint]),
diff --git a/lcr-net_amd/csrc/encoder.hip b/lcr-net_amd/csrc/encoder.hip
--- a/lcr-net_amd/csrc/encoder.hip
+++ b/lcr-net_amd/csrc/encoder.hip
@@ -107,6 +107,27 @@
     } else if ((rc = TURN(b.kp_wt ? lcr_gemm_f32(A, b.kp_wt, kpo, M, mid, 15 * mid, 0, 1, b.kp_b, nn, q.seg, sp.S, g, stc, s)
                                   : lcr_gemm_f32(A, b.kp_w, kpo, M, mid, 15 * mid, 0, 0, b.kp_b, nn, q.seg, sp.S, g, stc, s)))) return rc;
   }
+  if (lcr_block_tail_ok(M, mid, b.cin, b.cout, b.shortcut.w != nullptr, q.min_rows)) {
+    double* sty = sp.take();
+    if (!sty) return LCR_ESPACE;
+    if ((rc = TURN(lcr_gemm_f32_anorm_stats_only(kpo, b.unary2.w, nullptr, M, b.cout, mid, b.unary2.b, stc, b.normconv_w, b.normconv_b, g, ENC_GN_EPS,
+                                                 ENC_SLOPE, q.seg, sp.S, g, sty, s))))
+      return rc;
+    const float* res = s_feats;
+    if (b.strided) {
+      float* pooled = ws.take<float>(static_cast<size_t>(M) * b.cin);
+      if (!pooled) return LCR_ESPACE;
+      if ((rc = TURN(lcr_maxpool(s_feats, idx, 0, M, Ns, H, b.cin, pooled, q.order, s)))) return rc;
+      res = pooled;
+    }
+    double* str = nullptr;
+    if (b.shortcut.w) {
+      if (!(str = sp.take())) return LCR_ESPACE;
+      if ((rc = TURN(lcr_gemm_f32_stats_only(res, b.shortcut.w, nullptr, M, b.cout, b.cin, 0, 1, b.shortcut.b, nullptr, q.seg, sp.S, g, str, s)))) return rc;
+    }
+    return TURN(lcr_block_tail(kpo, stc, b.normconv_w, b.normconv_b, g, b.unary2.w, b.unary2.b, sty, b.unary2.gn_w, b.unary2.gn_b, res, b.shortcut.w,
+                               b.shortcut.b, str, b.shortcut.gn_w, b.shortcut.gn_b, out, M, b.cout, mid, b.cin, g, q.seg, sp.S, ENC_GN_EPS, ENC_SLOPE, s));
+  }
   float* y;
   double* sty;
   static const bool no_anorm = getenv("LCR_NO_NORM_ON_LOAD") != nullptr;
diff --git a/lcr-net_amd/csrc/gemm_f32.hip b/lcr-net_amd/csrc/gemm_f32.hip
--- a/lcr-net_amd/csrc/gemm_f32.hip
+++ b/lcr-net_amd/csrc/gemm_f32.hip
@@ -158,7 +158,7 @@
   return s;
 }
 
-template <int BM, int BN, int WM, int WN, int NT>
+template <int BM, int BN, int WM, int WN, int NT, bool STORE = true>
 __device__ __forceinline__ void gemm_epilogue(floatx16 (&acc)[NT], float* __restrict__ C, int64_t M, int N, int64_t m0, int n0, int64_t m_tile,
                                               const GemmEpilogue& ep, const float (&bias_v)[NT], int blk_first, int64_t blk_seg_start,
                                               int64_t blk_seg_end, int wm, int wn, int lane) {
@@ -179,7 +179,7 @@
         for (int r = 0; r < 16; ++r) {
           const unsigned dr = static_cast<unsigned>((r & 3) + 8 * (r >> 2));
           const float v = acc[j][r] / ep.rowdiv[row_l + dr] + bv;
-          C[off0 + dr * static_cast<unsigned>(N)] = v;
+          if (STORE) C[off0 + dr * static_cast<unsigned>(N)] = v;
           acc[j][r] = v;
         }
       } else {
@@ -187,7 +187,7 @@
         for (int r = 0; r < 16; ++r) {
           const unsigned dr = static_cast<unsigned>((r & 3) + 8 * (r >> 2));
           const float v = acc[j][r] + bv;
-          C[off0 + dr * static_cast<unsigned>(N)] = v;
+          if (STORE) C[off0 + dr * static_cast<unsigned>(N)] = v;
           acc[j][r] = v;
         }
       }
@@ -204,7 +204,7 @@
       if (row < M) {
         if (ep.rowdiv) v = v / ep.rowdiv[row];
         v += bv;
-        if (col < N) C[row * N + col] = v;
+        if (STORE && col < N) C[row * N + col] = v;
       } else {
         v = 0.f;
       }
@@ -296,7 +296,7 @@
   }
 }
 
-template <int BM, int BN, int WM, int WN, bool TA, bool TB, bool VEC, bool SHORT = false, bool ANORM = false>
+template <int BM, int BN, int WM, int WN, bool TA, bool TB, bool VEC, bool SHORT = false, bool ANORM = false, bool STATS_ONLY = false>
 __global__ __launch_bounds__(GM_T, SHORT ? 6 : 2) void k_gemm_f32(const float* __restrict__ A, const float* __restrict__ B, float* __restrict__ C,
                                                        int64_t M, int N, int K, GemmEpilogue ep, GemmBatch batch, ANorm an) {
   static_assert(!ANORM || (SHORT && !TA && VEC && BN / (32 * WN) == 1), "normalise-on-load: light form, row-major A");
@@ -572,7 +572,215 @@
       for (int r = 0; r < 16; ++r) acc[j][r] += acc2[j][r];
   }
 
-  gemm_epilogue<BM, BN, WM, WN, NT>(acc, C, M, N, m0, n0, m_tile, ep, bias_v, blk_first, blk_seg_start, blk_seg_end, wm, wn, lane);
+  gemm_epilogue<BM, BN, WM, WN, NT, !STATS_ONLY>(acc, C, M, N, m0, n0, m_tile, ep, bias_v, blk_first, blk_seg_start, blk_seg_end, wm, wn, lane);
+}
+
+struct BlockTail {
+  const float*  kpo;
+  const float*  w2;
+  const float*  b2;
+  const double* y_stats;
+  const float * y_gamma, *y_beta;
+  const float*  res;
+  const float*  ws;
+  const float*  bs;
+  const double* r_stats;
+  const float * r_gamma, *r_beta;
+  float*        out;
+  int64_t       M;
+  int           N, mid, cin, groups, S;
+  const int64_t* seg_len;
+  float         eps, slope;
+};
+
+template <int RM>
+__global__ __launch_bounds__(GM_T, 4) void k_block_tail(BlockTail p, ANorm an) {
+  static_assert(RM == 1 || RM == 2, "plain or GroupNorm-ed residual");
+  constexpr int BM = 64, BN = 64, WN = 2, LDR = GM_BK + 4;
+  __shared__ __attribute__((aligned(16))) float As[BM * LDR];
+  __shared__ __attribute__((aligned(16))) float Bs[BN * LDR];
+  __shared__ __attribute__((aligned(16))) float s_an[4 * AN_KMAX];
+  __shared__ float2 s_mr[2 * 64];
+  __shared__ float2 s_ymr[2 * 64], s_rmr[2 * 64];
+  const int64_t M = p.M;
+  const int N = p.N, K = p.mid;
+  const int lane = threadIdx.x & 63, w = __builtin_amdgcn_readfirstlane(threadIdx.x >> 6);
+  const int wm = w / WN, wn = w % WN;
+  const int ntn = (N + BN - 1) / BN;
+  const int xcd = blockIdx.x & 7, slot_id = blockIdx.x >> 3;
+  const int64_t m_tile = static_cast<int64_t>(slot_id / ntn) * 8 + xcd;
+  const int64_t m0 = m_tile * BM;
+  const int n0 = (slot_id % ntn) * BN;
+  if (m0 >= M) return;
+
+  LoaderT<BM, LDR, true, true> la;
+  LoaderT<BN, LDR, true, true> lb;
+  const int nk1 = (K + GM_BK - 1) / GM_BK, nk2 = RM == 2 ? (p.cin + GM_BK - 1) / GM_BK : 0;
+  auto gload = [&](int t) {
+    if (RM == 2 && t >= nk1) {
+      la.load(p.res, M, p.cin, m0, (t - nk1) * GM_BK);
+      lb.load(p.ws, N, p.cin, n0, (t - nk1) * GM_BK);
+    } else {
+      la.load(p.kpo, M, K, m0, t * GM_BK);
+      lb.load(p.w2, N, K, n0, t * GM_BK);
+    }
+  };
+  gload(0);
+  const int col = n0 + wn * 32 + (lane & 31);
+  const bool col_ok = col < N;
+  const int colc = col_ok ? col : N - 1;
+  const float bias_y = p.b2 ? p.b2[colc] : 0.f, gam_y = p.y_gamma[colc], bet_y = p.y_beta[colc];
+  float bias_r = 0.f, gam_r = 0.f, bet_r = 0.f;
+  if (RM == 2) {
+    bias_r = p.bs ? p.bs[colc] : 0.f;
+    gam_r = p.r_gamma[colc];
+    bet_r = p.r_beta[colc];
+  }
+  float an_g[2] = {0.f, 0.f}, an_b[2] = {0.f, 0.f};
+#pragma unroll
+  for (int u = 0; u < 2; ++u) {
+    const int e = threadIdx.x + u * GM_T;
+    if (e < 2 * K) {
+      const int k = e >= K ? e - K : e;
+      an_g[u] = an.gamma[k];
+      an_b[u] = an.beta[k];
+    }
+  }
+  int blk_first = 0;
+  int64_t blk_seg_end = p.seg_len[0];
+  while (blk_first + 1 < p.S && m0 >= blk_seg_end) {
+    ++blk_first;
+    blk_seg_end += p.seg_len[blk_first];
+  }
+  const int an_split = static_cast<int>(min(static_cast<int64_t>(BM), blk_seg_end - m0));
+  const int gs_a = K / an.groups, gs_o = N / p.groups;
+  const int g_lo = n0 / gs_o, g_n = (min(n0 + BN, N) - 1) / gs_o - g_lo + 1;
+  if (threadIdx.x < 2 * an.groups) {
+    const int e = threadIdx.x;
+    const int slot = e >= an.groups ? 1 : 0, g = e - slot * an.groups;
+    const int sg = min(blk_first + slot, p.S - 1);
+    const double cnt = static_cast<double>(p.seg_len[sg]) * gs_a;
+    double sx = 0.0, sxx = 0.0;
+    for (int rep = 0; rep < GN_REPLICAS; ++rep) {
+      const int64_t o = ((static_cast<int64_t>(rep) * p.S + sg) * an.groups + g) * 2;
+      sx += an.stats[o];
+      sxx += an.stats[o + 1];
+    }
+    const double mean = sx / cnt;
+    const double var = fmax(sxx / cnt - mean * mean, 0.0);
+    s_mr[e] = make_float2(static_cast<float>(mean), static_cast<float>(1.0 / sqrt(var + static_cast<double>(an.eps))));
+  } else if (threadIdx.x >= 128 && threadIdx.x - 128 < 2 * g_n) {
+    const int e = threadIdx.x - 128;
+    const int slot = e >= g_n ? 1 : 0, g = g_lo + e - slot * g_n;
+    const int sg = min(blk_first + slot, p.S - 1);
+    const double cnt = static_cast<double>(p.seg_len[sg]) * gs_o;
+    double sx = 0.0, sxx = 0.0, rx = 0.0, rxx = 0.0;
+    for (int rep = 0; rep < GN_REPLICAS; ++rep) {
+      const int64_t o = ((static_cast<int64_t>(rep) * p.S + sg) * p.groups + g) * 2;
+      sx += p.y_stats[o];
+      sxx += p.y_stats[o + 1];
+      if (RM == 2) {
+        rx += p.r_stats[o];
+        rxx += p.r_stats[o + 1];
+      }
+    }
+    const double m = sx / cnt;
+    const double var = fmax(sxx / cnt - m * m, 0.0);
+    s_ymr[slot * 64 + e - slot * g_n] = make_float2(static_cast<float>(m), static_cast<float>(1.0 / sqrt(var + static_cast<double>(p.eps))));
+    if (RM == 2) {
+      const double rm = rx / cnt;
+      const double rv = fmax(rxx / cnt - rm * rm, 0.0);
+      s_rmr[slot * 64 + e - slot * g_n] = make_float2(static_cast<float>(rm), static_cast<float>(1.0 / sqrt(rv + static_cast<double>(p.eps))));
+    }
+  }
+  __syncthreads();
+#pragma unroll
+  for (int u = 0; u < 2; ++u) {
+    const int e = threadIdx.x + u * GM_T;
+    if (e < 2 * K) {
+      const int slot = e >= K ? 1 : 0, k = e - slot * K;
+      const float2 mr = s_mr[slot * an.groups + k / gs_a];
+      const float sc = mr.y * an_g[u];
+      s_an[slot * 2 * AN_KMAX + k] = sc;
+      s_an[slot * 2 * AN_KMAX + AN_KMAX + k] = fmaf(-mr.x, sc, an_b[u]);
+    }
+  }
+  float xa[2], xb[2], ra[2] = {1.f, 1.f}, rb[2] = {0.f, 0.f};
+#pragma unroll
+  for (int sl = 0; sl < 2; ++sl) {
+    const int gi = sl * 64 + colc / gs_o - g_lo;
+    const float2 mr = s_ymr[gi];
+    xa[sl] = mr.y * gam_y;
+    xb[sl] = fmaf(-mr.x, xa[sl], bet_y);
+    if (RM == 2) {
+      const float2 rr = s_rmr[gi];
+      ra[sl] = rr.y * gam_r;
+      rb[sl] = fmaf(-rr.x, ra[sl], bet_r);
+    }
+  }
+  __syncthreads();
+
+  floatx16 acc, accr;
+#pragma unroll
+  for (int r = 0; r < 16; ++r) acc[r] = accr[r] = 0.f;
+  const int half = lane >> 5;
+  const float* as = As + (wm * 32 + (lane & 31)) * LDR + half * 16;
+  const float* bs = Bs + (wn * 32 + (lane & 31)) * LDR + half * 16;
+  auto kstep = [&](int t, floatx16& c, bool norm) {
+    if (t > 0) __syncthreads();
+    if (norm) la.store_norm(As, s_an, an_split, an.slope);
+    else la.store(As);
+    lb.store(Bs);
+    if (t + 1 < nk1 + nk2) gload(t + 1);
+    __syncthreads();
+#pragma unroll
+    for (int q = 0; q < 4; ++q) {
+      const float4 a4 = *reinterpret_cast<const float4*>(as + 4 * q), b4 = *reinterpret_cast<const float4*>(bs + 4 * q);
+      c = __builtin_amdgcn_mfma_f32_32x32x2f32(a4.x, b4.x, c, 0, 0, 0);
+      c = __builtin_amdgcn_mfma_f32_32x32x2f32(a4.y, b4.y, c, 0, 0, 0);
+      c = __builtin_amdgcn_mfma_f32_32x32x2f32(a4.z, b4.z, c, 0, 0, 0);
+      c = __builtin_amdgcn_mfma_f32_32x32x2f32(a4.w, b4.w, c, 0, 0, 0);
+    }
+  };
+  for (int t = 0; t < nk1; ++t) kstep(t, acc, true);
+  if (RM == 2)
+    for (int t = nk1; t < nk1 + nk2; ++t) kstep(t, accr, false);
+
+  const int64_t wrow0 = m0 + wm * 32;
+  const bool interior = m0 + BM <= M && n0 + BN <= N && M * static_cast<int64_t>(N) < (int64_t(1) << 30);
+  const int row_in0 = wm * 32 + 4 * half;
+  if (interior) {
+    const unsigned off0 = (static_cast<unsigned>(m0) + static_cast<unsigned>(row_in0)) * static_cast<unsigned>(N) + static_cast<unsigned>(col);
+    float rv[16];
+    if (RM == 1) {
+#pragma unroll
+      for (int r = 0; r < 16; ++r) rv[r] = p.res[off0 + static_cast<unsigned>((r & 3) + 8 * (r >> 2)) * static_cast<unsigned>(N)];
+    }
+#pragma unroll
+    for (int r = 0; r < 16; ++r) {
+      const int dr = (r & 3) + 8 * (r >> 2);
+      const int sl = row_in0 + dr >= an_split ? 1 : 0;
+      float v = fmaf(acc[r] + bias_y, xa[sl], xb[sl]);
+      if (RM == 2) v += fmaf(accr[r] + bias_r, ra[sl], rb[sl]);
+      else v += rv[r];
+      v = v > 0.f ? v : v * p.slope;
+      p.out[off0 + static_cast<unsigned>(dr) * static_cast<unsigned>(N)] = v;
+    }
+  } else {
+#pragma unroll
+    for (int r = 0; r < 16; ++r) {
+      const int dr = (r & 3) + 8 * (r >> 2);
+      const int64_t row = wrow0 + 4 * half + dr;
+      if (row < M && col_ok) {
+        const int sl = row_in0 + dr >= an_split ? 1 : 0;
+        float v = fmaf(acc[r] + bias_y, xa[sl], xb[sl]);
+        if (RM == 2) v += fmaf(accr[r] + bias_r, ra[sl], rb[sl]);
+        else v += p.res[row * N + col];
+        v = v > 0.f ? v : v * p.slope;
+        p.out[row * N + col] = v;
+      }
+    }
+  }
 }
 
 template <int N_OUTSTANDING>
@@ -1316,10 +1524,10 @@
   return GF_TILE;
 }
 
-extern "C" int lcr_gemm_f32_anorm(const float* A, const float* B, float* C, int64_t M, int N, int K, const float* bias,
-                                  const double* a_stats, const float* a_gamma, const float* a_beta, int a_groups, float a_eps,
-                                  float a_slope, const int64_t* seg_len, int S, int groups, double* stats, void* stream) {
-  if (!A || !B || !C || M < 0 || N <= 32 || K <= 0 || K > AN_KMAX || K % 4 != 0 || !a_stats || !a_gamma || !a_beta || a_groups < 1 ||
+static int gemm_anorm_impl(bool stats_only, const float* A, const float* B, float* C, int64_t M, int N, int K, const float* bias,
+                           const double* a_stats, const float* a_gamma, const float* a_beta, int a_groups, float a_eps, float a_slope,
+                           const int64_t* seg_len, int S, int groups, double* stats, void* stream) {
+  if (!A || !B || (!C && !stats_only) || (stats_only && !stats) || M < 0 || N <= 32 || K <= 0 || K > AN_KMAX || K % 4 != 0 || !a_stats || !a_gamma || !a_beta || a_groups < 1 ||
       K % a_groups != 0 || a_groups > 64 || !seg_len || S < 1 || reinterpret_cast<uintptr_t>(A) % 16 != 0 || reinterpret_cast<uintptr_t>(B) % 16 != 0) {
     set_error("lcr_gemm_f32_anorm: needs 32 < N, K <= 256, K % 4 == 0, a_groups dividing K, a segment table and 16-byte aligned operands");
     return LCR_EARG;
@@ -1337,9 +1545,105 @@
   GemmEpilogue ep{bias, nullptr, seg_len, S, groups, stats};
   ANorm an{a_stats, a_gamma, a_beta, a_groups, a_eps, a_slope};
   const int mt8 = (div_up(M, 64) + 7) / 8 * 8;
-  LCR_LAUNCH_TIMED((k_gemm_f32<64, 64, 2, 2, false, true, true, true, true>), dim3(mt8 * div_up(N, 64)), dim3(GM_T), 0, st, A, B, C, M,
+  if (stats_only)
+    LCR_LAUNCH_TIMED((k_gemm_f32<64, 64, 2, 2, false, true, true, true, true, true>), dim3(mt8 * div_up(N, 64)), dim3(GM_T), 0, st, A, B, C, M,
+                     N, K, ep, GemmBatch{}, an);
+  else
+    LCR_LAUNCH_TIMED((k_gemm_f32<64, 64, 2, 2, false, true, true, true, true>), dim3(mt8 * div_up(N, 64)), dim3(GM_T), 0, st, A, B, C, M,
                      N, K, ep, GemmBatch{}, an);
   return check_launch("lcr_gemm_f32_anorm");
+}
+
+extern "C" int lcr_gemm_f32_anorm(const float* A, const float* B, float* C, int64_t M, int N, int K, const float* bias,
+                                  const double* a_stats, const float* a_gamma, const float* a_beta, int a_groups, float a_eps,
+                                  float a_slope, const int64_t* seg_len, int S, int groups, double* stats, void* stream) {
+  return gemm_anorm_impl(false, A, B, C, M, N, K, bias, a_stats, a_gamma, a_beta, a_groups, a_eps, a_slope, seg_len, S, groups, stats, stream);
+}
+
+extern "C" int lcr_gemm_f32_anorm_stats_only(const float* A, const float* B, float* C, int64_t M, int N, int K, const float* bias,
+                                             const double* a_stats, const float* a_gamma, const float* a_beta, int a_groups, float a_eps,
+                                             float a_slope, const int64_t* seg_len, int S, int groups, double* stats, void* stream) {
+  return gemm_anorm_impl(true, A, B, C, M, N, K, bias, a_stats, a_gamma, a_beta, a_groups, a_eps, a_slope, seg_len, S, groups, stats, stream);
+}
+
+extern "C" int lcr_gemm_f32_stats_only(const float* A, const float* B, float* C, int64_t M, int N, int K, int transA, int transB,
+                                       const float* bias, const float* rowdiv, const int64_t* seg_len, int S, int groups, double* stats,
+                                       void* stream) {
+  if (!A || !B || M < 0 || N <= 0 || K <= 0 || !stats || !seg_len || S < 1 || groups < 1 || N % groups != 0 ||
+      ((N / groups) & (N / groups - 1)) != 0) {
+    set_error("lcr_gemm_f32_stats_only: needs operands, a statistics table, seg_len, S >= 1 and groups dividing N into power-of-two sized groups");
+    return LCR_EARG;
+  }
+  const bool vec = K % 4 == 0 && reinterpret_cast<uintptr_t>(A) % 16 == 0 && reinterpret_cast<uintptr_t>(B) % 16 == 0;
+  if (transA || !transB || gemm_form(M, N, K, 0, 1, vec) != GF_SHORT) {
+    set_error("lcr_gemm_f32_stats_only: only the light form (A [M,K], B [N,K], K %% 4 == 0, K <= 256, 16-byte aligned operands)");
+    return LCR_EARG;
+  }
+  hipStream_t st = static_cast<hipStream_t>(stream);
+  KernelTimerScope timed(KT_GEMM, st, M, N, K);
+  if (M == 0) return LCR_OK;
+  GemmEpilogue ep{bias, rowdiv, seg_len, S, groups, stats};
+  if (N <= 32) {
+    const int mt8 = (div_up(M, 128) + 7) / 8 * 8;
+    LCR_LAUNCH_TIMED((k_gemm_f32<128, 32, 4, 1, false, true, true, true, false, true>), dim3(mt8 * div_up(N, 32)), dim3(GM_T), 0, st, A, B, C, M, N, K,
+                     ep, GemmBatch{}, ANorm{});
+  } else {
+    const int mt8 = (div_up(M, 64) + 7) / 8 * 8;
+    LCR_LAUNCH_TIMED((k_gemm_f32<64, 64, 2, 2, false, true, true, true, false, true>), dim3(mt8 * div_up(N, 64)), dim3(GM_T), 0, st, A, B, C, M, N, K,
+                     ep, GemmBatch{}, ANorm{});
+  }
+  return check_launch("lcr_gemm_f32_stats_only");
+}
+
+constexpr bool BT_DEFAULT_ON = false;
+static int g_force_block_tail = -1;
+extern "C" void lcr_block_tail_debug(int mode) { g_force_block_tail = mode; }
+constexpr double BT_HBM_BYTES_PER_S = 8e12, BT_FP32_FLOPS = 157.3e12, BT_FACTOR = 0.7;
+static bool block_tail_recompute_ok(int64_t M, int mid, int cin, int cout, bool has_shortcut, int64_t min_rows) {
+  static const bool env_on = getenv("LCR_BLOCK_TAIL") ? atoi(getenv("LCR_BLOCK_TAIL")) != 0 : BT_DEFAULT_ON;
+  const bool off = g_force_block_tail >= 0 ? g_force_block_tail == 0 : !env_on;
+  static const bool no_anorm = getenv("LCR_NO_NORM_ON_LOAD") != nullptr;
+  if (off || no_anorm || M < 1 || mid < 1 || cin < 1 || cout < 1) return false;
+  if (!(mid <= AN_KMAX && mid % 4 == 0 && cout > 32 && min_rows >= 64)) return false;
+  if (has_shortcut && (cin % 4 != 0 || gemm_form(M, cout, cin, 0, 1, true) != GF_SHORT)) return false;
+  if (!has_shortcut && cin != cout) return false;
+  const double tensors = has_shortcut ? 2.0 : 1.0;
+  const double t_bytes = 8.0 * static_cast<double>(M) * cout * tensors / BT_HBM_BYTES_PER_S;
+  const double t_flops = 2.0 * static_cast<double>(M) * cout * (mid + (has_shortcut ? cin : 0)) / BT_FP32_FLOPS;
+  return t_bytes >= BT_FACTOR * t_flops;
+}
+extern "C" int lcr_block_tail_ok(int64_t M, int mid, int cin, int cout, int has_shortcut, int64_t min_rows) {
+  return block_tail_recompute_ok(M, mid, cin, cout, has_shortcut != 0, min_rows) ? 1 : 0;
+}
+
+extern "C" int lcr_block_tail(const float* kpo, const double* kp_stats, const float* kp_gamma, const float* kp_beta, int kp_groups,
+                              const float* w2, const float* b2, const double* y_stats, const float* y_gamma, const float* y_beta,
+                              const float* res, const float* ws, const float* bs, const double* r_stats, const float* r_gamma,
+                              const float* r_beta, float* out, int64_t M, int cout, int mid, int cin, int groups, const int64_t* seg_len,
+                              int S, float eps, float slope, void* stream) {
+  const bool sc = ws != nullptr;
+  const auto al16 = [](const void* q) { return reinterpret_cast<uintptr_t>(q) % 16 == 0; };
+  if (!kpo || !kp_stats || !kp_gamma || !kp_beta || !w2 || !y_stats || !y_gamma || !y_beta || !res || !out || !seg_len || M < 0 || S < 1 ||
+      (sc && (!r_stats || !r_gamma || !r_beta))) {
+    set_error("lcr_block_tail: bad argument");
+    return LCR_EARG;
+  }
+  if (cout <= 32 || mid < 1 || mid > AN_KMAX || mid % 4 != 0 || kp_groups < 1 || kp_groups > 64 || mid % kp_groups != 0 || groups < 1 ||
+      cout % groups != 0 || ((cout / groups) & (cout / groups - 1)) != 0 || (sc && (cin < 1 || cin > AN_KMAX || cin % 4 != 0)) ||
+      !al16(kpo) || !al16(w2) || (sc && (!al16(res) || !al16(ws)))) {
+    set_error("lcr_block_tail: needs 32 < cout, mid and cin <= 256 and multiples of 4, kp_groups <= 64 dividing mid, groups dividing cout into "
+              "power-of-two sized groups and 16-byte aligned operands");
+    return LCR_EARG;
+  }
+  hipStream_t st = static_cast<hipStream_t>(stream);
+  KernelTimerScope timed(KT_GEMM, st, M, cout, mid + (sc ? cin : 0));
+  if (M == 0) return LCR_OK;
+  BlockTail p{kpo, w2, b2, y_stats, y_gamma, y_beta, res, ws, bs, r_stats, r_gamma, r_beta, out, M, cout, mid, sc ? cin : 0, groups, S, seg_len, eps, slope};
+  ANorm an{kp_stats, kp_gamma, kp_beta, kp_groups, eps, slope};
+  const int mt8 = (div_up(M, 64) + 7) / 8 * 8;
+  if (sc) LCR_LAUNCH_TIMED((k_block_tail<2>), dim3(mt8 * div_up(cout, 64)), dim3(GM_T), 0, st, p, an);
+  else LCR_LAUNCH_TIMED((k_block_tail<1>), dim3(mt8 * div_up(cout, 64)), dim3(GM_T), 0, st, p, an);
+  return check_launch("lcr_block_tail");
 }
 
 extern "C" int lcr_gemm_f32(const float* A, const float* B, float* C, int64_t M, int N, int K, int transA, int transB, const float* bias,
diff --git a/lcr-net_amd/functional.py b/lcr-net_amd/functional.py
--- a/lcr-net_amd/functional.py
+++ b/lcr-net_amd/functional.py
@@ -278,6 +278,60 @@
         int(a_groups), GN_EPS, float(slope), _lib.ptr(seg_len), S, int(groups), _lib.ptr(stats), _lib.stream_ptr(a.device)),
         "lcr_gemm_f32_anorm"), meta=(M, N, K))
     return c, stats
+
+
+def gemm_stats_only(a, weight, bias=None, seg_len=None, groups=0, c=None):
+    _lib.require_cuda(a, weight)
+    assert a.dtype == torch.float32 and weight.dtype == torch.float32 and a.is_contiguous() and weight.is_contiguous() and groups
+    M, K = a.shape
+    N = weight.shape[0]
+    assert weight.shape[1] == K, "inner dimensions differ"
+    seg_len = _seg(seg_len, M, a.device)
+    S = seg_len.numel()
+    stats = _zero_stats(S, groups, a.device)
+    _timed("gemm", lambda: _lib.check(_lib.lib().lcr_gemm_f32_stats_only(
+        _lib.ptr(a), _lib.ptr(weight), _lib.ptr(c), M, N, K, 0, 1, _lib.ptr(bias), None, _lib.ptr(seg_len), S, int(groups), _lib.ptr(stats),
+        _lib.stream_ptr(a.device)), "lcr_gemm_f32_stats_only"), meta=(M, N, K))
+    return stats
+
+
+def gemm_anorm_stats_only(a, a_stats, a_gamma, a_beta, a_groups, weight, bias=None, seg_len=None, groups=0, slope=0.1, c=None):
+    _lib.require_cuda(a, weight)
+    assert a.dtype == torch.float32 and weight.dtype == torch.float32 and a.is_contiguous() and weight.is_contiguous() and groups
+    M, K = a.shape
+    N = weight.shape[0]
+    assert weight.shape[1] == K and gemm_anorm_ok(K, N)
+    seg_len = _seg(seg_len, M, a.device)
+    S = seg_len.numel()
+    stats = _zero_stats(S, groups, a.device)
+    _timed("gemm", lambda: _lib.check(_lib.lib().lcr_gemm_f32_anorm_stats_only(
+        _lib.ptr(a), _lib.ptr(weight), _lib.ptr(c), M, N, K, _lib.ptr(bias), _lib.ptr(a_stats), _lib.ptr(a_gamma), _lib.ptr(a_beta),
+        int(a_groups), GN_EPS, float(slope), _lib.ptr(seg_len), S, int(groups), _lib.ptr(stats), _lib.stream_ptr(a.device)),
+        "lcr_gemm_f32_anorm_stats_only"), meta=(M, N, K))
+    return stats
+
+
+def block_tail_ok(M, mid, cin, cout, has_shortcut, min_rows):
+    return bool(_lib.lib().lcr_block_tail_ok(int(M), int(mid), int(cin), int(cout), int(bool(has_shortcut)), int(min_rows or 0)))
+
+
+def block_tail(kpo, kp_norm, unary2, y_norm, res, shortcut=None, r_norm=None, groups=32, seg_len=None, slope=0.1):
+    _lib.require_cuda(kpo, res)
+    (w2, b2), (ws, bs) = unary2, shortcut if shortcut is not None else (None, None)
+    rs, rg, rb = r_norm if r_norm is not None else (None, None, None)
+    M, mid = kpo.shape
+    cout = w2.shape[0]
+    cin = ws.shape[1] if ws is not None else cout
+    assert kpo.is_contiguous() and res.is_contiguous() and w2.is_contiguous() and w2.shape[1] == mid
+    assert tuple(res.shape) == (M, cin) and (ws is None or (ws.is_contiguous() and ws.shape[0] == cout))
+    seg_len = _seg(seg_len, M, kpo.device)
+    out = torch.empty((M, cout), dtype=torch.float32, device=kpo.device)
+    _timed("gemm", lambda: _lib.check(_lib.lib().lcr_block_tail(
+        _lib.ptr(kpo), _lib.ptr(kp_norm[0]), _lib.ptr(kp_norm[1]), _lib.ptr(kp_norm[2]), int(groups), _lib.ptr(w2), _lib.ptr(b2),
+        _lib.ptr(y_norm[0]), _lib.ptr(y_norm[1]), _lib.ptr(y_norm[2]), _lib.ptr(res), _lib.ptr(ws), _lib.ptr(bs), _lib.ptr(rs), _lib.ptr(rg),
+        _lib.ptr(rb), _lib.ptr(out), M, cout, mid, cin, int(groups), _lib.ptr(seg_len), seg_len.numel(), GN_EPS, float(slope),
+        _lib.stream_ptr(kpo.device)), "lcr_block_tail"), meta=(M, cout, mid + (cin if ws is not None else 0)))
+    return out
 
 
 def groupnorm_stats(x, groups, seg_len=None):
diff --git a/lcr-net_amd/modules/kpconv/modules.py b/lcr-net_amd/modules/kpconv/modules.py
--- a/lcr-net_amd/modules/kpconv/modules.py
+++ b/lcr-net_amd/modules/kpconv/modules.py
@@ -132,6 +132,16 @@
             x, pos = self.unary1(s_feats, s_ctx, want_pos=True)
         x, stats = self.KPConv.forward_raw(x, q_points, s_points, neighbor_indices, s_pos=pos, seg_len=q_ctx.seg_len, groups=g,
                                            order=q_ctx.order)
+        has_sc = not isinstance(self.unary_shortcut, nn.Identity)
+        if F.block_tail_ok(x.shape[0], x.shape[1], self.in_channels, self.out_channels, has_sc,
+                           x.shape[0] if q_ctx.seg_len is None else q_ctx.min_rows):
+            nc, u2, us = self.norm_conv.norm, self.unary2, self.unary_shortcut
+            ystats = F.gemm_anorm_stats_only(x, stats, nc.weight, nc.bias, g, u2.mlp.weight, bias=u2.mlp.bias, seg_len=q_ctx.seg_len, groups=g)
+            shortcut = F.maxpool(s_feats, neighbor_indices, order=q_ctx.order) if self.strided else s_feats
+            rstats = F.gemm_stats_only(shortcut, us.mlp.weight, bias=us.mlp.bias, seg_len=q_ctx.seg_len, groups=g) if has_sc else None
+            return F.block_tail(x, (stats, nc.weight, nc.bias), (u2.mlp.weight, u2.mlp.bias), (ystats, u2.norm.norm.weight, u2.norm.norm.bias),
+                                shortcut, (us.mlp.weight, us.mlp.bias) if has_sc else None,
+                                (rstats, us.norm.norm.weight, us.norm.norm.bias) if has_sc else None, groups=g, seg_len=q_ctx.seg_len)
         if q_ctx.norm_on_load(x.shape[1], self.out_channels, x.shape[0]):
             y, ystats = F.gemm_anorm(x, stats, self.norm_conv.norm.weight, self.norm_conv.norm.bias, g, self.unary2.mlp.weight,
                                      bias=self.unary2.mlp.bias, seg_len=q_ctx.seg_len, groups=g)
diff --git a/lcr-net_amd/native_encoder.py b/lcr-net_amd/native_encoder.py
--- a/lcr-net_amd/native_encoder.py
+++ b/lcr-net_amd/native_encoder.py
@@ -141,7 +141,7 @@
             and all(int(S[i].shape[1]) == int(N[i].shape[1]) and int(S[i].shape[0]) == int(P[i + 1].shape[0]) for i in range(3)))
 
 
-def forward(enc, feats, data_dict):
+def forward(enc, feats, data_dict, ws=None):
     tab = table_for(enc)
     P, N, Sub = data_dict["points"], data_dict["neighbors"], data_dict["subsampling"]
     dev = feats.device
@@ -164,7 +164,9 @@
     lim = (ctypes.c_int * 4)(*limits)
     nbytes = ctypes.c_size_t(0)
     _lib.check(L.lcr_encoder_ws_bytes(ctypes.byref(tab.w), n_host, nseg, ctypes.byref(nbytes)), "lcr_encoder_ws_bytes")
-    ws = torch.empty(nbytes.value, dtype=torch.uint8, device=dev)
+    if ws is None:
+        ws = torch.empty(nbytes.value, dtype=torch.uint8, device=dev)
+    assert ws.dtype == torch.uint8 and ws.is_contiguous() and ws.numel() >= nbytes.value and ws.device == dev
     outs = [torch.empty((n[i], tab.out_channels[i]), dtype=torch.float32, device=dev) for i in range(4)]
     vp4 = ctypes.c_void_p * 4
     pts = vp4(*[p.data_ptr() for p in P])
```

Result: no change. 3002 scans/s, median of 2 (+0.0%).
